# LARS-research/RED-GNN

Hardware: AMD Instinct MI355X
Metric: edges aggregated/sec + MRR-eval queries/sec, family KG n_layer=3 at 1/2/4/8 GPU (higher is better)
Workload: dtype f32; 1 GPU; C2 synthetic KG 10000 entities / 50 relations / 200000 triples (seed 1234), n_layer=3 hidden_dim=64 attn_dim=5, eval step = expansion + fused layers + GRU/readout + filtered ranking, 1024 queries per GPU; batch_per_gpu=1024, global_batch=1024

## Files before the change

include/redgnn.h:

```cpp
#ifndef REDGNN_H
#define REDGNN_H

#include <stddef.h>
#include <stdint.h>

#ifdef __cplusplus
extern "C" {
#endif

typedef struct rg_graph rg_graph;
typedef struct rg_frontier rg_frontier;

const char* rg_last_error(void);
int rg_version(void);
int rg_hipgraph_fill_nodes(void* hip_graph);

int rg_graph_create(int32_t n_ent, int32_t n_rel, const int32_t* triples_host, int64_t n,
                    int add_inverse, rg_graph** out);
int rg_graph_create_device(int32_t n_ent, int32_t n_rel, const int32_t* triples_dev, int64_t n,
                           int add_inverse, void* stream, rg_graph** out);
int rg_graph_export_packs(const rg_graph* g, int32_t* n_packs, int32_t* n_vrows, int32_t* ent_host, int32_t* pack_host, int32_t* rows_host,
                          int32_t* vrows_host);
int rg_tgraph_create(int32_t n_ent, int32_t n_rela_rows, int32_t n_time, const int32_t* quads_host, int64_t n,
                     rg_graph** out);
int rg_tgraph_create_excluding(int32_t n_ent, int32_t n_rela_rows, int32_t n_time, const int32_t* quads_host, int64_t n,
                               const int64_t* exclude_rows_host, int64_t n_exclude, rg_graph** out);
int rg_graph_destroy(rg_graph* g);
int64_t rg_graph_n_fact(const rg_graph* g);
int rg_graph_export(const rg_graph* g, int32_t* out_ptr_host, int32_t* out_rel_tail_host,
                    int32_t* in_ptr_host, int32_t* in_head_rel_host);
int rg_graph_export_out_by_tail(const rg_graph* g, int32_t* rel_tail_host, int32_t* pos_host, uint32_t* packed_host);
int rg_graph_export_time(const rg_graph* g, int32_t* out_time_host, int32_t* in_time_host);

size_t rg_frontier_workspace_bytes(int32_t n_ent, int32_t batch, int32_t n_levels);
int rg_frontier_create(int32_t n_ent, int32_t batch, int32_t n_levels, void* workspace_dev,
                       size_t workspace_bytes, rg_frontier** out);
int rg_frontier_destroy(rg_frontier* f);
int rg_frontier_reset(rg_frontier* f, const int32_t* q_sub_dev, void* stream);
int rg_frontier_reset_nodes(rg_frontier* f, const int32_t* nodes_dev, int64_t n, void* stream);
int rg_frontier_expand(rg_frontier* f, const rg_graph* g, int64_t* counts_host, void* stream);
int rg_frontier_expand_async(rg_frontier* f, const rg_graph* g, void* stream);
int rg_frontier_expand_nodes_async(rg_frontier* f, const rg_graph* g, int32_t* nodes_out, int32_t* prev_idx_out, void* stream);
int rg_frontier_set_edge_hint(rg_frontier* f, int64_t n_edges);
const int32_t* rg_frontier_count_ptr(const rg_frontier* f);
int rg_frontier_level_counts(const rg_frontier* f, int64_t* counts_host, void* stream);
int rg_frontier_nodes(const rg_frontier* f, int32_t* nodes_out, int32_t* prev_idx_out,
                      int32_t* old_nodes_new_idx_out, void* stream);
size_t rg_frontier_edges_scratch_bytes(int64_t n_new);
int rg_frontier_edges(const rg_frontier* f, const rg_graph* g, int32_t level,
                      const int32_t* nodes_new, int64_t n_new, int32_t* edges_out,
                      int32_t* row_ptr_out, void* scratch_dev, void* stream);

size_t rg_layer_fwd_scratch_bytes(const rg_frontier* f, const rg_graph* g, int32_t ld);
int rg_layer_fwd_plan(const rg_frontier* f, const rg_graph* g, int32_t level, int64_t n_old, int64_t n_new,
                      int64_t n_edges, int32_t ld);
int rg_layer_fwd_single_source(const rg_frontier* f, const rg_graph* g, int32_t level);
int rg_layer_fwd(const rg_frontier* f, const rg_graph* g, int32_t level, int64_t n_new,
                 const float* hidden, const float* rela, int32_t d, int32_t ld,
                 const float* a_s, const float* a_r, const float* a_q, int32_t ap,
                 const float* w_alpha, const float* b_alpha, int32_t attn_dim,
                 float* agg_out, void* scratch_dev, size_t scratch_bytes, int32_t walk, void* stream);

int rg_attn_tables(int32_t n_layer, int32_t n_rela_rows, int32_t batch, int32_t d, int32_t ld, int32_t attn_dim, int32_t ap,
                   const float* const* rela, const float* const* Wr, const float* const* Wqr, const float* const* bqr,
                   const int64_t* q_rel, float* a_r_out, float* a_q_out, float* rela_pad_out, void* stream);

int rg_tlayer_fwd(const rg_frontier* f, const rg_graph* g, int32_t level, int64_t n_new, const int32_t* q_time,
                  const float* hidden_dir, const float* rela_dir, const float* time_dir, int32_t d, int32_t ld,
                  const float* a_s, const float* a_r, const float* a_q, int32_t ap,
                  const float* w_alpha, const float* b_alpha, int32_t attn_dim,
                  float* agg_out, void* scratch_dev, size_t scratch_bytes, void* stream);

int rg_frontier_set_window(rg_frontier* f, const int32_t* win_lo_dev, const int32_t* win_hi_dev, int32_t n_data);
int rg_xlayer_fwd(const rg_frontier* f, const rg_graph* g, int32_t level, int64_t n_new, const int32_t* q_time,
                  const int32_t* loop_time, const int32_t* row_time, int32_t n_data,
                  const float* hidden_p, const float* rela_p, const float* time_p, int32_t n_tab, int32_t d, int32_t ld,
                  const float* a_s, const float* a_r, const float* a_q, int32_t ap,
                  const float* w_alpha, const float* b_alpha, int32_t attn_dim,
                  float* agg_out, void* scratch_dev, size_t scratch_bytes, void* stream);

size_t rg_layer_bwd_scratch_bytes(const rg_frontier* f, const rg_graph* g, int32_t ld, int32_t ap);
int rg_layer_bwd(const rg_frontier* f, const rg_graph* g, int32_t level, int64_t n_old,
                 const float* hidden, const float* rela, int32_t d, int32_t ld,
                 const float* a_s, const float* a_r, const float* a_q, int32_t ap,
                 const float* w_alpha, const float* b_alpha, int32_t attn_dim,
                 const float* grad_agg,
                 float* grad_hidden, float* grad_rela, float* grad_a_s, float* grad_a_r, float* grad_a_q,
                 float* grad_w_alpha, float* grad_b_alpha,
                 void* scratch_dev, size_t scratch_bytes, void* stream);

size_t rg_tlayer_bwd_scratch_bytes(const rg_frontier* f, const rg_graph* g, int32_t ld, int32_t ap);
int rg_tlayer_bwd(const rg_frontier* f, const rg_graph* g, int32_t level, int64_t n_old, const int32_t* q_time,
                  const float* hidden_dir, const float* rela_dir, const float* time_dir, int32_t d, int32_t ld,
                  const float* a_s, const float* a_r, const float* a_q, int32_t ap,
                  const float* w_alpha, const float* b_alpha, int32_t attn_dim,
                  const float* grad_agg,
                  float* grad_hidden_dir, float* grad_rela_dir, float* grad_time_dir, float* grad_a_s, float* grad_a_r,
                  float* grad_a_q, float* grad_w_alpha,
                  void* scratch_dev, size_t scratch_bytes, void* stream);

int rg_xlayer_bwd(const rg_frontier* f, const rg_graph* g, int32_t level, int64_t n_old, const int32_t* q_time,
                  const int32_t* loop_time, const int32_t* row_time, int32_t n_data,
                  const float* hidden_p, const float* rela_p, const float* time_p, int32_t n_tab, int32_t d, int32_t ld,
                  const float* a_s, const float* a_r, const float* a_q, int32_t ap,
                  const float* w_alpha, const float* b_alpha, int32_t attn_dim,
                  const float* grad_agg,
                  float* grad_hidden_p, float* grad_rela_p, float* grad_time_p, float* grad_a_s, float* grad_a_r,
                  float* grad_a_q, float* grad_w_alpha,
                  void* scratch_dev, size_t scratch_bytes, void* stream);

int rg_dense_fwd_supported(int32_t d, int32_t attn_dim);
int rg_dense_fwd(int64_t n, int32_t d, int32_t ld, const float* agg, const float* hidden_prev,
                 const int32_t* prev_idx, const float* W_h, int32_t act,
                 const float* w_ih, const float* w_hh, const float* b_ih, const float* b_hh,
                 const float* Ws_next, int32_t attn_dim, int32_t ap, float* a_s_out,
                 const float* W_final, const int32_t* nodes, int32_t n_ent, float* scores_all,
                 float* hidden_out, int32_t precision, void* scratch, int64_t scratch_bytes, void* stream);
int64_t rg_dense_scratch_bytes(int32_t d, int32_t precision);

int rg_split3_roundtrip(const float* x, int64_t n_rows, int32_t cols, float* back, float* parts, void* stream);
int rg_split3_product_check(int32_t which, int64_t n, int32_t d, const float* agg, const float* hidden_prev, const int32_t* prev_idx,
                            const float* W_h, int32_t act, const float* w_ih, const float* w_hh, const float* b_ih, const float* b_hh,
                            float* out, void* stream);

size_t rg_gram_tn_scratch_bytes(int32_t m, int32_t n);
int rg_gram_tn(const float* g, int64_t ldg, int32_t m, const float* x, int64_t ldx, int32_t n, int64_t n_rows, float* out, float* colsum,
               void* scratch_dev, size_t scratch_bytes, void* stream);

int rg_rank(const float* scores, int32_t batch, int32_t n_ent,
            const int32_t* ans_ptr, const int32_t* ans_idx,
            const int32_t* filt_ptr, const int32_t* filt_idx,
            float* ranks_out, void* stream);

int rg_topk(const float* scores, int32_t batch, int32_t n_ent, int32_t k, const int64_t* q_key,
            const int64_t* known_keys, const int64_t* known_ptr, const int32_t* known_idx, int64_t n_keys,
            int32_t* idx_out, float* score_out, void* stream);

int rg_segment_rank(const float* scores, const int32_t* ent, int64_t n_pairs, const void* seg_ptr, int32_t seg_ptr_is64,
                    const int32_t* target, int32_t batch,
                    const int64_t* key_sp, const int64_t* sp_keys, const int64_t* sp_ptr, const int32_t* sp_idx, int64_t n_sp,
                    const int64_t* key_spt, const int64_t* spt_keys, const int64_t* spt_ptr, const int32_t* spt_idx, int64_t n_spt,
                    float* rank_out, float* rank_fil_out, float* rank_fil_t_out, int32_t* found_out, void* stream);

int rg_segment_topk(const float* scores, const int32_t* ent, int64_t n_pairs, const void* seg_ptr, int32_t seg_ptr_is64,
                    int32_t batch, int32_t k, const int64_t* q_key, const int64_t* known_keys, const int64_t* known_ptr,
                    const int32_t* known_idx, int64_t n_keys, int32_t* idx_out, float* score_out, float* prob_out, void* stream);

int rg_segment_eval(const float* scores, const int32_t* ent, int64_t n_pairs, const void* seg_ptr, int32_t seg_ptr_is64,
                    const int32_t* target, int32_t batch, int32_t n_ent,
                    const int64_t* key_a, const int64_t* a_keys, const int64_t* a_ptr, const int32_t* a_idx, int64_t n_a,
                    const int64_t* key_b, const int64_t* b_keys, const int64_t* b_ptr, const int32_t* b_idx, int64_t n_b,
                    float* logp_out, int32_t* count_out, int32_t* visited_out, void* stream);

size_t rg_paths_scratch_bytes(int64_t n_edges, int32_t k);
int rg_paths_topk(const int32_t* edges, const float* alpha, const int64_t* offsets, int32_t row_lo, int32_t row_hi, int32_t n_hops,
                  int32_t k, void* scratch, int64_t* path_edge, double* path_prod, int32_t* path_count, void* stream);

size_t rg_rule_ground_scratch_bytes(int32_t n_ent, int32_t n_rules, int32_t n_sources);
int rg_rule_ground(const rg_graph* g, const int32_t* head, const int32_t* body, int32_t n_rules, int32_t n_hops,
                   const int32_t* sources, int32_t n_sources, void* scratch, int64_t* counts, void* stream);

int rg_dense_fwd_dev(int64_t n_cap, const int32_t* n_dev, int64_t n_hint, int32_t d, int32_t ld, const float* agg, const float* hidden_prev,
                     const int32_t* prev_idx, const float* W_h, int32_t act,
                     const float* w_ih, const float* w_hh, const float* b_ih, const float* b_hh,
                     const float* Ws_next, int32_t attn_dim, int32_t ap, float* a_s_out,
                     const float* W_final, const int32_t* nodes, int32_t n_ent, float* scores_all,
                     float* hidden_out, int32_t precision, void* scratch, int64_t scratch_bytes, void* stream);

int rg_dense_train_fwd(int64_t n, int32_t d, const float* agg, const float* hidden_prev, const int32_t* prev_idx,
                       const float* W_h, int32_t act, const float* w_ih, const float* w_hh, const float* b_ih, const float* b_hh,
                       const float* mask, float* hidden_out, float* x_out, float* gates_ws_out, void* stream);

int rg_dense_train_fwd_as(int64_t n, int32_t d, const float* agg, const float* hidden_prev, const int32_t* prev_idx,
                          const float* W_h, int32_t act, const float* w_ih, const float* w_hh, const float* b_ih, const float* b_hh,
                          const float* mask, const float* Ws_next, int32_t attn_dim, int32_t ap,
                          float* hidden_out, float* x_out, float* gates_ws_out, float* a_s_out, void* stream);

int rg_rows_addmm(const float* base, int64_t ldb, const float* g, int64_t ldg, int32_t k, const float* W, int32_t n, int64_t n_rows,
                  float* out, int64_t ldo, void* stream);

int rg_rows_linear(const float* x, int64_t n_rows, int64_t ldx, int32_t k, const float* w, const float* bias, int32_t n,
                   float* out, int64_t ldo, void* stream);

int rg_dense_train_bwd(int64_t n, int32_t d, const float* grad_hidden, const float* gates_ws, const float* x, const float* mask,
                       float keep, int32_t act, const float* W_h, const float* w_ih, const float* w_hh,
                       float* grad_gates_i, float* grad_gates_h, float* grad_pre, float* grad_agg, float* grad_h0, void* stream);

int rg_dense_train_bwd2(int64_t n, int32_t d, const float* grad_hidden, const float* gates_ws, const float* x, const float* mask,
                        float keep, int32_t act, const float* W_h, const float* w_ih, const float* w_hh, const int32_t* prev_idx,
                        float* grad_gates_i, float* grad_gates_hn, float* grad_pre, float* grad_agg, float* grad_prev, void* stream);

size_t rg_explain_scratch_bytes(const rg_frontier* f);
int rg_explain_seed(const rg_frontier* f, int32_t batch, int32_t n_ent, int32_t level, const int32_t* objs, uint32_t* marks_out,
                    uint8_t* reached_out, void* stream);
int rg_explain_count(const rg_frontier* f, const rg_graph* g, int32_t batch, int32_t n_ent, int32_t level, const uint32_t* marks,
                     const float* a_s, const float* a_r, const float* a_q, int32_t ap, const float* w_alpha, const float* b_alpha,
                     int32_t attn_dim, float min_alpha, uint32_t* marks_prev_out, int32_t* word_ptr_out, void* scratch,
                     size_t scratch_bytes, int64_t* n_edges_host, void* stream);
int rg_explain_emit(const rg_frontier* f, const rg_graph* g, int32_t batch, int32_t n_ent, int32_t level, const uint32_t* marks,
                    const float* a_s, const float* a_r, const float* a_q, int32_t ap, const float* w_alpha, const float* b_alpha,
                    int32_t attn_dim, float min_alpha, const int32_t* word_ptr, int32_t* edges_out, float* alpha_out, void* stream);
int rg_explain_gather(int64_t n, int32_t hop, int32_t batch, const int32_t* edges, const float* alpha, const int64_t* row_first,
                      const int64_t* row_base, int64_t n_out, int32_t* edges_out, float* alpha_out, void* stream);

int rg_texplain_count(const rg_frontier* f, const rg_graph* g, int32_t batch, int32_t n_ent, int32_t level, const uint32_t* marks,
                      const float* a_s, const float* a_r, const float* a_q, int32_t ap, const float* w_alpha, const float* b_alpha,
                      int32_t attn_dim, float min_alpha, uint32_t* marks_prev_out, int32_t* word_ptr_out, void* scratch,
                      size_t scratch_bytes, int64_t* n_edges_host, void* stream);
int rg_texplain_emit(const rg_frontier* f, const rg_graph* g, int32_t batch, int32_t n_ent, int32_t level, const uint32_t* marks,
                     const float* a_s, const float* a_r, const float* a_q, int32_t ap, const float* w_alpha, const float* b_alpha,
                     int32_t attn_dim, float min_alpha, const int32_t* word_ptr, int32_t* edges_out, float* alpha_out,
                     int32_t* time_out, void* stream);

int rg_xexplain_count(const rg_frontier* f, const rg_graph* g, int32_t batch, int32_t n_ent, int32_t level, const uint32_t* marks,
                      const float* a_s, const float* a_r, const float* a_q, int32_t ap, const float* w_alpha, const float* b_alpha,
                      int32_t attn_dim, float min_alpha, uint32_t* marks_prev_out, int32_t* word_ptr_out, void* scratch,
                      size_t scratch_bytes, int64_t* n_edges_host, void* stream);
int rg_xexplain_emit(const rg_frontier* f, const rg_graph* g, int32_t batch, int32_t n_ent, int32_t level, const uint32_t* marks,
                     const float* a_s, const float* a_r, const float* a_q, int32_t ap, const float* w_alpha, const float* b_alpha,
                     int32_t attn_dim, float min_alpha, const int32_t* word_ptr, int32_t* edges_out, float* alpha_out,
                     int32_t* row_out, void* stream);

int rg_attn_profile(const rg_frontier* f, const rg_graph* g, int32_t batch, int32_t n_ent, int32_t level, int64_t n_old,
                    const float* a_s, const float* a_r, const float* a_q, int32_t ap, const float* w_alpha, const float* b_alpha,
                    int32_t attn_dim, int64_t* sum_out, int64_t* count_out, void* stream);

int rg_tattn_profile(const rg_frontier* f, const rg_graph* g, int32_t batch, int32_t n_ent, int32_t level, int64_t n_old,
                     const int32_t* q_time, const float* a_s, const float* a_r, const float* a_q, int32_t ap, const float* w_alpha,
                     const float* b_alpha, int32_t attn_dim, int64_t* sum_out, int64_t* count_out, void* stream);

int rg_xattn_profile(const rg_frontier* f, const rg_graph* g, int32_t batch, int32_t n_ent, int32_t level, int64_t n_old,
                     const int32_t* q_time, const int32_t* loop_time, const int32_t* row_time,
                     const uint8_t* lag_bin, int32_t n_lag, int32_t n_bins,
                     const float* a_s, const float* a_r, const float* a_q, int32_t ap, const float* w_alpha,
                     const float* b_alpha, int32_t attn_dim, int64_t* sum_out, int64_t* count_out, void* stream);

#ifdef __cplusplus
}
#endif
#endif
```

red-gnn_amd/_lib.py:

```python
import ctypes as C
import os

_PKG = os.path.dirname(os.path.abspath(__file__))
LIB_PATH = os.environ.get("RG_LIB") or os.path.join(_PKG, "libredgnn.so")

SYMBOLS = [
    "rg_last_error", "rg_version", "rg_hipgraph_fill_nodes",
    "rg_graph_create", "rg_graph_create_device", "rg_graph_export_packs", "rg_tgraph_create", "rg_tgraph_create_excluding", "rg_graph_destroy", "rg_graph_n_fact", "rg_graph_export", "rg_graph_export_out_by_tail",
    "rg_frontier_workspace_bytes", "rg_frontier_create", "rg_frontier_destroy", "rg_frontier_reset",
    "rg_frontier_reset_nodes", "rg_frontier_expand", "rg_frontier_nodes", "rg_frontier_edges_scratch_bytes", "rg_frontier_edges",
    "rg_layer_fwd_scratch_bytes", "rg_layer_fwd", "rg_layer_fwd_plan", "rg_layer_fwd_single_source", "rg_tlayer_fwd", "rg_xlayer_fwd", "rg_frontier_set_window", "rg_layer_bwd_scratch_bytes", "rg_layer_bwd", "rg_tlayer_bwd_scratch_bytes", "rg_tlayer_bwd", "rg_xlayer_bwd", "rg_dense_fwd_supported", "rg_dense_scratch_bytes", "rg_dense_fwd", "rg_dense_fwd_dev", "rg_dense_train_fwd", "rg_dense_train_fwd_as", "rg_rows_addmm", "rg_dense_train_bwd", "rg_dense_train_bwd2", "rg_split3_roundtrip", "rg_split3_product_check", "rg_gram_tn_scratch_bytes", "rg_gram_tn", "rg_rank",
    "rg_frontier_expand_async", "rg_frontier_expand_nodes_async", "rg_frontier_set_edge_hint", "rg_frontier_count_ptr", "rg_frontier_level_counts", "rg_attn_tables",
    "rg_explain_scratch_bytes", "rg_explain_seed", "rg_explain_count", "rg_explain_emit", "rg_explain_gather",
    "rg_topk",
    "rg_attn_profile",
    "rg_graph_export_time", "rg_texplain_count", "rg_texplain_emit", "rg_tattn_profile",
    "rg_segment_rank", "rg_segment_topk",
    "rg_xexplain_count", "rg_xexplain_emit",
    "rg_xattn_profile", "rg_rows_linear",
    "rg_segment_eval",
    "rg_paths_scratch_bytes", "rg_paths_topk",
    "rg_rule_ground_scratch_bytes", "rg_rule_ground",
]

_lib = None


class NativeError(RuntimeError):
    pass


def lib():
    global _lib
    if _lib is not None:
        return _lib
    if not os.path.exists(LIB_PATH):
        raise NativeError(
            "libredgnn.so is missing at %s: the HIP extension is not built. Run "
            "`python -c 'import __graft_entry__ as g; g.build()'` (needs hipcc). There is no CPU fallback." % LIB_PATH)
    import torch
    L = C.CDLL(LIB_PATH)
    vp, i32, i64, sz = C.c_void_p, C.c_int32, C.c_int64, C.c_size_t
    L.rg_last_error.restype = C.c_char_p
    L.rg_version.restype = C.c_int
    L.rg_hipgraph_fill_nodes.argtypes = [vp]
    L.rg_graph_create.argtypes = [i32, i32, vp, i64, C.c_int, C.POINTER(vp)]
    L.rg_graph_create_device.argtypes = [i32, i32, vp, i64, C.c_int, vp, C.POINTER(vp)]
    L.rg_graph_export_packs.argtypes = [vp, C.POINTER(i32), C.POINTER(i32), vp, vp, vp, vp]
    L.rg_tgraph_create.argtypes = [i32, i32, i32, vp, i64, C.POINTER(vp)]
    L.rg_tgraph_create_excluding.argtypes = [i32, i32, i32, vp, i64, vp, i64, C.POINTER(vp)]
    L.rg_graph_destroy.argtypes = [vp]
    L.rg_graph_n_fact.argtypes = [vp]
    L.rg_graph_n_fact.restype = i64
    L.rg_graph_export.argtypes = [vp, vp, vp, vp, vp]
    L.rg_graph_export_out_by_tail.argtypes = [vp, vp, vp, vp]
    L.rg_frontier_workspace_bytes.argtypes = [i32, i32, i32]
    L.rg_frontier_workspace_bytes.restype = sz
    L.rg_frontier_create.argtypes = [i32, i32, i32, vp, sz, C.POINTER(vp)]
    L.rg_frontier_destroy.argtypes = [vp]
    L.rg_frontier_reset.argtypes = [vp, vp, vp]
    L.rg_frontier_reset_nodes.argtypes = [vp, vp, i64, vp]
    L.rg_frontier_expand.argtypes = [vp, vp, C.POINTER(i64), vp]
    L.rg_frontier_expand_async.argtypes = [vp, vp, vp]
    L.rg_frontier_expand_nodes_async.argtypes = [vp, vp, vp, vp, vp]
    L.rg_frontier_set_edge_hint.argtypes = [vp, i64]
    L.rg_attn_tables.argtypes = [i32, i32, i32, i32, i32, i32, i32, vp, vp, vp, vp, vp, vp, vp, vp, vp]
    L.rg_frontier_count_ptr.argtypes = [vp]
    L.rg_frontier_count_ptr.restype = vp
    L.rg_frontier_level_counts.argtypes = [vp, C.POINTER(i64), vp]
    L.rg_frontier_nodes.argtypes = [vp, vp, vp, vp, vp]
    L.rg_frontier_edges_scratch_bytes.argtypes = [i64]
    L.rg_frontier_edges_scratch_bytes.restype = sz
    L.rg_frontier_edges.argtypes = [vp, vp, i32, vp, i64, vp, vp, vp, vp]
    L.rg_layer_fwd_scratch_bytes.argtypes = [vp, vp, i32]
    L.rg_layer_fwd_scratch_bytes.restype = sz
    L.rg_layer_fwd.argtypes = [vp, vp, i32, i64, vp, vp, i32, i32, vp, vp, vp, i32, vp, vp, i32, vp, vp, sz, i32, vp]
    L.rg_layer_fwd_plan.argtypes = [vp, vp, i32, i64, i64, i64, i32]
    L.rg_layer_fwd_single_source.argtypes = [vp, vp, i32]
    L.rg_tlayer_fwd.argtypes = [vp, vp, i32, i64, vp, vp, vp, vp, i32, i32, vp, vp, vp, i32, vp, vp, i32, vp, vp, sz, vp]
    L.rg_xlayer_fwd.argtypes = [vp, vp, i32, i64, vp, vp, vp, i32, vp, vp, vp, i32, i32, i32, vp, vp, vp, i32, vp, vp, i32, vp, vp, sz, vp]
    L.rg_frontier_set_window.argtypes = [vp, vp, vp, i32]
    L.rg_layer_bwd_scratch_bytes.argtypes = [vp, vp, i32, i32]
    L.rg_layer_bwd_scratch_bytes.restype = sz
    L.rg_layer_bwd.argtypes = [vp, vp, i32, i64, vp, vp, i32, i32, vp, vp, vp, i32, vp, vp, i32,
                               vp, vp, vp, vp, vp, vp, vp, vp, vp, sz, vp]
    L.rg_tlayer_bwd_scratch_bytes.argtypes = [vp, vp, i32, i32]
    L.rg_tlayer_bwd_scratch_bytes.restype = sz
    L.rg_tlayer_bwd.argtypes = [vp, vp, i32, i64, vp, vp, vp, vp, i32, i32, vp, vp, vp, i32, vp, vp, i32,
                                vp, vp, vp, vp, vp, vp, vp, vp, vp, sz, vp]
    L.rg_xlayer_bwd.argtypes = [vp, vp, i32, i64, vp, vp, vp, i32, vp, vp, vp, i32, i32, i32, vp, vp, vp, i32, vp, vp, i32,
                                vp, vp, vp, vp, vp, vp, vp, vp, vp, sz, vp]
    L.rg_dense_fwd_supported.argtypes = [i32, i32]
    L.rg_dense_fwd.argtypes = [i64, i32, i32, vp, vp, vp, vp, i32, vp, vp, vp, vp, vp, i32, i32, vp, vp, vp, i32, vp, vp, i32, vp, i64, vp]
    L.rg_dense_scratch_bytes.argtypes = [i32, i32]
    L.rg_dense_scratch_bytes.restype = i64
    L.rg_dense_fwd_dev.argtypes = [i64, vp, i64, i32, i32, vp, vp, vp, vp, i32, vp, vp, vp, vp, vp, i32, i32, vp, vp, vp, i32, vp, vp, i32, vp, i64, vp]
    L.rg_dense_train_fwd.argtypes = [i64, i32, vp, vp, vp, vp, i32, vp, vp, vp, vp, vp, vp, vp, vp, vp]
    L.rg_dense_train_fwd_as.argtypes = [i64, i32, vp, vp, vp, vp, i32, vp, vp, vp, vp, vp, vp, i32, i32, vp, vp, vp, vp, vp]
    L.rg_rows_addmm.argtypes = [vp, i64, vp, i64, i32, vp, i32, i64, vp, i64, vp]
    L.rg_dense_train_bwd.argtypes = [i64, i32, vp, vp, vp, vp, C.c_float, i32, vp, vp, vp, vp, vp, vp, vp, vp, vp]
    L.rg_dense_train_bwd2.argtypes = [i64, i32, vp, vp, vp, vp, C.c_float, i32, vp, vp, vp, vp, vp, vp, vp, vp, vp, vp]
    L.rg_rank.argtypes = [vp, i32, i32, vp, vp, vp, vp, vp, vp]
    L.rg_topk.argtypes = [vp, i32, i32, i32, vp, vp, vp, vp, i64, vp, vp, vp]
    L.rg_split3_roundtrip.argtypes = [vp, i64, i32, vp, vp, vp]
    L.rg_gram_tn_scratch_bytes.argtypes = [i32, i32]
    L.rg_gram_tn_scratch_bytes.restype = sz
    L.rg_gram_tn.argtypes = [vp, i64, i32, vp, i64, i32, i64, vp, vp, vp, sz, vp]
    L.rg_split3_product_check.argtypes = [i32, i64, i32, vp, vp, vp, vp, i32, vp, vp, vp, vp, vp, vp]
    L.rg_explain_scratch_bytes.argtypes = [vp]
    L.rg_explain_scratch_bytes.restype = sz
    L.rg_explain_seed.argtypes = [vp, i32, i32, i32, vp, vp, vp, vp]
    L.rg_explain_count.argtypes = [vp, vp, i32, i32, i32, vp, vp, vp, vp, i32, vp, vp, i32, C.c_float, vp, vp, vp, sz,
                                   C.POINTER(i64), vp]
    L.rg_explain_emit.argtypes = [vp, vp, i32, i32, i32, vp, vp, vp, vp, i32, vp, vp, i32, C.c_float, vp, vp, vp, vp]
    L.rg_explain_gather.argtypes = [i64, i32, i32, vp, vp, vp, vp, i64, vp, vp, vp]
    L.rg_attn_profile.argtypes = [vp, vp, i32, i32, i32, i64, vp, vp, vp, i32, vp, vp, i32, vp, vp, vp]
    L.rg_graph_export_time.argtypes = [vp, vp, vp]
    L.rg_texplain_count.argtypes = L.rg_explain_count.argtypes
    L.rg_texplain_emit.argtypes = [vp, vp, i32, i32, i32, vp, vp, vp, vp, i32, vp, vp, i32, C.c_float, vp, vp, vp, vp, vp]
    L.rg_tattn_profile.argtypes = [vp, vp, i32, i32, i32, i64, vp, vp, vp, vp, i32, vp, vp, i32, vp, vp, vp]
    L.rg_segment_rank.argtypes = [vp, vp, i64, vp, i32, vp, i32, vp, vp, vp, vp, i64, vp, vp, vp, vp, i64, vp, vp, vp, vp, vp]
    L.rg_segment_topk.argtypes = [vp, vp, i64, vp, i32, i32, i32, vp, vp, vp, vp, i64, vp, vp, vp, vp]
    L.rg_segment_eval.argtypes = [vp, vp, i64, vp, i32, vp, i32, i32, vp, vp, vp, vp, i64, vp, vp, vp, vp, i64, vp, vp, vp, vp]
    L.rg_xexplain_count.argtypes = L.rg_explain_count.argtypes
    L.rg_xexplain_emit.argtypes = L.rg_texplain_emit.argtypes
    L.rg_rows_linear.argtypes = [vp, i64, i64, i32, vp, vp, i32, vp, i64, vp]
    L.rg_xattn_profile.argtypes = [vp, vp, i32, i32, i32, i64, vp, vp, vp, vp, i32, i32, vp, vp, vp, i32, vp, vp, i32, vp, vp, vp]
    L.rg_paths_scratch_bytes.argtypes = [i64, i32]
    L.rg_paths_scratch_bytes.restype = sz
    L.rg_paths_topk.argtypes = [vp, vp, vp, i32, i32, i32, i32, vp, vp, vp, vp, vp]
    L.rg_rule_ground_scratch_bytes.argtypes = [i32, i32, i32]
    L.rg_rule_ground_scratch_bytes.restype = sz
    L.rg_rule_ground.argtypes = [vp, vp, vp, i32, i32, vp, i32, vp, vp, vp]
    _lib = L
    return L


def check(rc):
    if rc != 0:
        raise NativeError(lib().rg_last_error().decode("utf-8", "replace"))


def ptr(t):
    if t is None:
        return None
    if hasattr(t, "data_ptr"):
        return C.c_void_p(t.data_ptr())
    return C.c_void_p(t.ctypes.data)


def stream_ptr():
    import torch
    return C.c_void_p(torch.cuda.current_stream().cuda_stream)
```

red-gnn_amd/csrc/attn.h:

```cpp
#pragma once
#include "common.h"

namespace rg {

__device__ __forceinline__ bool bm_has(const int2& wp, int e) { return ((uint32_t)wp.x >> (e & 31)) & 1u; }
__device__ __forceinline__ int bm_rank(const int2& wp, int e) { return wp.y + __popc((uint32_t)wp.x & ((1u << (e & 31)) - 1u)); }

__device__ __forceinline__ float4 f4add(const float4& a, const float4& b) { return make_float4(a.x + b.x, a.y + b.y, a.z + b.z, a.w + b.w); }

__device__ __forceinline__ float4 attn_w4(const float* __restrict__ w_alpha, int attn_dim, int k) {
  float w[4];
#pragma unroll
  for (int u = 0; u < 4; ++u) w[u] = 4 * k + u < attn_dim ? w_alpha[4 * k + u] : 0.f;
  return make_float4(w[0], w[1], w[2], w[3]);
}

template <int AP4, int BLOCK>
__device__ __forceinline__ void stage_attention(float4* ar_l, float4* w_l, const float4* __restrict__ a_r, int n_rows,
                                                const float* __restrict__ w_alpha, int attn_dim) {
  for (int i = threadIdx.x; i < n_rows * AP4; i += BLOCK) ar_l[i] = a_r[i];
  if (threadIdx.x < AP4) w_l[threadIdx.x] = attn_w4(w_alpha, attn_dim, threadIdx.x);
}

__device__ __forceinline__ float attn_term(float& z, float w, float pre) {
  const float zr = fmaxf(pre, 0.f);
  z = fmaf(w, zr, z);
  return zr;
}
__device__ __forceinline__ void attn_acc(float& z, const float4& w, const float4& u, const float4& v, float4& zr) {
  zr.x = attn_term(z, w.x, u.x + v.x);
  zr.y = attn_term(z, w.y, u.y + v.y);
  zr.z = attn_term(z, w.z, u.z + v.z);
  zr.w = attn_term(z, w.w, u.w + v.w);
}
__device__ __forceinline__ void attn_acc(float& z, const float4& w, const float4& u, const float4& v) {
  float4 zr;
  attn_acc(z, w, u, v, zr);
}
__device__ __forceinline__ void attn_acc_fwd(float& z, const float4& w, const float4& as, const float4& ar, const float4& aq) {
  attn_term(z, w.x, as.x + ar.x + aq.x);
  attn_term(z, w.y, as.y + ar.y + aq.y);
  attn_term(z, w.z, as.z + ar.z + aq.z);
  attn_term(z, w.w, as.w + ar.w + aq.w);
}

__device__ __forceinline__ float attn_alpha(float z) { return __builtin_amdgcn_rcpf(1.0f + __expf(-z)); }

template <bool WG_RELEASE>
__device__ __forceinline__ void strip_fence() {
  if constexpr (WG_RELEASE) __builtin_amdgcn_fence(__ATOMIC_RELEASE, "workgroup");
  else __builtin_amdgcn_fence(__ATOMIC_ACQ_REL, "wavefront");
  __builtin_amdgcn_wave_barrier();
}

template <int G, bool WG_RELEASE>
__device__ __forceinline__ int group_compact(float4* my_stage, int lane, bool valid, const float4& t) {
  const int lane_g = lane & (G - 1), gshift = lane & ~(G - 1);
  const unsigned long long gmask = G == 64 ? ~0ull : ((1ull << G) - 1ull);
  const unsigned long long m = (__ballot(valid) >> gshift) & gmask;
  const int cnt = __popcll(m);
  const int pos = __popcll(m & ((1ull << lane_g) - 1ull));
  strip_fence<WG_RELEASE>();
  if (lane_g >= cnt) my_stage[lane_g] = f4zero();
  if (valid) my_stage[pos] = t;
  strip_fence<WG_RELEASE>();
  return cnt;
}

}
```

red-gnn_amd/csrc/common.h:

```cpp
#pragma once
#include <hip/hip_runtime.h>
#include <stdint.h>
#include <stdio.h>
#include <string>
#include <type_traits>

#include "redgnn.h"

namespace rg {

void set_error(const char* fmt, ...);

#define RG_CHECK(cond, ...)                 \
  do {                                      \
    if (!(cond)) {                          \
      ::rg::set_error(__VA_ARGS__);         \
      return 1;                             \
    }                                       \
  } while (0)

#define RG_HIP(expr)                                                                  \
  do {                                                                                \
    hipError_t e_ = (expr);                                                           \
    if (e_ != hipSuccess) {                                                           \
      ::rg::set_error("%s failed: %s (%s:%d)", #expr, hipGetErrorString(e_), __FILE__, \
                      __LINE__);                                                      \
      return 1;                                                                       \
    }                                                                                 \
  } while (0)

#define RG_LAUNCH_CHECK() RG_HIP(hipGetLastError())

int zero_async(void* p, size_t bytes, hipStream_t s);
int zero2_async(void* p1, size_t bytes1, void* p2, size_t bytes2, hipStream_t s);
int copy_words_async(void* dst, const void* src, int n_words, hipStream_t s);

static inline int64_t ceil_div(int64_t a, int64_t b) { return (a + b - 1) / b; }
static inline size_t align_up(size_t x, size_t a) { return (x + a - 1) / a * a; }

size_t scan_scratch_elems(int64_t n);
int scan_exclusive(const uint32_t* in, int32_t* out, int64_t n, bool popc, int32_t* total_dev,
                   int32_t* scratch, hipStream_t s);

template <typename F>
inline int with_ap4(int ap4, const char* who, F&& f) {
  switch (ap4) {
    case 1: return f(std::integral_constant<int, 1>());
    case 2: return f(std::integral_constant<int, 2>());
    case 3: return f(std::integral_constant<int, 3>());
    case 4: return f(std::integral_constant<int, 4>());
    case 8: return f(std::integral_constant<int, 8>());
    default: set_error("%s: padded attention dim %d not in {4,8,12,16,32}", who, ap4 * 4); return 1;
  }
}

template <typename F>
inline int with_g(int ld4, F&& f) {
  if (ld4 <= 4) return f(std::integral_constant<int, 4>());
  if (ld4 <= 8) return f(std::integral_constant<int, 8>());
  if (ld4 <= 16) return f(std::integral_constant<int, 16>());
  if (ld4 <= 32) return f(std::integral_constant<int, 32>());
  return f(std::integral_constant<int, 64>());
}

__device__ __forceinline__ float4 f4zero() { return make_float4(0.f, 0.f, 0.f, 0.f); }

template <int CTRL>
__device__ __forceinline__ float dpp_add(float v) {
  const int t = __builtin_amdgcn_update_dpp(0, __float_as_int(v), CTRL, 0xf, 0xf, false);
  return v + __int_as_float(t);
}

template <int G>
__device__ __forceinline__ float group_sum(float v) {
  if constexpr (G >= 16) {
    v = dpp_add<0x128>(v);
    v = dpp_add<0x124>(v);
    v = dpp_add<0x122>(v);
    v = dpp_add<0x121>(v);
    if constexpr (G >= 32) v += __shfl_xor(v, 16, 64);
    if constexpr (G >= 64) v += __shfl_xor(v, 32, 64);
  } else {
    for (int o = G / 2; o > 0; o >>= 1) v += __shfl_xor(v, o, 64);
  }
  return v;
}

}

#include <vector>
namespace rg { int place_rows_best_fit(const int4* vrows, int32_t n_vrows, std::vector<int4>* place, std::vector<int32_t>* pack_nrows); }

constexpr int RG_VROW_MAX = 128;
struct rg_vrows {
  int32_t n = 0, n_split = 0, n_slots = 0;
  int4* rows = nullptr;
  int4* split = nullptr;
};

constexpr int RG_PACK = 128;
struct rg_packs {
  int32_t n = 0;
  int2* ent = nullptr;
  int4* pack = nullptr;
  int2* rows = nullptr;
};

struct rg_graph {
  void* arena = nullptr;
  int32_t n_ent = 0, n_rel = 0;
  int32_t n_rela_rows = 0;
  int32_t n_time = 0;
  int32_t* in_time = nullptr;
  int32_t* out_time = nullptr;
  int64_t n_fact = 0;
  int32_t max_in_deg = 0, max_out_deg = 0;
  int32_t* out_ptr = nullptr;
  int2* out_rt = nullptr;
  int32_t* in_ptr = nullptr;
  int2* in_hr = nullptr;
  uint32_t* in_pk = nullptr;
  uint32_t* out_pk = nullptr;
  int2* out_bt_rt = nullptr;
  uint32_t* out_bt_pk = nullptr;
  int32_t* out_bt_pos = nullptr;
  rg_vrows in_vr, out_vr;
  rg_packs in_pk_packs;
  int32_t* rel_ptr = nullptr;
  int2* rel_ht = nullptr;
  rg_vrows rel_vr;
  int32_t* rel_tm = nullptr;
  int32_t* time_ptr = nullptr;
  int2* time_ht = nullptr;
  int32_t* time_rel = nullptr;
  rg_vrows time_vr;
};

constexpr int RG_MAX_LEVELS = 16;
constexpr int RG_QSTRIDE = 32;
constexpr size_t RG_QUEUE_BYTES = 8 * RG_QSTRIDE * sizeof(int32_t);
struct rg_frontier {
  int32_t n_ent = 0, B = 0, BW = 0, W = 0, n_levels = 0;
  uint32_t* bitsT[2] = {nullptr, nullptr};
  int2* bm[RG_MAX_LEVELS] = {};
  uint32_t* words_tmp = nullptr;
  int32_t* prefix_tmp = nullptr;
  int32_t* scan_scratch = nullptr;
  int32_t* counters = nullptr;
  const int32_t* win_lo = nullptr;
  const int32_t* win_hi = nullptr;
  int32_t win_n_data = 0;
  mutable bool queues_clean = false;
  int32_t* queues = nullptr;
  int64_t* counts_pinned = nullptr;
  int level = -1;
  int tcur = 0;
  int64_t n_nodes[RG_MAX_LEVELS] = {};
  int64_t n_edges = 0;
  bool single_source = false;
  int32_t* sub = nullptr;
  int64_t edge_hint = -1;
  const int2* bm_of(int lvl) const { return bm[lvl % n_levels]; }
};
```

red-gnn_amd/csrc/graph.hip:

```cpp
#include <stdarg.h>
#include <string.h>

#include <algorithm>
#include <vector>

#include "common.h"

namespace rg {

static thread_local std::string g_err;

void set_error(const char* fmt, ...) {
  char buf[1024];
  va_list ap;
  va_start(ap, fmt);
  vsnprintf(buf, sizeof(buf), fmt, ap);
  va_end(ap);
  g_err = buf;
}

constexpr int SCAN_T = 256;
constexpr int SCAN_ITEMS = 8;
constexpr int SCAN_TILE = SCAN_T * SCAN_ITEMS;

template <bool POPC>
__device__ __forceinline__ int32_t scan_load(const uint32_t* in, int64_t i, int64_t n) {
  if (i >= n) return 0;
  uint32_t v = in[i];
  return POPC ? __popc(v) : (int32_t)v;
}

__device__ __forceinline__ int32_t wave_incl_scan(int32_t v) {
  const int lane = threadIdx.x & 63;
#pragma unroll
  for (int o = 1; o < 64; o <<= 1) {
    int32_t t = __shfl_up(v, o, 64);
    if (lane >= o) v += t;
  }
  return v;
}

__device__ __forceinline__ int32_t block_excl_scan(int32_t v, int32_t* block_total) {
  __shared__ int32_t wsum[SCAN_T / 64];
  const int lane = threadIdx.x & 63, w = threadIdx.x >> 6;
  int32_t inc = wave_incl_scan(v);
  if (lane == 63) wsum[w] = inc;
  __syncthreads();
  int32_t base = 0, tot = 0;
#pragma unroll
  for (int i = 0; i < SCAN_T / 64; ++i) {
    int32_t x = wsum[i];
    if (i < w) base += x;
    tot += x;
  }
  __syncthreads();
  *block_total = tot;
  return base + inc - v;
}

template <bool POPC>
__global__ __launch_bounds__(SCAN_T) void scan_reduce_kernel(const uint32_t* in, int64_t n, int32_t* sums) {
  const int64_t base = (int64_t)blockIdx.x * SCAN_TILE + (int64_t)threadIdx.x * SCAN_ITEMS;
  int32_t acc = 0;
#pragma unroll
  for (int i = 0; i < SCAN_ITEMS; ++i) acc += scan_load<POPC>(in, base + i, n);
  int32_t tot;
  block_excl_scan(acc, &tot);
  if (threadIdx.x == 0) sums[blockIdx.x] = tot;
}

template <bool POPC>
__global__ __launch_bounds__(SCAN_T) void scan_apply_kernel(const uint32_t* in, int32_t* out, int64_t n,
                                                            const int32_t* offsets, int32_t* total) {
  const int64_t base = (int64_t)blockIdx.x * SCAN_TILE + (int64_t)threadIdx.x * SCAN_ITEMS;
  int32_t v[SCAN_ITEMS];
  int32_t acc = 0;
#pragma unroll
  for (int i = 0; i < SCAN_ITEMS; ++i) {
    v[i] = scan_load<POPC>(in, base + i, n);
    acc += v[i];
  }
  int32_t tot;
  int32_t ex = block_excl_scan(acc, &tot);
  if (offsets) ex += offsets[blockIdx.x];
#pragma unroll
  for (int i = 0; i < SCAN_ITEMS; ++i) {
    if (base + i < n) out[base + i] = ex;
    ex += v[i];
  }
  if (!offsets && total && threadIdx.x == 0) *total = tot;
}

__global__ void zero_words_kernel(uint32_t* __restrict__ p, int64_t n_words) {
  const int64_t stride = (int64_t)gridDim.x * blockDim.x;
  for (int64_t i = (int64_t)blockIdx.x * blockDim.x + threadIdx.x; i < n_words; i += stride) p[i] = 0u;
}
__global__ void zero_quads_kernel(uint4* __restrict__ p, int64_t n_quads) {
  const int64_t stride = (int64_t)gridDim.x * blockDim.x;
  for (int64_t i = (int64_t)blockIdx.x * blockDim.x + threadIdx.x; i < n_quads; i += stride) p[i] = make_uint4(0u, 0u, 0u, 0u);
}
__global__ void copy_words_kernel(uint32_t* __restrict__ dst, const uint32_t* __restrict__ src, int n) {
  if ((int)threadIdx.x < n) dst[threadIdx.x] = src[threadIdx.x];
}

int zero_async(void* p, size_t bytes, hipStream_t s) {
  if (bytes == 0) return 0;
  RG_CHECK(((uintptr_t)p & 3) == 0 && (bytes & 3) == 0, "zero_async: unaligned fill (%p, %zu B)", p, bytes);
  if (((uintptr_t)p & 15) == 0 && (bytes & 15) == 0 && bytes >= 4096) {
    const int64_t n = (int64_t)(bytes / 16);
    hipLaunchKernelGGL(zero_quads_kernel, dim3((unsigned)std::min<int64_t>(ceil_div(n, 256), 4096)), dim3(256), 0, s, (uint4*)p, n);
  } else {
    const int64_t n = (int64_t)(bytes / 4);
    hipLaunchKernelGGL(zero_words_kernel, dim3((unsigned)std::min<int64_t>(ceil_div(n, 256), 4096)), dim3(256), 0, s, (uint32_t*)p, n);
  }
  RG_LAUNCH_CHECK();
  return 0;
}

__global__ void zero2_quads_kernel(uint4* __restrict__ p1, int64_t n1, uint4* __restrict__ p2, int64_t n2) {
  const int64_t stride = (int64_t)gridDim.x * blockDim.x;
  for (int64_t i = (int64_t)blockIdx.x * blockDim.x + threadIdx.x; i < n1 + n2; i += stride) {
    if (i < n1) p1[i] = make_uint4(0u, 0u, 0u, 0u);
    else p2[i - n1] = make_uint4(0u, 0u, 0u, 0u);
  }
}

int zero2_async(void* p1, size_t bytes1, void* p2, size_t bytes2, hipStream_t s) {
  if ((((uintptr_t)p1 | (uintptr_t)p2) & 15) != 0 || ((bytes1 | bytes2) & 15) != 0) return zero_async(p1, bytes1, s) || zero_async(p2, bytes2, s);
  const int64_t n = (int64_t)((bytes1 + bytes2) / 16);
  if (n == 0) return 0;
  hipLaunchKernelGGL(zero2_quads_kernel, dim3((unsigned)std::min<int64_t>(ceil_div(n, 256), 4096)), dim3(256), 0, s, (uint4*)p1,
                     (int64_t)(bytes1 / 16), (uint4*)p2, (int64_t)(bytes2 / 16));
  RG_LAUNCH_CHECK();
  return 0;
}

int copy_words_async(void* dst, const void* src, int n_words, hipStream_t s) {
  RG_CHECK(n_words > 0 && n_words <= 256, "copy_words_async: %d words", n_words);
  hipLaunchKernelGGL(copy_words_kernel, dim3(1), dim3(256), 0, s, (uint32_t*)dst, (const uint32_t*)src, n_words);
  RG_LAUNCH_CHECK();
  return 0;
}

size_t scan_scratch_elems(int64_t n) {
  size_t tot = 0;
  while (n > SCAN_TILE) {
    n = ceil_div(n, SCAN_TILE);
    tot += align_up((size_t)n, 64) * 2;
  }
  return tot + 64;
}

int scan_exclusive(const uint32_t* in, int32_t* out, int64_t n, bool popc, int32_t* total_dev,
                   int32_t* scratch, hipStream_t s) {
  if (n <= 0) {
    if (total_dev && zero_async(total_dev, sizeof(int32_t), s)) return 1;
    return 0;
  }
  const int64_t nb = ceil_div(n, SCAN_TILE);
  if (nb == 1) {
    if (popc)
      hipLaunchKernelGGL(scan_apply_kernel<true>, dim3(1), dim3(SCAN_T), 0, s, in, out, n, nullptr, total_dev);
    else
      hipLaunchKernelGGL(scan_apply_kernel<false>, dim3(1), dim3(SCAN_T), 0, s, in, out, n, nullptr, total_dev);
    RG_LAUNCH_CHECK();
    return 0;
  }
  int32_t* sums = scratch;
  int32_t* sums_scanned = scratch + align_up((size_t)nb, 64);
  int32_t* next = sums_scanned + align_up((size_t)nb, 64);
  if (popc)
    hipLaunchKernelGGL(scan_reduce_kernel<true>, dim3(nb), dim3(SCAN_T), 0, s, in, n, sums);
  else
    hipLaunchKernelGGL(scan_reduce_kernel<false>, dim3(nb), dim3(SCAN_T), 0, s, in, n, sums);
  RG_LAUNCH_CHECK();
  if (scan_exclusive((const uint32_t*)sums, sums_scanned, nb, false, total_dev, next, s)) return 1;
  if (popc)
    hipLaunchKernelGGL(scan_apply_kernel<true>, dim3(nb), dim3(SCAN_T), 0, s, in, out, n, sums_scanned, nullptr);
  else
    hipLaunchKernelGGL(scan_apply_kernel<false>, dim3(nb), dim3(SCAN_T), 0, s, in, out, n, sums_scanned, nullptr);
  RG_LAUNCH_CHECK();
  return 0;
}

}

struct HostVrows { std::vector<int4> rows, split; };
static void host_vrows(const std::vector<int32_t>& ptr, int32_t n_ent, HostVrows* h, rg_vrows* out) {
  std::vector<int4>& rows = h->rows;
  std::vector<int4>& split = h->split;
  int32_t slots = 0;
  for (int32_t e = 0; e < n_ent; ++e) {
    const int32_t beg = ptr[e], len = ptr[e + 1] - ptr[e];
    if (len <= RG_VROW_MAX) {
      rows.push_back(make_int4(e, beg, len, -1));
    } else {
      const int32_t n_seg = (len + RG_VROW_MAX - 1) / RG_VROW_MAX;
      split.push_back(make_int4(e, slots, n_seg, 0));
      for (int32_t k = 0; k < n_seg; ++k) {
        const int32_t b = beg + k * RG_VROW_MAX;
        rows.push_back(make_int4(e, b, std::min(RG_VROW_MAX, beg + len - b), slots + k));
      }
      slots += n_seg;
    }
  }
  std::stable_sort(rows.begin(), rows.end(), [](const int4& a, const int4& b) { return a.z > b.z; });
  out->n = (int32_t)rows.size(); out->n_split = (int32_t)split.size(); out->n_slots = slots;
}

struct HostPacks { std::vector<int2> ent; std::vector<int4> pack; std::vector<int2> rows; };

namespace rg {
int place_rows_best_fit(const int4* vrows, int32_t n_vrows, std::vector<int4>* place, std::vector<int32_t>* pack_nrows) {
  std::vector<int32_t> open_by_room[RG_PACK + 1];
  std::vector<int32_t> fill;
  place->assign(n_vrows, make_int4(-1, 0, 0, 0));
  pack_nrows->clear();
  for (int32_t i = 0; i < n_vrows; ++i) {
    const int4& r = vrows[i];
    if (r.z <= 0) continue;
    int32_t p;
    if (r.w >= 0) { p = (int32_t)fill.size(); fill.push_back(0); pack_nrows->push_back(0); }
    else {
      int room = r.z;
      while (room <= RG_PACK && open_by_room[room].empty()) ++room;
      if (room > RG_PACK) { p = (int32_t)fill.size(); fill.push_back(0); pack_nrows->push_back(0); room = RG_PACK; }
      else { p = open_by_room[room].back(); open_by_room[room].pop_back(); }
      if (room - r.z > 0) open_by_room[room - r.z].push_back(p);
    }
    (*place)[i] = make_int4(p, fill[p], (*pack_nrows)[p], 0);
    fill[p] += r.z;
    (*pack_nrows)[p] += 1;
  }
  return (int)fill.size();
}
}

static void host_packs(const std::vector<int4>& vrows, const std::vector<uint32_t>& in_pk, HostPacks* hp, rg_packs* out) {
  std::vector<int4> place;
  std::vector<int32_t> pack_nrows;
  const size_t n = (size_t)rg::place_rows_best_fit(vrows.data(), (int32_t)vrows.size(), &place, &pack_nrows);
  std::vector<int32_t> row0(n + 1, 0);
  for (size_t p = 0; p < n; ++p) row0[p + 1] = row0[p] + pack_nrows[p];
  hp->ent.assign(n * RG_PACK, make_int2(-1, 0));
  hp->pack.resize(n);
  hp->rows.resize(row0[n]);
  for (size_t i = 0; i < vrows.size(); ++i) {
    const int4& r = vrows[i];
    const int4& pl = place[i];
    if (pl.x < 0) continue;
    for (int32_t j = 0; j < r.z; ++j) hp->ent[(size_t)pl.x * RG_PACK + pl.y + j] = make_int2((int32_t)in_pk[r.y + j], pl.z);
    hp->rows[row0[pl.x] + pl.z] = make_int2(r.x, r.w);
    if (pl.z == 0) hp->pack[pl.x] = make_int4(row0[pl.x], pack_nrows[pl.x], r.w, r.x);
  }
  out->n = (int32_t)n;
}

struct Arena {
  struct Item { void** field; const void* src; size_t bytes, off; };
  std::vector<Item> items;
  size_t total = 0;
  template <typename P, typename V>
  void add(P** field, const V& v) {
    const size_t bytes = v.size() * sizeof(typename V::value_type);
    items.push_back({(void**)field, (const void*)v.data(), bytes, total});
    total += rg::align_up(std::max<size_t>(bytes, 16), 256);
  }
};

extern "C" {

const char* rg_last_error(void) { return rg::g_err.c_str(); }
int rg_version(void) { return 12; }

static int build_graph(int32_t n_ent, int32_t n_rel, int32_t n_rela_rows, const std::vector<int32_t>& H,
                       const std::vector<int32_t>& R, const std::vector<int32_t>& T, const std::vector<int32_t>* TIME,
                       int32_t n_time, rg_graph** out) {
  const int64_t n_fact = (int64_t)H.size();
  std::vector<int32_t> out_ptr(n_ent + 1, 0), in_ptr(n_ent + 1, 0);
  for (int64_t i = 0; i < n_fact; ++i) { out_ptr[H[i] + 1]++; in_ptr[T[i] + 1]++; }
  int32_t max_in = 0, max_out = 0;
  for (int32_t e = 0; e < n_ent; ++e) {
    max_out = out_ptr[e + 1] > max_out ? out_ptr[e + 1] : max_out;
    max_in = in_ptr[e + 1] > max_in ? in_ptr[e + 1] : max_in;
    out_ptr[e + 1] += out_ptr[e];
    in_ptr[e + 1] += in_ptr[e];
  }
  std::vector<int2> out_rt(n_fact), in_hr(n_fact);
  std::vector<int32_t> in_time(TIME ? n_fact : 0), out_time(TIME ? n_fact : 0);
  {
    std::vector<int32_t> po(out_ptr.begin(), out_ptr.end() - 1), pi(in_ptr.begin(), in_ptr.end() - 1);
    for (int64_t i = 0; i < n_fact; ++i) {
      const int32_t q = pi[T[i]]++;
      in_hr[q] = make_int2(H[i], R[i]);
      if (TIME) in_time[q] = (*TIME)[i];
    }
    std::vector<int32_t> by_rel(n_fact), out_fact(n_fact);
    {
      std::vector<int32_t> pr(n_rela_rows + 1, 0);
      for (int64_t i = 0; i < n_fact; ++i) pr[R[i] + 1]++;
      for (int32_t r = 0; r < n_rela_rows; ++r) pr[r + 1] += pr[r];
      for (int64_t i = 0; i < n_fact; ++i) by_rel[pr[R[i]]++] = (int32_t)i;
    }
    for (int64_t k = 0; k < n_fact; ++k) out_fact[po[H[by_rel[k]]]++] = by_rel[k];
    for (int64_t j = 0; j < n_fact; ++j) {
      const int32_t i = out_fact[j];
      out_rt[j] = make_int2(R[i], T[i]);
      if (TIME) out_time[j] = (*TIME)[i];
    }
  }
  rg_graph* g = new rg_graph();
  g->n_ent = n_ent; g->n_rel = n_rel; g->n_rela_rows = n_rela_rows; g->n_time = n_time;
  g->n_fact = n_fact; g->max_in_deg = max_in; g->max_out_deg = max_out;
  Arena A;
  A.add(&g->out_ptr, out_ptr); A.add(&g->in_ptr, in_ptr); A.add(&g->out_rt, out_rt); A.add(&g->in_hr, in_hr);
  if (TIME) { A.add(&g->in_time, in_time); A.add(&g->out_time, out_time); }
  std::vector<uint32_t> in_pk, out_pk;
  if (n_ent <= (1 << 20) && n_rela_rows <= (1 << 12)) {
    in_pk.resize(n_fact); out_pk.resize(n_fact);
    for (int64_t i = 0; i < n_fact; ++i) {
      in_pk[i] = ((uint32_t)in_hr[i].y << 20) | (uint32_t)in_hr[i].x;
      out_pk[i] = ((uint32_t)out_rt[i].x << 20) | (uint32_t)out_rt[i].y;
    }
    A.add(&g->in_pk, in_pk); A.add(&g->out_pk, out_pk);
  }
  std::vector<int2> out_bt_rt;
  std::vector<uint32_t> out_bt_pk;
  std::vector<int32_t> out_bt_pos;
  if (!TIME) {
    out_bt_rt.resize(n_fact); out_bt_pos.resize(n_fact);
    std::vector<int32_t> po(out_ptr.begin(), out_ptr.end() - 1);
    for (int32_t t = 0; t < n_ent; ++t)
      for (int32_t q = in_ptr[t]; q < in_ptr[t + 1]; ++q) {
        const int32_t j = po[in_hr[q].x]++;
        out_bt_rt[j] = make_int2(in_hr[q].y, t);
        out_bt_pos[j] = q;
      }
    A.add(&g->out_bt_rt, out_bt_rt); A.add(&g->out_bt_pos, out_bt_pos);
    if (!in_pk.empty()) {
      out_bt_pk.resize(n_fact);
      for (int64_t j = 0; j < n_fact; ++j) out_bt_pk[j] = ((uint32_t)out_bt_rt[j].x << 20) | (uint32_t)out_bt_rt[j].y;
      A.add(&g->out_bt_pk, out_bt_pk);
    }
  }
  std::vector<int32_t> rel_ptr(n_rela_rows + 1, 0), rel_tm(TIME ? n_fact : 0);
  std::vector<int2> rel_ht(n_fact);
  for (int64_t i = 0; i < n_fact; ++i) rel_ptr[R[i] + 1]++;
  for (int32_t r = 0; r < n_rela_rows; ++r) rel_ptr[r + 1] += rel_ptr[r];
  {
    std::vector<int32_t> pr(rel_ptr.begin(), rel_ptr.end() - 1);
    for (int64_t i = 0; i < n_fact; ++i) {
      const int32_t q = pr[R[i]]++;
      rel_ht[q] = make_int2(H[i], T[i]);
      if (TIME) rel_tm[q] = (*TIME)[i];
    }
  }
  A.add(&g->rel_ptr, rel_ptr); A.add(&g->rel_ht, rel_ht);
  std::vector<int32_t> time_ptr, time_rel;
  std::vector<int2> time_ht;
  HostVrows hv_in, hv_out, hv_rel, hv_time;
  if (TIME) {
    A.add(&g->rel_tm, rel_tm);
    time_ptr.assign(n_time + 1, 0); time_rel.resize(n_fact); time_ht.resize(n_fact);
    for (int64_t i = 0; i < n_fact; ++i) time_ptr[(*TIME)[i] + 1]++;
    for (int32_t t = 0; t < n_time; ++t) time_ptr[t + 1] += time_ptr[t];
    std::vector<int32_t> pt(time_ptr.begin(), time_ptr.end() - 1);
    for (int64_t i = 0; i < n_fact; ++i) {
      const int32_t q = pt[(*TIME)[i]]++;
      time_ht[q] = make_int2(H[i], T[i]);
      time_rel[q] = R[i];
    }
    A.add(&g->time_ptr, time_ptr); A.add(&g->time_ht, time_ht); A.add(&g->time_rel, time_rel);
    host_vrows(time_ptr, n_time, &hv_time, &g->time_vr);
    A.add(&g->time_vr.rows, hv_time.rows); A.add(&g->time_vr.split, hv_time.split);
  }
  host_vrows(in_ptr, n_ent, &hv_in, &g->in_vr);
  host_vrows(out_ptr, n_ent, &hv_out, &g->out_vr);
  host_vrows(rel_ptr, n_rela_rows, &hv_rel, &g->rel_vr);
  A.add(&g->in_vr.rows, hv_in.rows); A.add(&g->in_vr.split, hv_in.split);
  A.add(&g->out_vr.rows, hv_out.rows); A.add(&g->out_vr.split, hv_out.split);
  A.add(&g->rel_vr.rows, hv_rel.rows); A.add(&g->rel_vr.split, hv_rel.split);
  HostPacks hp;
  if (!TIME && !in_pk.empty() && n_rela_rows < (1 << 12)) {
    host_packs(hv_in.rows, in_pk, &hp, &g->in_pk_packs);
    A.add(&g->in_pk_packs.ent, hp.ent); A.add(&g->in_pk_packs.pack, hp.pack); A.add(&g->in_pk_packs.rows, hp.rows);
  }

  std::vector<char> staging(A.total);
  for (const Arena::Item& it : A.items)
    if (it.bytes) memcpy(staging.data() + it.off, it.src, it.bytes);
  hipError_t e = hipMalloc(&g->arena, A.total);
  if (e == hipSuccess) e = hipMemcpy(g->arena, staging.data(), A.total, hipMemcpyHostToDevice);
  if (e != hipSuccess) {
    rg::set_error("rg_graph_create: uploading %zu B failed: %s", A.total, hipGetErrorString(e));
    rg_graph_destroy(g);
    return 1;
  }
  for (const Arena::Item& it : A.items) *it.field = (char*)g->arena + it.off;
  *out = g;
  return 0;
}

int rg_graph_create(int32_t n_ent, int32_t n_rel, const int32_t* triples, int64_t n, int add_inverse,
                    rg_graph** out) {
  RG_CHECK(out != nullptr, "rg_graph_create: out is NULL");
  *out = nullptr;
  RG_CHECK(n_ent > 0 && n_rel > 0, "rg_graph_create: n_ent=%d n_rel=%d must be positive", n_ent, n_rel);
  RG_CHECK(n >= 0 && (n == 0 || triples != nullptr), "rg_graph_create: bad triples (n=%lld)", (long long)n);
  const int64_t n_fact = (add_inverse ? 2 * n : n) + n_ent;
  RG_CHECK(n_fact < (int64_t)1 << 31, "rg_graph_create: %lld fact rows do not fit int32", (long long)n_fact);
  std::vector<int32_t> H(n_fact), R(n_fact), T(n_fact);
  const int32_t max_rel = add_inverse ? n_rel : 2 * n_rel;
  for (int64_t i = 0; i < n; ++i) {
    const int32_t h = triples[3 * i], r = triples[3 * i + 1], t = triples[3 * i + 2];
    RG_CHECK(h >= 0 && h < n_ent && t >= 0 && t < n_ent && r >= 0 && r < max_rel,
             "rg_graph_create: triple %lld = (%d,%d,%d) out of range", (long long)i, h, r, t);
    H[i] = h; R[i] = r; T[i] = t;
    if (add_inverse) { H[n + i] = t; R[n + i] = r + n_rel; T[n + i] = h; }
  }
  const int64_t id0 = n_fact - n_ent;
  for (int32_t e = 0; e < n_ent; ++e) { H[id0 + e] = e; R[id0 + e] = 2 * n_rel; T[id0 + e] = e; }
  return build_graph(n_ent, n_rel, 2 * n_rel + 1, H, R, T, nullptr, 0, out);
}

static int tgraph_create(const char* who, int32_t n_ent, int32_t n_rela_rows, int32_t n_time, const int32_t* quads, int64_t n,
                         const int64_t* exclude, int64_t n_exclude, rg_graph** out) {
  RG_CHECK(out != nullptr, "%s: out is NULL", who);
  *out = nullptr;
  RG_CHECK(n_ent > 0 && n_rela_rows > 0 && n_time > 0, "%s: n_ent=%d n_rela_rows=%d n_time=%d must be positive", who, n_ent, n_rela_rows, n_time);
  RG_CHECK(n >= 0 && n < ((int64_t)1 << 31) && (n == 0 || quads != nullptr), "%s: bad quadruples (n=%lld)", who, (long long)n);
  RG_CHECK(n_exclude >= 0 && (n_exclude == 0 || exclude != nullptr), "%s: bad exclusion list", who);
  std::vector<char> drop(n_exclude ? n : 0, 0);
  for (int64_t k = 0; k < n_exclude; ++k) {
    RG_CHECK(exclude[k] >= 0 && exclude[k] < n, "%s: excluded row %lld out of range (n=%lld)", who, (long long)exclude[k], (long long)n);
    drop[exclude[k]] = 1;
  }
  std::vector<int32_t> H, R, T, TM;
  H.reserve(n); R.reserve(n); T.reserve(n); TM.reserve(n);
  for (int64_t i = 0; i < n; ++i) {
    if (n_exclude && drop[i]) continue;
    const int32_t h = quads[4 * i], r = quads[4 * i + 1], t = quads[4 * i + 2], tm = quads[4 * i + 3];
    RG_CHECK(h >= 0 && h < n_ent && t >= 0 && t < n_ent && r >= 0 && r < n_rela_rows && tm >= 0 && tm < n_time,
             "%s: quadruple %lld = (%d,%d,%d,%d) out of range", who, (long long)i, h, r, t, tm);
    H.push_back(h); R.push_back(r); T.push_back(t); TM.push_back(tm);
  }
  return build_graph(n_ent, 0, n_rela_rows, H, R, T, &TM, n_time, out);
}

int rg_tgraph_create(int32_t n_ent, int32_t n_rela_rows, int32_t n_time, const int32_t* quads, int64_t n, rg_graph** out) {
  return tgraph_create("rg_tgraph_create", n_ent, n_rela_rows, n_time, quads, n, nullptr, 0, out);
}

int rg_tgraph_create_excluding(int32_t n_ent, int32_t n_rela_rows, int32_t n_time, const int32_t* quads, int64_t n,
                               const int64_t* exclude_rows, int64_t n_exclude, rg_graph** out) {
  return tgraph_create("rg_tgraph_create_excluding", n_ent, n_rela_rows, n_time, quads, n, exclude_rows, n_exclude, out);
}

int rg_graph_destroy(rg_graph* g) {
  if (!g) return 0;
  if (g->arena) (void)hipFree(g->arena);
  delete g;
  return 0;
}

int64_t rg_graph_n_fact(const rg_graph* g) { return g ? g->n_fact : -1; }

int rg_graph_export(const rg_graph* g, int32_t* out_ptr, int32_t* out_rt, int32_t* in_ptr, int32_t* in_hr) {
  RG_CHECK(g != nullptr, "rg_graph_export: graph is NULL");
  if (out_ptr) RG_HIP(hipMemcpy(out_ptr, g->out_ptr, (g->n_ent + 1) * sizeof(int32_t), hipMemcpyDeviceToHost));
  if (in_ptr) RG_HIP(hipMemcpy(in_ptr, g->in_ptr, (g->n_ent + 1) * sizeof(int32_t), hipMemcpyDeviceToHost));
  if (out_rt) RG_HIP(hipMemcpy(out_rt, g->out_rt, g->n_fact * sizeof(int2), hipMemcpyDeviceToHost));
  if (in_hr) RG_HIP(hipMemcpy(in_hr, g->in_hr, g->n_fact * sizeof(int2), hipMemcpyDeviceToHost));
  return 0;
}

int rg_graph_export_out_by_tail(const rg_graph* g, int32_t* rel_tail, int32_t* pos, uint32_t* packed) {
  RG_CHECK(g != nullptr, "rg_graph_export_out_by_tail: graph is NULL");
  RG_CHECK(g->out_bt_rt && g->out_bt_pos, "rg_graph_export_out_by_tail: the graph has no out-list by tail (static graphs only)");
  RG_CHECK(!packed || g->out_bt_pk, "rg_graph_export_out_by_tail: the graph's entries are not packed");
  if (rel_tail) RG_HIP(hipMemcpy(rel_tail, g->out_bt_rt, g->n_fact * sizeof(int2), hipMemcpyDeviceToHost));
  if (pos) RG_HIP(hipMemcpy(pos, g->out_bt_pos, g->n_fact * sizeof(int32_t), hipMemcpyDeviceToHost));
  if (packed) RG_HIP(hipMemcpy(packed, g->out_bt_pk, g->n_fact * sizeof(uint32_t), hipMemcpyDeviceToHost));
  return 0;
}

int rg_graph_export_time(const rg_graph* g, int32_t* out_time, int32_t* in_time) {
  RG_CHECK(g != nullptr, "rg_graph_export_time: graph is NULL");
  RG_CHECK(g->n_time > 0 && g->in_time && g->out_time, "rg_graph_export_time: the graph has no timestamps (build it with rg_tgraph_create)");
  if (out_time) RG_HIP(hipMemcpy(out_time, g->out_time, g->n_fact * sizeof(int32_t), hipMemcpyDeviceToHost));
  if (in_time) RG_HIP(hipMemcpy(in_time, g->in_time, g->n_fact * sizeof(int32_t), hipMemcpyDeviceToHost));
  return 0;
}

int rg_hipgraph_fill_nodes(void* graph) {
  size_t n = 0;
  if (hipGraphGetNodes((hipGraph_t)graph, nullptr, &n) != hipSuccess) { rg::set_error("rg_hipgraph_fill_nodes: hipGraphGetNodes failed"); return -1; }
  std::vector<hipGraphNode_t> nodes(n);
  if (n && hipGraphGetNodes((hipGraph_t)graph, nodes.data(), &n) != hipSuccess) { rg::set_error("rg_hipgraph_fill_nodes: hipGraphGetNodes failed"); return -1; }
  int count = 0;
  for (size_t i = 0; i < n; ++i) {
    hipGraphNodeType t;
    if (hipGraphNodeGetType(nodes[i], &t) != hipSuccess) { rg::set_error("rg_hipgraph_fill_nodes: hipGraphNodeGetType failed"); return -1; }
    if (t == hipGraphNodeTypeMemset) ++count;
  }
  return count;
}

int rg_graph_export_packs(const rg_graph* g, int32_t* n_packs, int32_t* n_vrows, int32_t* ent, int32_t* pack, int32_t* rows, int32_t* vrows) {
  RG_CHECK(g != nullptr, "rg_graph_export_packs: graph is NULL");
  if (n_packs) *n_packs = g->in_pk_packs.n;
  if (n_vrows) *n_vrows = g->in_vr.n;
  if (ent && g->in_pk_packs.n) RG_HIP(hipMemcpy(ent, g->in_pk_packs.ent, (size_t)g->in_pk_packs.n * RG_PACK * sizeof(int2), hipMemcpyDeviceToHost));
  if (pack && g->in_pk_packs.n) RG_HIP(hipMemcpy(pack, g->in_pk_packs.pack, (size_t)g->in_pk_packs.n * sizeof(int4), hipMemcpyDeviceToHost));
  if (rows && g->in_pk_packs.n) RG_HIP(hipMemcpy(rows, g->in_pk_packs.rows, (size_t)g->in_vr.n * sizeof(int2), hipMemcpyDeviceToHost));
  if (vrows) RG_HIP(hipMemcpy(vrows, g->in_vr.rows, (size_t)g->in_vr.n * sizeof(int4), hipMemcpyDeviceToHost));
  return 0;
}

}
```

red-gnn_amd/csrc/graph_device.hip:

```cpp
#include <hipcub/hipcub.hpp>

#include <algorithm>
#include <vector>

#include "common.h"

namespace {

struct Tmp {
  std::vector<void*> ptrs;
  char* block = nullptr;
  size_t block_bytes = 0, used = 0;
  explicit Tmp(size_t bytes) {
    if (hipMalloc((void**)&block, bytes) == hipSuccess) block_bytes = bytes; else block = nullptr;
  }
  template <typename T>
  T* get(size_t n) {
    const size_t bytes = rg::align_up(std::max<size_t>(n, 1) * sizeof(T), 256);
    if (used + bytes <= block_bytes) { T* p = (T*)(block + used); used += bytes; return p; }
    void* p = nullptr;
    if (hipMalloc(&p, bytes) != hipSuccess) return nullptr;
    ptrs.push_back(p);
    return (T*)p;
  }
  ~Tmp() {
    for (void* p : ptrs) (void)hipFree(p);
    if (block) (void)hipFree(block);
  }
};

__global__ void rows_kernel(const int32_t* __restrict__ trip, int64_t n, int add_inverse, int n_ent, int n_rel, int max_rel,
                            int32_t* __restrict__ H, int32_t* __restrict__ R, int32_t* __restrict__ T, int64_t n_fact, int32_t* __restrict__ err) {
  const int64_t i = (int64_t)blockIdx.x * blockDim.x + threadIdx.x;
  if (i >= n_fact) return;
  const int64_t n_dir = add_inverse ? 2 * n : n;
  if (i < n_dir) {
    const int64_t j = i < n ? i : i - n;
    const int32_t h = trip[3 * j], r = trip[3 * j + 1], t = trip[3 * j + 2];
    if (h < 0 || h >= n_ent || t < 0 || t >= n_ent || r < 0 || r >= max_rel) { atomicMax(err, 1 + (int32_t)std::min<int64_t>(j, 0x7ffffffe)); H[i] = R[i] = T[i] = 0; return; }
    if (i < n) { H[i] = h; R[i] = r; T[i] = t; }
    else { H[i] = t; R[i] = r + n_rel; T[i] = h; }
  } else {
    const int32_t e = (int32_t)(i - n_dir);
    H[i] = e; R[i] = 2 * n_rel; T[i] = e;
  }
}

__global__ void iota_kernel(uint32_t* __restrict__ v, int64_t n) {
  const int64_t i = (int64_t)blockIdx.x * blockDim.x + threadIdx.x;
  if (i < n) v[i] = (uint32_t)i;
}

template <int MODE>
__global__ void keys_kernel(const int32_t* __restrict__ H, const int32_t* __restrict__ R, const int32_t* __restrict__ T, int rel_bits,
                            uint64_t* __restrict__ keys, int64_t n) {
  const int64_t i = (int64_t)blockIdx.x * blockDim.x + threadIdx.x;
  if (i >= n) return;
  keys[i] = MODE == 0 ? (uint64_t)T[i] : (MODE == 1 ? (((uint64_t)H[i] << rel_bits) | (uint64_t)R[i])
                                       : (MODE == 2 ? (uint64_t)R[i] : (((uint64_t)H[i] << rel_bits) | (uint64_t)T[i])));
}

__global__ void invert_perm_kernel(const uint32_t* __restrict__ perm, int32_t* __restrict__ inv, int64_t n) {
  const int64_t q = (int64_t)blockIdx.x * blockDim.x + threadIdx.x;
  if (q < n) inv[perm[q]] = (int32_t)q;
}
__global__ void gather_words_kernel(const uint32_t* __restrict__ perm, const int32_t* __restrict__ in, int32_t* __restrict__ out, int64_t n) {
  const int64_t j = (int64_t)blockIdx.x * blockDim.x + threadIdx.x;
  if (j < n) out[j] = in[perm[j]];
}

__global__ void hist_kernel(const int32_t* __restrict__ key, int64_t n, uint32_t* __restrict__ cnt) {
  const int64_t i = (int64_t)blockIdx.x * blockDim.x + threadIdx.x;
  if (i < n) atomicAdd(&cnt[key[i]], 1u);
}

__global__ void gather_pairs_kernel(const uint32_t* __restrict__ perm, const int32_t* __restrict__ A, const int32_t* __restrict__ B,
                                    int2* __restrict__ out, uint32_t* __restrict__ pk, int pk_mode, int64_t n) {
  const int64_t q = (int64_t)blockIdx.x * blockDim.x + threadIdx.x;
  if (q >= n) return;
  const uint32_t i = perm[q];
  const int2 v = make_int2(A[i], B[i]);
  out[q] = v;
  if (pk) pk[q] = pk_mode == 0 ? (((uint32_t)v.y << 20) | (uint32_t)v.x)
                               : (((uint32_t)v.x << 20) | (uint32_t)v.y);
}

__global__ void vrow_count_kernel(const int32_t* __restrict__ ptr, int n_rows, uint32_t* __restrict__ n_seg, uint32_t* __restrict__ is_split,
                                  uint32_t* __restrict__ split_seg) {
  const int e = blockIdx.x * blockDim.x + threadIdx.x;
  if (e >= n_rows) return;
  const int len = ptr[e + 1] - ptr[e];
  const int cut = len > RG_VROW_MAX;
  const int k = cut ? (len + RG_VROW_MAX - 1) / RG_VROW_MAX : 1;
  n_seg[e] = k; is_split[e] = cut; split_seg[e] = cut ? k : 0;
}

__global__ void vrow_emit_kernel(const int32_t* __restrict__ ptr, int n_rows, const int32_t* __restrict__ row_off, const int32_t* __restrict__ split_off,
                                 const int32_t* __restrict__ slot_off, int4* __restrict__ rows, uint32_t* __restrict__ keys, int4* __restrict__ split) {
  const int e = blockIdx.x * blockDim.x + threadIdx.x;
  if (e >= n_rows) return;
  const int beg = ptr[e], len = ptr[e + 1] - ptr[e];
  if (len <= RG_VROW_MAX) {
    rows[row_off[e]] = make_int4(e, beg, len, -1);
    keys[row_off[e]] = (uint32_t)(RG_VROW_MAX - len);
  } else {
    const int k = (len + RG_VROW_MAX - 1) / RG_VROW_MAX;
    split[split_off[e]] = make_int4(e, slot_off[e], k, 0);
    for (int j = 0; j < k; ++j) {
      const int b = beg + j * RG_VROW_MAX, l = min(RG_VROW_MAX, beg + len - b);
      rows[row_off[e] + j] = make_int4(e, b, l, slot_off[e] + j);
      keys[row_off[e] + j] = (uint32_t)(RG_VROW_MAX - l);
    }
  }
}

__global__ void gather_rows_kernel(const uint32_t* __restrict__ perm, const int4* __restrict__ in, int4* __restrict__ out, int n) {
  const int i = blockIdx.x * blockDim.x + threadIdx.x;
  if (i < n) out[i] = in[perm[i]];
}

__global__ void pack_emit_kernel(const int4* __restrict__ vrows, const int4* __restrict__ place, int n_vrows, const int32_t* __restrict__ pack_row0,
                                 const uint32_t* __restrict__ in_pk, int2* __restrict__ ent, int4* __restrict__ pack, int2* __restrict__ rows) {
  const int i = blockIdx.x;
  if (i >= n_vrows) return;
  const int4 r = vrows[i];
  const int4 pl = place[i];
  if (pl.x < 0) return;
  for (int j = threadIdx.x; j < r.z; j += blockDim.x) ent[(int64_t)pl.x * RG_PACK + pl.y + j] = make_int2((int)in_pk[r.y + j], pl.z);
  if (threadIdx.x == 0) {
    rows[pack_row0[pl.x] + pl.z] = make_int2(r.x, r.w);
    if (pl.z == 0) pack[pl.x] = make_int4(pack_row0[pl.x], 0, r.w, r.x);
  }
}

__global__ void pack_count_kernel(const int32_t* __restrict__ pack_nrows, int4* __restrict__ pack, int n_packs) {
  const int p = blockIdx.x * blockDim.x + threadIdx.x;
  if (p < n_packs) pack[p].y = pack_nrows[p];
}

__global__ void fill_int2_kernel(int2* __restrict__ p, int64_t n, int2 v) {
  const int64_t i = (int64_t)blockIdx.x * blockDim.x + threadIdx.x;
  if (i < n) p[i] = v;
}

__global__ void max_kernel(const int32_t* __restrict__ ptr, int n_rows, int32_t* __restrict__ out) {
  const int e = blockIdx.x * blockDim.x + threadIdx.x;
  if (e < n_rows) atomicMax(out, ptr[e + 1] - ptr[e]);
}

#define DEV_HIP(expr)                                                                          \
  do {                                                                                         \
    hipError_t e_ = (expr);                                                                    \
    if (e_ != hipSuccess) {                                                                    \
      ::rg::set_error("rg_graph_create_device: %s failed: %s", #expr, hipGetErrorString(e_)); \
      return 1;                                                                                \
    }                                                                                          \
  } while (0)

inline unsigned blocks(int64_t n, int t = 256) { return (unsigned)std::max<int64_t>(rg::ceil_div(n, t), 1); }

static int sort_perm(Tmp& tmp, const uint64_t* keys, int bits, int64_t n, uint32_t* perm_out, hipStream_t s) {
  uint64_t* keys_out = tmp.get<uint64_t>(n);
  uint32_t* iota = tmp.get<uint32_t>(n);
  if (!keys_out || !iota) { rg::set_error("rg_graph_create_device: out of device memory"); return 1; }
  hipLaunchKernelGGL(iota_kernel, dim3(blocks(n)), dim3(256), 0, s, iota, n);
  size_t bytes = 0;
  DEV_HIP(hipcub::DeviceRadixSort::SortPairs(nullptr, bytes, keys, keys_out, iota, perm_out, (int)n, 0, bits, s));
  char* scratch = tmp.get<char>(bytes);
  if (!scratch) { rg::set_error("rg_graph_create_device: out of device memory"); return 1; }
  DEV_HIP(hipcub::DeviceRadixSort::SortPairs(scratch, bytes, keys, keys_out, iota, perm_out, (int)n, 0, bits, s));
  return 0;
}

static int build_ptr(Tmp& tmp, const int32_t* key, int64_t n, int n_rows, int32_t* ptr, hipStream_t s) {
  uint32_t* cnt = tmp.get<uint32_t>(n_rows + 1);
  int32_t* scr = tmp.get<int32_t>(rg::scan_scratch_elems(n_rows + 1));
  if (!cnt || !scr) { rg::set_error("rg_graph_create_device: out of device memory"); return 1; }
  DEV_HIP(hipMemsetAsync(cnt, 0, (size_t)(n_rows + 1) * 4, s));
  hipLaunchKernelGGL(hist_kernel, dim3(blocks(n)), dim3(256), 0, s, key, n, cnt);
  return rg::scan_exclusive(cnt, ptr, n_rows + 1, false, nullptr, scr, s);
}

struct VrowsDev { int4* rows = nullptr; int4* split = nullptr; int32_t* counts = nullptr; int cap_rows = 0, cap_split = 0; };

static int build_vrows(Tmp& tmp, const int32_t* ptr, int n_rows, int64_t n_fact, VrowsDev* out, hipStream_t s) {
  uint32_t* n_seg = tmp.get<uint32_t>(n_rows + 1);
  uint32_t* is_split = tmp.get<uint32_t>(n_rows + 1);
  uint32_t* split_seg = tmp.get<uint32_t>(n_rows + 1);
  int32_t* row_off = tmp.get<int32_t>(n_rows + 1);
  int32_t* split_off = tmp.get<int32_t>(n_rows + 1);
  int32_t* slot_off = tmp.get<int32_t>(n_rows + 1);
  int32_t* scr = tmp.get<int32_t>(rg::scan_scratch_elems(n_rows + 1));
  out->cap_rows = (int)(n_rows + n_fact / RG_VROW_MAX + 2);
  out->cap_split = (int)(n_fact / (RG_VROW_MAX + 1) + 2);
  int4* rows_u = tmp.get<int4>(out->cap_rows);
  uint32_t* keys = tmp.get<uint32_t>(out->cap_rows);
  uint32_t* keys_o = tmp.get<uint32_t>(out->cap_rows);
  uint32_t* iota = tmp.get<uint32_t>(out->cap_rows);
  uint32_t* perm = tmp.get<uint32_t>(out->cap_rows);
  out->rows = tmp.get<int4>(out->cap_rows);
  out->split = tmp.get<int4>(out->cap_split);
  out->counts = tmp.get<int32_t>(4);
  if (!n_seg || !is_split || !split_seg || !row_off || !split_off || !slot_off || !scr || !rows_u || !keys || !keys_o || !iota || !perm ||
      !out->rows || !out->split || !out->counts) { rg::set_error("rg_graph_create_device: out of device memory"); return 1; }
  hipLaunchKernelGGL(vrow_count_kernel, dim3(blocks(n_rows)), dim3(256), 0, s, ptr, n_rows, n_seg, is_split, split_seg);
  if (rg::scan_exclusive(n_seg, row_off, n_rows, false, &out->counts[0], scr, s)) return 1;
  if (rg::scan_exclusive(is_split, split_off, n_rows, false, &out->counts[1], scr, s)) return 1;
  if (rg::scan_exclusive(split_seg, slot_off, n_rows, false, &out->counts[2], scr, s)) return 1;
  hipLaunchKernelGGL(vrow_emit_kernel, dim3(blocks(n_rows)), dim3(256), 0, s, ptr, n_rows, row_off, split_off, slot_off, rows_u, keys, out->split);
  int32_t n_v = 0;
  DEV_HIP(hipMemcpyAsync(&n_v, &out->counts[0], 4, hipMemcpyDeviceToHost, s));
  DEV_HIP(hipStreamSynchronize(s));
  hipLaunchKernelGGL(iota_kernel, dim3(blocks(n_v)), dim3(256), 0, s, iota, (int64_t)n_v);
  size_t bytes = 0;
  DEV_HIP(hipcub::DeviceRadixSort::SortPairs(nullptr, bytes, keys, keys_o, iota, perm, n_v, 0, 8, s));
  char* scratch = tmp.get<char>(bytes);
  if (!scratch) { rg::set_error("rg_graph_create_device: out of device memory"); return 1; }
  DEV_HIP(hipcub::DeviceRadixSort::SortPairs(scratch, bytes, keys, keys_o, iota, perm, n_v, 0, 8, s));
  hipLaunchKernelGGL(gather_rows_kernel, dim3(blocks(n_v)), dim3(256), 0, s, perm, rows_u, out->rows, n_v);
  RG_LAUNCH_CHECK();
  return 0;
}

}

extern "C" int rg_graph_create_device(int32_t n_ent, int32_t n_rel, const int32_t* triples_dev, int64_t n, int add_inverse, void* stream,
                                      rg_graph** out) {
  RG_CHECK(out != nullptr, "rg_graph_create_device: out is NULL");
  *out = nullptr;
  RG_CHECK(n_ent > 0 && n_rel > 0, "rg_graph_create_device: n_ent=%d n_rel=%d must be positive", n_ent, n_rel);
  RG_CHECK(n >= 0 && (n == 0 || triples_dev != nullptr), "rg_graph_create_device: bad triples (n=%lld)", (long long)n);
  const int64_t n_fact = (add_inverse ? 2 * n : n) + n_ent;
  RG_CHECK(n_fact < (int64_t)1 << 31, "rg_graph_create_device: %lld fact rows do not fit int32", (long long)n_fact);
  hipStream_t s = (hipStream_t)stream;
  const int n_rela_rows = 2 * n_rel + 1;
  const int max_rel = add_inverse ? n_rel : 2 * n_rel;
  int rel_bits = 1, ent_bits = 1;
  while ((1 << rel_bits) < n_rela_rows) ++rel_bits;
  while (((int64_t)1 << ent_bits) < n_ent) ++ent_bits;
  Tmp tmp((size_t)n_fact * 208 + (size_t)n_ent * 96 + ((size_t)8 << 20));
  int32_t* H = tmp.get<int32_t>(n_fact); int32_t* R = tmp.get<int32_t>(n_fact); int32_t* T = tmp.get<int32_t>(n_fact);
  uint64_t* keys = tmp.get<uint64_t>(n_fact);
  uint32_t* perm_in = tmp.get<uint32_t>(n_fact); uint32_t* perm_out = tmp.get<uint32_t>(n_fact); uint32_t* perm_rel = tmp.get<uint32_t>(n_fact);
  int32_t* flags = tmp.get<int32_t>(16);
  int32_t* out_ptr = tmp.get<int32_t>(n_ent + 2); int32_t* in_ptr = tmp.get<int32_t>(n_ent + 2); int32_t* rel_ptr = tmp.get<int32_t>(n_rela_rows + 2);
  int2* out_rt = tmp.get<int2>(n_fact); int2* in_hr = tmp.get<int2>(n_fact); int2* rel_ht = tmp.get<int2>(n_fact);
  const bool packed = n_ent <= (1 << 20) && n_rela_rows <= (1 << 12);
  uint32_t* in_pk = packed ? tmp.get<uint32_t>(n_fact) : nullptr; uint32_t* out_pk = packed ? tmp.get<uint32_t>(n_fact) : nullptr;
  RG_CHECK(H && R && T && keys && perm_in && perm_out && perm_rel && flags && out_ptr && in_ptr && rel_ptr && out_rt && in_hr && rel_ht &&
           (!packed || (in_pk && out_pk)), "rg_graph_create_device: out of device memory");
  DEV_HIP(hipMemsetAsync(flags, 0, 64, s));
  hipLaunchKernelGGL(rows_kernel, dim3(blocks(n_fact)), dim3(256), 0, s, triples_dev, n, add_inverse, n_ent, n_rel, max_rel, H, R, T, n_fact, flags);
  hipLaunchKernelGGL(keys_kernel<0>, dim3(blocks(n_fact)), dim3(256), 0, s, H, R, T, rel_bits, keys, n_fact);
  if (sort_perm(tmp, keys, ent_bits, n_fact, perm_in, s)) return 1;
  hipLaunchKernelGGL(keys_kernel<1>, dim3(blocks(n_fact)), dim3(256), 0, s, H, R, T, rel_bits, keys, n_fact);
  if (sort_perm(tmp, keys, ent_bits + rel_bits, n_fact, perm_out, s)) return 1;
  hipLaunchKernelGGL(keys_kernel<2>, dim3(blocks(n_fact)), dim3(256), 0, s, H, R, T, rel_bits, keys, n_fact);
  if (sort_perm(tmp, keys, rel_bits, n_fact, perm_rel, s)) return 1;
  hipLaunchKernelGGL(gather_pairs_kernel, dim3(blocks(n_fact)), dim3(256), 0, s, perm_in, H, R, in_hr, in_pk, 0, n_fact);
  hipLaunchKernelGGL(gather_pairs_kernel, dim3(blocks(n_fact)), dim3(256), 0, s, perm_out, R, T, out_rt, out_pk, 1, n_fact);
  hipLaunchKernelGGL(gather_pairs_kernel, dim3(blocks(n_fact)), dim3(256), 0, s, perm_rel, H, T, rel_ht, (uint32_t*)nullptr, 0, n_fact);
  uint32_t* perm_bt = tmp.get<uint32_t>(n_fact); int32_t* inv_in = tmp.get<int32_t>(n_fact);
  int2* out_bt_rt = tmp.get<int2>(n_fact); int32_t* out_bt_pos = tmp.get<int32_t>(n_fact);
  uint32_t* out_bt_pk = packed ? tmp.get<uint32_t>(n_fact) : nullptr;
  RG_CHECK(perm_bt && inv_in && out_bt_rt && out_bt_pos && (!packed || out_bt_pk), "rg_graph_create_device: out of device memory");
  hipLaunchKernelGGL(keys_kernel<3>, dim3(blocks(n_fact)), dim3(256), 0, s, H, R, T, ent_bits, keys, n_fact);
  if (sort_perm(tmp, keys, 2 * ent_bits, n_fact, perm_bt, s)) return 1;
  hipLaunchKernelGGL(invert_perm_kernel, dim3(blocks(n_fact)), dim3(256), 0, s, perm_in, inv_in, n_fact);
  hipLaunchKernelGGL(gather_pairs_kernel, dim3(blocks(n_fact)), dim3(256), 0, s, perm_bt, R, T, out_bt_rt, out_bt_pk, 1, n_fact);
  hipLaunchKernelGGL(gather_words_kernel, dim3(blocks(n_fact)), dim3(256), 0, s, perm_bt, inv_in, out_bt_pos, n_fact);
  if (build_ptr(tmp, T, n_fact, n_ent, in_ptr, s) || build_ptr(tmp, H, n_fact, n_ent, out_ptr, s) || build_ptr(tmp, R, n_fact, n_rela_rows, rel_ptr, s)) return 1;
  hipLaunchKernelGGL(max_kernel, dim3(blocks(n_ent)), dim3(256), 0, s, in_ptr, n_ent, &flags[1]);
  hipLaunchKernelGGL(max_kernel, dim3(blocks(n_ent)), dim3(256), 0, s, out_ptr, n_ent, &flags[2]);
  VrowsDev vin, vout, vrel;
  if (build_vrows(tmp, in_ptr, n_ent, n_fact, &vin, s) || build_vrows(tmp, out_ptr, n_ent, n_fact, &vout, s) ||
      build_vrows(tmp, rel_ptr, n_rela_rows, n_fact, &vrel, s)) return 1;
  int32_t host[16];
  DEV_HIP(hipMemcpyAsync(host, vin.counts, 12, hipMemcpyDeviceToHost, s));
  DEV_HIP(hipMemcpyAsync(host + 4, vout.counts, 12, hipMemcpyDeviceToHost, s));
  DEV_HIP(hipMemcpyAsync(host + 8, vrel.counts, 12, hipMemcpyDeviceToHost, s));
  DEV_HIP(hipMemcpyAsync(host + 12, flags, 16, hipMemcpyDeviceToHost, s));
  DEV_HIP(hipStreamSynchronize(s));
  RG_CHECK(host[12] == 0, "rg_graph_create_device: triple %d out of range", host[12] - 1);
  const bool want_packs = packed && n_rela_rows < (1 << 12);
  int4* place = nullptr; int32_t* pack_nrows = nullptr; int32_t* pack_row0 = nullptr;
  int n_packs = 0;
  if (want_packs) {
    const int nv = host[0];
    place = tmp.get<int4>(nv);
    pack_nrows = tmp.get<int32_t>(nv + 1);
    pack_row0 = tmp.get<int32_t>(nv + 1);
    int32_t* scr = tmp.get<int32_t>(rg::scan_scratch_elems(nv + 1));
    RG_CHECK(place && pack_nrows && pack_row0 && scr, "rg_graph_create_device: out of device memory");
    std::vector<int4> vrows_h(nv), place_h;
    std::vector<int32_t> nrows_h;
    DEV_HIP(hipMemcpyAsync(vrows_h.data(), vin.rows, (size_t)nv * sizeof(int4), hipMemcpyDeviceToHost, s));
    DEV_HIP(hipStreamSynchronize(s));
    n_packs = rg::place_rows_best_fit(vrows_h.data(), nv, &place_h, &nrows_h);
    DEV_HIP(hipMemcpyAsync(place, place_h.data(), (size_t)nv * sizeof(int4), hipMemcpyHostToDevice, s));
    if (n_packs) DEV_HIP(hipMemcpyAsync(pack_nrows, nrows_h.data(), (size_t)n_packs * sizeof(int32_t), hipMemcpyHostToDevice, s));
    DEV_HIP(hipStreamSynchronize(s));
    if (rg::scan_exclusive((const uint32_t*)pack_nrows, pack_row0, n_packs, false, nullptr, scr, s)) return 1;
  }
  rg_graph* g = new rg_graph();
  g->n_ent = n_ent; g->n_rel = n_rel; g->n_rela_rows = n_rela_rows; g->n_time = 0; g->n_fact = n_fact;
  g->max_in_deg = host[13]; g->max_out_deg = host[14];
  g->in_vr.n = host[0]; g->in_vr.n_split = host[1]; g->in_vr.n_slots = host[2];
  g->out_vr.n = host[4]; g->out_vr.n_split = host[5]; g->out_vr.n_slots = host[6];
  g->rel_vr.n = host[8]; g->rel_vr.n_split = host[9]; g->rel_vr.n_slots = host[10];
  g->in_pk_packs.n = n_packs;
  struct Item { void** field; const void* src; size_t bytes, off; };
  std::vector<Item> items;
  size_t total = 0;
  auto add = [&](void** field, const void* src, size_t bytes) {
    items.push_back({field, src, bytes, total});
    total += rg::align_up(std::max<size_t>(bytes, 16), 256);
  };
  add((void**)&g->out_ptr, out_ptr, (size_t)(n_ent + 1) * 4); add((void**)&g->in_ptr, in_ptr, (size_t)(n_ent + 1) * 4);
  add((void**)&g->out_rt, out_rt, (size_t)n_fact * 8); add((void**)&g->in_hr, in_hr, (size_t)n_fact * 8);
  if (packed) { add((void**)&g->in_pk, in_pk, (size_t)n_fact * 4); add((void**)&g->out_pk, out_pk, (size_t)n_fact * 4); }
  add((void**)&g->out_bt_rt, out_bt_rt, (size_t)n_fact * 8); add((void**)&g->out_bt_pos, out_bt_pos, (size_t)n_fact * 4);
  if (packed) add((void**)&g->out_bt_pk, out_bt_pk, (size_t)n_fact * 4);
  add((void**)&g->rel_ptr, rel_ptr, (size_t)(n_rela_rows + 1) * 4); add((void**)&g->rel_ht, rel_ht, (size_t)n_fact * 8);
  add((void**)&g->in_vr.rows, vin.rows, (size_t)g->in_vr.n * 16); add((void**)&g->in_vr.split, vin.split, (size_t)g->in_vr.n_split * 16);
  add((void**)&g->out_vr.rows, vout.rows, (size_t)g->out_vr.n * 16); add((void**)&g->out_vr.split, vout.split, (size_t)g->out_vr.n_split * 16);
  add((void**)&g->rel_vr.rows, vrel.rows, (size_t)g->rel_vr.n * 16); add((void**)&g->rel_vr.split, vrel.split, (size_t)g->rel_vr.n_split * 16);
  const size_t ent_off = total;
  if (n_packs > 0) {
    add((void**)&g->in_pk_packs.ent, nullptr, (size_t)n_packs * RG_PACK * 8);
    add((void**)&g->in_pk_packs.pack, nullptr, (size_t)n_packs * 16);
    add((void**)&g->in_pk_packs.rows, nullptr, (size_t)g->in_vr.n * 8);
  }
  hipError_t e = hipMalloc(&g->arena, total);
  if (e != hipSuccess) {
    rg::set_error("rg_graph_create_device: allocating %zu B failed: %s", total, hipGetErrorString(e));
    delete g;
    return 1;
  }
  for (const Item& it : items) {
    *it.field = (char*)g->arena + it.off;
    if (it.src && it.bytes) (void)hipMemcpyAsync(*it.field, it.src, it.bytes, hipMemcpyDeviceToDevice, s);
  }
  (void)ent_off;
  if (n_packs > 0) {
    hipLaunchKernelGGL(fill_int2_kernel, dim3(blocks((int64_t)n_packs * RG_PACK)), dim3(256), 0, s, g->in_pk_packs.ent, (int64_t)n_packs * RG_PACK,
                       make_int2(-1, 0));
    hipLaunchKernelGGL(pack_emit_kernel, dim3(g->in_vr.n), dim3(64), 0, s, g->in_vr.rows, place, g->in_vr.n, pack_row0, g->in_pk, g->in_pk_packs.ent,
                       g->in_pk_packs.pack, g->in_pk_packs.rows);
    hipLaunchKernelGGL(pack_count_kernel, dim3(blocks(n_packs)), dim3(256), 0, s, pack_nrows, g->in_pk_packs.pack, n_packs);
  }
  e = hipStreamSynchronize(s);
  if (e == hipSuccess) e = hipGetLastError();
  if (e != hipSuccess) {
    rg::set_error("rg_graph_create_device: build failed: %s", hipGetErrorString(e));
    rg_graph_destroy(g);
    return 1;
  }
  *out = g;
  return 0;
}
```

red-gnn_amd/csrc/layer_fwd.hip:

```cpp
#include "layer_fwd_kernel.h"
#include "layer_fwd_src1.h"
#include "layer_fwd_wp.h"

extern "C" size_t rg_layer_fwd_scratch_bytes(const rg_frontier* f, const rg_graph* g, int32_t ld) {
  if (!f || !g) return 0;
  return rg::align_up((size_t)f->B * g->in_vr.n_slots * ld * sizeof(float), 256) + rg::align_up((size_t)f->B * g->in_vr.n_slots, 256) + 256;
}

static bool src1_applies(const rg_frontier* f, const rg_graph* g, int32_t level) {
  return level == 1 && f->level >= 1 && f->single_source && f->sub && !f->win_lo && g->n_time == 0 && g->out_bt_pos && g->out_bt_rt;
}

static int plan_general(const rg_frontier* f, const rg_graph* g, int32_t level, int64_t n_old, int64_t n_new, int64_t n_edges, int32_t ld) {
  if (g->in_pk_packs.n == 0 || level != f->level || n_old < 0 || n_new <= 0 || n_edges < 0 || !rgwp::offsets_fit(n_old, ld)) return 1;
  const double candidates = (double)n_new * (double)g->n_fact / (double)g->n_ent;
  const bool tiny = n_new * 16 < (int64_t)f->B * f->n_ent;
  const bool short_rows = (double)g->n_fact < 12.0 * (double)g->n_ent;
  if (!tiny && !short_rows && (double)n_edges >= 0.4 * candidates) return 1;
  const double group_bytes = (double)n_old * ld * sizeof(float) / f->BW;
  int code = group_bytes <= 3.0 * (1 << 20) ? 2 : (group_bytes <= 6.0 * (1 << 20) ? 3 : 4);
  auto items = [&](int c) { return (int64_t)f->BW * (1 << (c - 2)) * g->in_pk_packs.n; };
  while (code < 5 && items(code) < 16384 && n_edges > 256 * items(code)) ++code;
  return code;
}

static int plan_walk(const rg_frontier* f, const rg_graph* g, int32_t level, int64_t n_old, int64_t n_new, int64_t n_edges, int32_t ld) {
  return src1_applies(f, g, level) ? 8 : plan_general(f, g, level, n_old, n_new, n_edges, ld);
}

extern "C" int rg_layer_fwd_single_source(const rg_frontier* f, const rg_graph* g, int32_t level) {
  return f && g && src1_applies(f, g, level) ? 1 : 0;
}

extern "C" int rg_layer_fwd_plan(const rg_frontier* f, const rg_graph* g, int32_t level, int64_t n_old, int64_t n_new,
                                 int64_t n_edges, int32_t ld) {
  if (!f || !g) return 1;
  return plan_general(f, g, level, n_old, n_new, n_edges, ld);
}

extern "C" int rg_layer_fwd(const rg_frontier* f, const rg_graph* g, int32_t level, int64_t n_new, const float* hidden,
                            const float* rela, int32_t d, int32_t ld, const float* a_s, const float* a_r,
                            const float* a_q, int32_t ap, const float* w_alpha, const float* b_alpha, int32_t attn_dim,
                            float* agg_out, void* scratch, size_t scratch_bytes, int32_t walk, void* stream) {
  RG_CHECK(f && g && hidden && rela && a_s && a_r && a_q && w_alpha && b_alpha && agg_out, "rg_layer_fwd: NULL argument");
  RG_CHECK((((uintptr_t)hidden | (uintptr_t)rela | (uintptr_t)a_s | (uintptr_t)a_r | (uintptr_t)a_q | (uintptr_t)agg_out |
             (uintptr_t)scratch) & 15) == 0, "rg_layer_fwd: float buffers must be 16-B aligned");
  RG_CHECK(walk >= 0 && walk <= 8, "rg_layer_fwd: walk=%d not in 0..8", walk);
  RG_CHECK(walk != 8 || src1_applies(f, g, level), "rg_layer_fwd: the single-source walk (8) needs level 1 of a frontier started by "
           "rg_frontier_reset, on a static graph (level %d, newest %d)", level, f->level);
  rgfwd::FwdArgs A;
  if (rgfwd::fill_common("rg_layer_fwd", f, g, level, n_new, d, ld, ap, attn_dim, scratch, scratch_bytes,
                         rg_layer_fwd_scratch_bytes(f, g, ld), &A)) return 1;
  if (n_new == 0) return 0;
  A.hidden = (const float4*)hidden; A.rela = (const float4*)rela;
  A.a_s = (const float4*)a_s; A.a_r = (const float4*)a_r; A.a_q = (const float4*)a_q;
  A.w_alpha = w_alpha; A.b_alpha = b_alpha;
  A.agg = (float4*)agg_out; A.partial = (float4*)scratch;
  hipStream_t s = (hipStream_t)stream;
  if (walk == 0)
    walk = plan_walk(f, g, level, f->n_nodes[(level - 1) % f->n_levels], f->n_nodes[level % f->n_levels],
                     level == f->level ? f->n_edges : -1, ld);
  if (walk == 8) {
    rgsrc1::Src1Args S;
    S.B = f->B; S.W = f->W; S.sub = f->sub; S.out_ptr = g->out_ptr; S.in_ptr = g->in_ptr;
    S.list_pk = g->out_bt_pk; S.list_rt = g->out_bt_rt; S.list_pos = g->out_bt_pos; S.bm_new = A.bm_new;
    S.hidden = A.hidden; S.rela = A.rela; S.ld4 = A.ld4; S.a_s = A.a_s; S.a_r = A.a_r; S.a_q = A.a_q;
    S.w_alpha = w_alpha; S.b_alpha = b_alpha; S.attn_dim = attn_dim; S.agg = A.agg;
    f->queues_clean = A.walk.queues_clean;
    return rgsrc1::launch(S, ld / 4, ap / 4, g->max_out_deg, s);
  }
  if (walk >= 2 && f->n_nodes[(level - 1) % f->n_levels] < 0 && !rgwp::offsets_fit((int64_t)f->B * f->n_ent, ld))
    walk = 1;
  if (walk >= 2) {
    RG_CHECK(g->in_pk_packs.n > 0, "rg_layer_fwd: the word-parallel walk needs a static graph with packed entries");
    RG_CHECK(level == f->level, "rg_layer_fwd: the word-parallel walk reads the entity-major bitmaps of the newest hop only "
             "(level %d, newest %d)", level, f->level);
    const int64_t n_old = f->n_nodes[(level - 1) % f->n_levels] >= 0 ? f->n_nodes[(level - 1) % f->n_levels] : (int64_t)f->B * f->n_ent;
    RG_CHECK(rgwp::offsets_fit(n_old, ld), "rg_layer_fwd: the word-parallel walk addresses the previous level by 32-bit byte offsets "
             "(%lld rows x %d floats is 4 GiB or more)", (long long)n_old, ld);
    rgwp::WpArgs W;
    W.n_sub = 1 << (walk - 2);
    W.n_packs = g->in_pk_packs.n; W.BW = f->BW; W.W = f->W; W.n_slots = g->in_vr.n_slots;
    W.n_items = (int64_t)f->BW * W.n_sub * W.n_packs;
    W.ent = g->in_pk_packs.ent; W.pack = g->in_pk_packs.pack; W.rows = g->in_pk_packs.rows;
    W.bits_old = f->bitsT[f->tcur ^ 1]; W.bits_new = f->bitsT[f->tcur];
    W.bm_old = A.bm_old; W.bm_new = A.bm_new;
    W.hidden = A.hidden; W.rela = A.rela; W.ld4 = A.ld4; W.a_s = A.a_s; W.a_r = A.a_r; W.a_q = A.a_q;
    W.w_alpha = w_alpha; W.b_alpha = b_alpha; W.attn_dim = attn_dim; W.n_rela_rows = g->n_rela_rows;
    W.agg = A.agg; W.partial = A.partial; W.queues = f->queues; W.queues_clean = A.walk.queues_clean;
    const int64_t n_e = level == f->level ? (f->n_edges >= 0 ? f->n_edges : f->edge_hint) : -1;
    const int64_t by_work = n_e < 0 ? 2 : 200 * W.n_items / std::max<int64_t>(n_e, 1);
    W.ipt = (int32_t)std::max<int64_t>(std::min<int64_t>(std::min<int64_t>(by_work, W.n_items / 8192), 32), 1);
    const size_t n_part = (size_t)f->B * g->in_vr.n_slots;
    W.written = n_part ? (uint8_t*)scratch + rg::align_up(n_part * ld * sizeof(float), 256) : nullptr;
    if (n_part && rg::zero_async(W.written, rg::align_up(n_part, 256), s)) return 1;
    if (rgwp::launch(W, ap / 4, s)) return 1;
    return rgfwd::launch_combine(A, f->B, g->in_vr, s, W.written);
  }
  const bool dense = n_new * 4 >= (int64_t)f->B * f->n_ent;
  return rgfwd::dispatch<false>(A, ld / 4, ap / 4, f->B, g->in_vr, dense, rg::walk_kpg(g->n_fact, g->in_vr.n), s);
}
```

red-gnn_amd/csrc/layer_fwd_kernel.h:

```cpp
#pragma once
#include "walk.h"

namespace rgfwd {
namespace {

struct FwdArgs {
  rg::WalkArgs walk;
  const int2* in_hr;
  const uint32_t* in_pk;
  const int2* bm_old;
  const int2* bm_new;
  int W;
  const float4* hidden;
  const float4* rela;
  int ld4;
  const float4* a_s;
  const float4* a_r;
  const float4* a_q;
  const float* w_alpha;
  const float* b_alpha;
  int attn_dim;
  int n_rela_rows;
  int rela_in_lds;
  float4* agg;
  float4* partial;
  const int32_t* in_time;
  const int32_t* q_time;
  int n_time;
  const float4* time_tab;
  const int32_t* win_lo;
  const int32_t* win_hi;
  const int32_t* row_time;
  const int32_t* loop_time;
  int n_data;
};

constexpr int FWD_BLOCK = 512;

template <int G, int AP4, bool PACKED, bool DENSE, int KPG, bool RELA_LDS, bool TEMPORAL>
__global__ __launch_bounds__(FWD_BLOCK, TEMPORAL ? 4 : (G >= 32 ? 4 : 6)) void layer_fwd_kernel(FwdArgs A) {
  extern __shared__ float4 lds[];
  constexpr int BLOCK = FWD_BLOCK;
  float4* stage = lds;
  float4* ar_l = lds + BLOCK;
  float4* w_l = ar_l + A.n_rela_rows * AP4;
  float4* rela_l = w_l + AP4;
  int4* recs = reinterpret_cast<int4*>(rela_l + (RELA_LDS ? A.n_rela_rows * G : 0));

  rg::stage_attention<AP4, BLOCK>(ar_l, w_l, A.a_r, A.n_rela_rows, A.w_alpha, A.attn_dim);
  if constexpr (RELA_LDS) {
    for (int i = threadIdx.x; i < A.n_rela_rows * G; i += BLOCK) {
      const int r = i / G, c = i - r * G;
      rela_l[i] = c < A.ld4 ? A.rela[(int64_t)r * A.ld4 + c] : rg::f4zero();
    }
  }
  __syncthreads();
  const float b_alpha = A.b_alpha[0];

  const int lane = threadIdx.x & 63, wv = threadIdx.x >> 6;
  const int lane_g = lane & (G - 1), gi_w = lane / G;
  float4* my_stage = stage + wv * 64 + gi_w * G;
  const bool row_lane = lane_g < A.ld4;
  const int lane_c = row_lane ? lane_g : A.ld4 - 1;

  auto run_item = [&](int beg, int end, int b) -> float4 {
    const float4* aq_p = A.a_q + (int64_t)b * AP4;
    float4 aq[AP4 <= 2 ? AP4 : 1];
    if constexpr (AP4 <= 2) {
#pragma unroll
      for (int k = 0; k < AP4; ++k) aq[k] = aq_p[k];
    }
    const int2* bm_row = A.bm_old + (int64_t)b * A.W;
    int qt = 0, wlo = 0, whi = 0;
    if constexpr (TEMPORAL) {
      qt = A.q_time[b];
      if (A.win_lo) { wlo = A.win_lo[b]; whi = A.win_hi[b]; }
    }
    float4 acc = rg::f4zero();
    for (int c0 = beg; c0 < end; c0 += G) {
      const int c = c0 + lane_g;
      bool valid = c < end;
      int s = 0, r = 0, trow = 0;
      float alpha = 0.f;
      if (valid) {
        int hd;
        if constexpr (PACKED) { const uint32_t pk = A.in_pk[c]; hd = pk & 0xFFFFF; r = pk >> 20; }
        else { const int2 hr = A.in_hr[c]; hd = hr.x; r = hr.y; }
        const int2 wp = bm_row[hd >> 5];
        valid = rg::bm_has(wp, hd);
        if constexpr (TEMPORAL) {
          if (A.win_lo && valid) {
            const int row = A.in_time[c];
            valid = row >= A.n_data || (row >= wlo && row < whi);
          }
        }
        if (valid) {
          s = rg::bm_rank(wp, hd);
          float z = b_alpha;
#pragma clang loop unroll_count(AP4 >= 8 ? 2 : AP4)
          for (int k = 0; k < AP4; ++k) {
            const float4 as = A.a_s[(int64_t)s * AP4 + k];
            const float4 ar = ar_l[r * AP4 + k];
            const float4 w = w_l[k];
            float4 q;
            if constexpr (AP4 <= 2) q = aq[k]; else q = aq_p[k];
            rg::attn_acc_fwd(z, w, as, ar, q);
          }
          alpha = rg::attn_alpha(z);
          if constexpr (TEMPORAL) {
            if (A.win_lo) {
              const int row = A.in_time[c];
              const int delta = qt - (row >= A.n_data ? A.loop_time[b] : A.row_time[row]);
              trow = min(max(delta, 0), A.n_time - 1);
            } else {
              const int dt = A.in_time[c] - qt;
              const int dir = dt > 0 ? 2 : (dt == 0 ? 1 : 0);
              s = s * 3 + dir;
              r = dir * A.n_rela_rows + r;
              trow = dir * A.n_time + (dt < 0 ? -dt : dt);
            }
          }
        }
      }
      const int cnt = rg::group_compact<G, false>(my_stage, lane, valid,
                                                  make_float4(__int_as_float(s), __int_as_float(r), alpha, __int_as_float(trow)));

      for (int k = 0; k < cnt; k += 4) {
        float4 tp[4], hv[4];
#pragma unroll
        for (int u = 0; u < 4; ++u) tp[u] = my_stage[k + u];
#pragma unroll
        for (int u = 0; u < 4; ++u)
          hv[u] = A.hidden[(int64_t)__float_as_int(tp[u].x) * A.ld4 + lane_c];
#pragma unroll
        for (int u = 0; u < 4; ++u) {
          const int ru = __float_as_int(tp[u].y);
          float4 rv;
          if constexpr (RELA_LDS) rv = rela_l[ru * G + lane_g];
          else rv = A.rela[(int64_t)ru * A.ld4 + lane_c];
          if constexpr (TEMPORAL) {
            const float4 tv = A.time_tab[(int64_t)__float_as_int(tp[u].w) * A.ld4 + lane_c];
            rv.x += tv.x; rv.y += tv.y; rv.z += tv.z; rv.w += tv.w;
          }
          const float al = tp[u].z;
          acc.x = fmaf(al, hv[u].x + rv.x, acc.x);
          acc.y = fmaf(al, hv[u].y + rv.y, acc.y);
          acc.z = fmaf(al, hv[u].z + rv.z, acc.z);
          acc.w = fmaf(al, hv[u].w + rv.w, acc.w);
        }
      }
    }
    return acc;
  };
  auto store_row = [&](int out, float4 acc) {
    if (!row_lane) return;
    if (out >= 0) A.agg[(int64_t)out * A.ld4 + lane_g] = acc;
    else A.partial[(int64_t)(-out - 1) * A.ld4 + lane_g] = acc;
  };
  rg::walk_items<G, DENSE, KPG, BLOCK>(A.walk, recs, [&](const int4& R, bool live) {
    const float4 acc = run_item(R.x, R.x + rg::walk_len(R), R.z);
    if (live) store_row(rg::walk_out(R, A.walk.n_slots), acc);
  });
}

__global__ void combine_kernel(const int4* __restrict__ split, int n_split, int n_slots, int B, const int2* __restrict__ bm_new,
                               int W, const float4* __restrict__ partial, float4* __restrict__ agg, int ld4,
                               const uint8_t* __restrict__ written) {
  const int64_t tid = (int64_t)blockIdx.x * blockDim.x + threadIdx.x;
  const int64_t item = tid / ld4;
  const int c = (int)(tid - item * ld4);
  if (item >= (int64_t)B * n_split) return;
  const int b = (int)(item / n_split);
  const int4 se = split[item - (int64_t)b * n_split];
  const int2 wp = bm_new[(int64_t)b * W + (se.x >> 5)];
  if (!rg::bm_has(wp, se.x)) return;
  const int o = rg::bm_rank(wp, se.x);
  const float4* p = partial + ((int64_t)b * n_slots + se.y) * ld4 + c;
  const uint8_t* wr = written ? written + (int64_t)b * n_slots + se.y : nullptr;
  float4 acc = make_float4(0.f, 0.f, 0.f, 0.f);
  bool started = false;
  for (int k0 = 0; k0 < se.z; k0 += 8) {
    float4 v[8];
    bool on[8];
#pragma unroll
    for (int u = 0; u < 8; ++u) {
      on[u] = k0 + u < se.z && (!wr || wr[k0 + u]);
      v[u] = p[(int64_t)min(k0 + u, se.z - 1) * ld4];
    }
#pragma unroll
    for (int u = 0; u < 8; ++u) {
      if (!on[u]) continue;
      if (!started) { acc = v[u]; started = true; }
      else { acc.x += v[u].x; acc.y += v[u].y; acc.z += v[u].z; acc.w += v[u].w; }
    }
  }
  agg[(int64_t)o * ld4 + c] = acc;
}

inline int launch_combine(const FwdArgs& A, int B, const rg_vrows& vr, hipStream_t s, const uint8_t* written = nullptr) {
  if (vr.n_split > 0) {
    const int64_t threads = (int64_t)B * vr.n_split * A.ld4;
    hipLaunchKernelGGL(combine_kernel, dim3(rg::ceil_div(threads, 256)), dim3(256), 0, s, vr.split, vr.n_split, vr.n_slots, B,
                       A.bm_new, A.W, A.partial, A.agg, A.ld4, written);
    RG_LAUNCH_CHECK();
  }
  return 0;
}

template <int G, int AP4, bool PACKED, bool DENSE, int KPG, bool RELA_LDS, bool TEMPORAL>
int launch3(const FwdArgs& A, size_t lds, int B, const rg_vrows& vr, hipStream_t s) {
  constexpr int BLOCK = FWD_BLOCK;
  auto kern = layer_fwd_kernel<G, AP4, PACKED, DENSE, KPG, RELA_LDS, TEMPORAL>;
  if (lds > 64 * 1024) RG_HIP(hipFuncSetAttribute((const void*)kern, hipFuncAttributeMaxDynamicSharedMemorySize, (int)lds));
  const int per_cu = lds <= 53 * 1024 ? 3 : (lds <= 80 * 1024 ? 2 : 1);
  const int grid = rg::walk_grid(A.walk.n_items, BLOCK, G, DENSE, per_cu, KPG);
  if (!A.walk.queues_clean && rg::zero_async(A.walk.queues, RG_QUEUE_BYTES, s)) return 1;
  hipLaunchKernelGGL(kern, dim3(grid), dim3(BLOCK), lds, s, A);
  RG_LAUNCH_CHECK();
  return launch_combine(A, B, vr, s);
}

template <int G, int AP4, bool PACKED, bool DENSE, int KPG, bool TEMPORAL>
int launch2k(const FwdArgs& A, int B, const rg_vrows& vr, hipStream_t s) {
  size_t lds = (size_t)(FWD_BLOCK + A.n_rela_rows * AP4 + AP4) * sizeof(float4);
  if (!DENSE) lds += (size_t)FWD_BLOCK * sizeof(int4);
  const size_t rela_bytes = (size_t)A.n_rela_rows * G * sizeof(float4);
  RG_CHECK(lds <= 160 * 1024, "rg_layer_fwd: attention tables need %zu B of LDS (> 160 KiB)", lds);
  if constexpr (!TEMPORAL) {
    if (lds + rela_bytes <= 53 * 1024) return launch3<G, AP4, PACKED, DENSE, KPG, true, false>(A, lds + rela_bytes, B, vr, s);
  }
  return launch3<G, AP4, PACKED, DENSE, KPG, false, TEMPORAL>(A, lds, B, vr, s);
}

template <int G, int AP4, bool PACKED, bool DENSE, bool TEMPORAL>
int launch2(const FwdArgs& A, int B, const rg_vrows& vr, int kpg, hipStream_t s) {
  if constexpr (DENSE) {
    if (kpg > 1) return launch2k<G, AP4, PACKED, true, rg::RG_KPG_SHORT, TEMPORAL>(A, B, vr, s);
  }
  return launch2k<G, AP4, PACKED, DENSE, 1, TEMPORAL>(A, B, vr, s);
}

template <int G, int AP4, bool TEMPORAL>
int launch(const FwdArgs& A, int B, const rg_vrows& vr, bool dense, int kpg, hipStream_t s) {
  if (A.in_pk) return dense ? launch2<G, AP4, true, true, TEMPORAL>(A, B, vr, kpg, s) : launch2<G, AP4, true, false, TEMPORAL>(A, B, vr, kpg, s);
  return dense ? launch2<G, AP4, false, true, TEMPORAL>(A, B, vr, kpg, s) : launch2<G, AP4, false, false, TEMPORAL>(A, B, vr, kpg, s);
}

inline int fill_common(const char* who, const rg_frontier* f, const rg_graph* g, int32_t level, int64_t n_new, int32_t d,
                       int32_t ld, int32_t ap, int32_t attn_dim, const void* scratch, size_t scratch_bytes, size_t need, FwdArgs* A) {
  RG_CHECK(g->n_ent == f->n_ent, "%s: graph has %d entities, frontier %d", who, g->n_ent, f->n_ent);
  RG_CHECK(level >= 1 && level <= f->level && level > f->level - f->n_levels + 1, "%s: level %d not resident (current %d, %d kept)",
           who, level, f->level, f->n_levels);
  RG_CHECK(f->n_nodes[level % f->n_levels] < 0 || n_new == f->n_nodes[level % f->n_levels], "%s: n_new=%lld but level %d has %lld nodes",
           who, (long long)n_new, level, (long long)f->n_nodes[level % f->n_levels]);
  RG_CHECK(d > 0 && ld >= d && ld % 4 == 0 && ld >= 16 && ld <= 256, "%s: d=%d ld=%d (need ld%%4==0, 16<=ld<=256)", who, d, ld);
  RG_CHECK(attn_dim > 0 && ap >= attn_dim && ap % 4 == 0, "%s: attn_dim=%d ap=%d", who, attn_dim, ap);
  RG_CHECK(g->in_vr.n_slots == 0 || (scratch && scratch_bytes >= need), "%s: scratch %zu B < required %zu B", who, scratch_bytes, need);
  RG_CHECK((int64_t)f->B * std::max(g->in_vr.n_slots, 1) < ((int64_t)1 << 31) && g->in_vr.n_slots < (1 << 22),
           "%s: batch * hub segments overflows int32", who);
  const int64_t n_items = (int64_t)f->B * g->in_vr.n;
  RG_CHECK(n_items / 8 + ((int64_t)1 << 26) < ((int64_t)1 << 31), "%s: work space too large for 32-bit queue tickets", who);
  A->walk.n_items = n_items; A->walk.n_vrows = g->in_vr.n; A->walk.n_slots = g->in_vr.n_slots; A->walk.vrows = g->in_vr.rows;
  A->walk.bm_test = f->bm_of(level); A->walk.W = f->W; A->walk.queues = f->queues;
  A->walk.queues_clean = f->queues_clean;
  f->queues_clean = false;
  A->in_hr = g->in_hr; A->in_pk = g->in_pk;
  A->bm_old = f->bm_of(level - 1); A->bm_new = f->bm_of(level); A->W = f->W;
  A->ld4 = ld / 4; A->attn_dim = attn_dim; A->n_rela_rows = g->n_rela_rows; A->rela_in_lds = 0;
  A->in_time = nullptr; A->q_time = nullptr; A->n_time = 0; A->time_tab = nullptr;
  A->win_lo = nullptr; A->win_hi = nullptr; A->row_time = nullptr; A->loop_time = nullptr; A->n_data = 0;
  return 0;
}

template <bool TEMPORAL>
int dispatch(const FwdArgs& A, int ld4, int ap4, int B, const rg_vrows& vr, bool dense, int kpg, hipStream_t s) {
  return rg::with_g(ld4, [&](auto g) {
    return rg::with_ap4(ap4, "rg_layer_fwd", [&](auto ap) {
      return launch<decltype(g)::value, decltype(ap)::value, TEMPORAL>(A, B, vr, dense, kpg, s);
    });
  });
}

}
}
```

red-gnn_amd/csrc/walk.h:

```cpp
#pragma once
#include "attn.h"

namespace rg {

struct WalkArgs {
  int64_t n_items;
  int32_t n_vrows;
  int32_t n_slots;
  const int4* vrows;
  const int2* bm_test;
  int W;
  int32_t* queues;
  bool queues_clean = false;
};

constexpr int RG_KPG_SHORT = 8;

__device__ __forceinline__ int walk_len(const int4& R) { return R.y & 255; }
__device__ __forceinline__ int walk_out(const int4& R, int n_slots) {
  const int sp1 = R.y >> 8;
  return sp1 == 0 ? R.w : -(R.z * n_slots + sp1 - 1) - 1;
}

template <int G, bool DENSE, int KPG, int BLOCK, bool ALWAYS = false, typename F = void>
__device__ __forceinline__ void walk_items(const WalkArgs& A, int4* recs, F&& run_item) {
  constexpr int GW = 64 / G, WPB = BLOCK / 64;
  constexpr int STEP = DENSE ? WPB * GW * KPG : WPB * 64;
  const int lane = threadIdx.x & 63, wv = threadIdx.x >> 6, gi_w = lane / G;

  auto test_item = [&](int b, int vr, int4& rec) -> bool {
    const int4 row = A.vrows[vr];
    if constexpr (ALWAYS) { rec = make_int4(row.y, row.z, b, row.x); return true; }
    const int2 wp = A.bm_test[(int64_t)b * A.W + (row.x >> 5)];
    if (!bm_has(wp, row.x)) return false;
    rec = make_int4(row.y, row.z | ((row.w + 1) << 8), b, bm_rank(wp, row.x));
    return true;
  };

  __shared__ int slot[2][4];
  int q = __builtin_amdgcn_s_getreg((3 << 11) | 20) & 7;
  auto resolve = [&](int off, int* out) {
    for (;;) {
      const int64_t qs = A.n_items * q / 8, ql = A.n_items * (q + 1) / 8 - qs;
      if (off < ql) {
        const int64_t item = qs + off;
        const int b0 = (int)(item / A.n_vrows);
        out[0] = b0; out[1] = (int)(item - (int64_t)b0 * A.n_vrows); out[2] = (int)min((int64_t)STEP, ql - off);
        return;
      }
      int head[8];
#pragma unroll
      for (int k = 0; k < 8; ++k) head[k] = __hip_atomic_load(&A.queues[k * RG_QSTRIDE], __ATOMIC_RELAXED, __HIP_MEMORY_SCOPE_AGENT);
      int best = -1;
#pragma unroll
      for (int j = 7; j >= 1; --j) {
        const int k = (q + j) & 7;
        if (head[k] < A.n_items * (k + 1) / 8 - A.n_items * k / 8) best = k;
      }
      if (best < 0) { out[2] = 0; return; }
      q = best;
      off = atomicAdd(&A.queues[q * RG_QSTRIDE], STEP);
    }
  };
  if (threadIdx.x == 0) resolve(atomicAdd(&A.queues[q * RG_QSTRIDE], STEP), slot[0]);
  int4* my_recs = recs + wv * 64;
  for (int p = 0;; p ^= 1) {
    __syncthreads();
    const int b0 = slot[p][0], vr0 = slot[p][1], cnt_items = slot[p][2];
    if (cnt_items == 0) break;
    int next_off = 0;
    if (threadIdx.x == 0) next_off = atomicAdd(&A.queues[q * RG_QSTRIDE], STEP);

    if constexpr (DENSE) {
#pragma unroll 1
      for (int k = 0; k < KPG; ++k) {
        const int idx = k * (WPB * GW) + wv * GW + gi_w;
        int b = b0, vr = vr0 + idx;
        while (vr >= A.n_vrows) { vr -= A.n_vrows; ++b; }
        int4 R = make_int4(0, 0, 0, 0);
        const bool live = idx < cnt_items && test_item(b, vr, R);
        if (!live) { R.x = 0; R.y = 0; }
        run_item(R, live);
      }
    } else {
      const int idx = wv * 64 + lane;
      int b = b0, vr = vr0 + idx;
      while (vr >= A.n_vrows) { vr -= A.n_vrows; ++b; }
      int4 rec = make_int4(0, 0, 0, 0);
      const bool ok = idx < cnt_items && test_item(b, vr, rec);
      const unsigned long long surv = __ballot(ok);
      const int n_surv = __popcll(surv);
      if (n_surv > 0) {
        __builtin_amdgcn_fence(__ATOMIC_ACQ_REL, "wavefront");
        __builtin_amdgcn_wave_barrier();
        if (ok) my_recs[__popcll(surv & ((1ull << lane) - 1ull))] = rec;
        __builtin_amdgcn_fence(__ATOMIC_ACQ_REL, "wavefront");
        __builtin_amdgcn_wave_barrier();
        for (int j = 0; j < n_surv; j += GW) {
          const bool live = j + gi_w < n_surv;
          const int4 R = live ? my_recs[j + gi_w] : make_int4(0, 0, 0, 0);
          run_item(R, live);
        }
      }
    }
    if (threadIdx.x == 0) resolve(next_off, slot[p ^ 1]);
  }
}

static inline int walk_kpg(int64_t n_fact, int32_t n_vrows) {
  return (double)n_fact / std::max(n_vrows, 1) < 12.0 ? RG_KPG_SHORT : 1;
}

static inline int walk_grid(int64_t n_items, int block, int g, bool dense, int per_cu, int kpg) {
  const int64_t steps = ceil_div(n_items, (int64_t)(block / 64) * (dense ? (64 / g) * kpg : 64));
  return (int)std::max<int64_t>(std::min<int64_t>(steps, 256 * per_cu), 1);
}

}
```

red-gnn_amd/engine.py:

```python
import ctypes as C

import numpy as np
import torch

from . import _lib


FORCE_WALK = 0

KERNEL_EVENTS = None
DENSE_EVENTS = None
BWD_EVENTS = None
EXPLAIN_EVENTS = None
PROFILE_EVENTS = None


def _require_gpu(device):
    device = torch.device(device)
    if device.type != "cuda":
        raise _lib.NativeError("red_gnn_amd runs on an MI355X (device 'cuda'); got device %r. "
                               "There is no CPU path in the product — the CPU restatement lives in oracle/ for tests only."
                               % (device,))
    if not torch.cuda.is_available():
        raise _lib.NativeError("red_gnn_amd needs an MI355X: no ROCm device is visible to this process. The HIP path has "
                               "no CPU fallback (the CPU restatement in oracle/ is test infrastructure only).")
    return device


_GRAPH_SERIAL = [0]


def _next_serial():
    _GRAPH_SERIAL[0] += 1
    return _GRAPH_SERIAL[0]


class Graph:

    def __init__(self, n_ent, n_rel, triples, add_inverse=True, device="cuda"):
        self.serial = _next_serial()
        self.device = _require_gpu(device)
        trip = np.ascontiguousarray(np.asarray(triples, dtype=np.int32).reshape(-1, 3))
        self.n_ent, self.n_rel = int(n_ent), int(n_rel)
        h = C.c_void_p()
        with torch.cuda.device(self.device):
            _lib.check(_lib.lib().rg_graph_create(self.n_ent, self.n_rel, _lib.ptr(trip), len(trip),
                                                  1 if add_inverse else 0, C.byref(h)))
        self.handle = h
        self.n_fact = int(_lib.lib().rg_graph_n_fact(h))

    @classmethod
    def from_device(cls, n_ent, n_rel, triples_dev, add_inverse=True):
        self = cls.__new__(cls)
        self.serial = _next_serial()
        self.device = _require_gpu(triples_dev.device)
        assert triples_dev.dtype == torch.int32 and triples_dev.dim() == 2 and triples_dev.shape[1] == 3
        trip = triples_dev.contiguous()
        self.n_ent, self.n_rel = int(n_ent), int(n_rel)
        h = C.c_void_p()
        with torch.cuda.device(self.device):
            _lib.check(_lib.lib().rg_graph_create_device(self.n_ent, self.n_rel, _lib.ptr(trip), trip.shape[0], 1 if add_inverse else 0,
                                                         _lib.stream_ptr(), C.byref(h)))
        self.handle = h
        self.n_fact = int(_lib.lib().rg_graph_n_fact(h))
        return self

    def export_packs(self):
        L = _lib.lib()
        n_packs, n_vrows = C.c_int32(), C.c_int32()
        _lib.check(L.rg_graph_export_packs(self.handle, C.byref(n_packs), C.byref(n_vrows), None, None, None, None))
        vr = np.empty((n_vrows.value, 4), np.int32)
        ent = np.empty((n_packs.value * 128, 2), np.int32)
        pack = np.empty((n_packs.value, 4), np.int32)
        rows = np.empty((n_vrows.value if n_packs.value else 0, 2), np.int32)
        _lib.check(L.rg_graph_export_packs(self.handle, None, None, _lib.ptr(ent), _lib.ptr(pack), _lib.ptr(rows), _lib.ptr(vr)))
        return vr, ent, pack, rows

    def export(self):
        op = np.empty(self.n_ent + 1, np.int32)
        ip = np.empty(self.n_ent + 1, np.int32)
        ort = np.empty((self.n_fact, 2), np.int32)
        ihr = np.empty((self.n_fact, 2), np.int32)
        _lib.check(_lib.lib().rg_graph_export(self.handle, _lib.ptr(op), _lib.ptr(ort), _lib.ptr(ip), _lib.ptr(ihr)))
        return op, ort, ip, ihr

    def export_out_by_tail(self):
        rt = np.empty((self.n_fact, 2), np.int32)
        pos = np.empty(self.n_fact, np.int32)
        _lib.check(_lib.lib().rg_graph_export_out_by_tail(self.handle, _lib.ptr(rt), _lib.ptr(pos), None))
        return rt, pos

    def close(self):
        if getattr(self, "handle", None) is not None and _lib._lib is not None:
            _lib.lib().rg_graph_destroy(self.handle)
        self.handle = None

    def __del__(self):
        try:
            self.close()
        except Exception:
            pass


class TemporalGraph(Graph):

    def __init__(self, n_ent, n_rela_rows, n_time, quads, device="cuda", exclude=None):
        self.serial = _next_serial()
        self.device = _require_gpu(device)
        q = quads if (isinstance(quads, np.ndarray) and quads.dtype == np.int32 and quads.flags.c_contiguous and quads.ndim == 2) \
            else np.ascontiguousarray(np.asarray(quads, dtype=np.int32).reshape(-1, 4))
        self.n_ent, self.n_rel, self.n_rela_rows, self.n_time = int(n_ent), 0, int(n_rela_rows), int(n_time)
        h = C.c_void_p()
        with torch.cuda.device(self.device):
            if exclude is None:
                _lib.check(_lib.lib().rg_tgraph_create(self.n_ent, self.n_rela_rows, self.n_time, _lib.ptr(q), len(q), C.byref(h)))
            else:
                ex = np.ascontiguousarray(np.asarray(exclude, dtype=np.int64).reshape(-1))
                _lib.check(_lib.lib().rg_tgraph_create_excluding(self.n_ent, self.n_rela_rows, self.n_time, _lib.ptr(q), len(q),
                                                                 _lib.ptr(ex), len(ex), C.byref(h)))
        self.handle = h
        self.n_fact = int(_lib.lib().rg_graph_n_fact(h))


    def export_time(self):
        ot = np.empty(self.n_fact, np.int32)
        it = np.empty(self.n_fact, np.int32)
        _lib.check(_lib.lib().rg_graph_export_time(self.handle, _lib.ptr(ot), _lib.ptr(it)))
        return ot, it


class Frontier:

    def __init__(self, n_ent, batch, n_levels=2, device="cuda"):
        self.device = _require_gpu(device)
        L = _lib.lib()
        self.n_ent, self.batch, self.n_levels = int(n_ent), int(batch), int(n_levels)
        nbytes = L.rg_frontier_workspace_bytes(self.n_ent, self.batch, self.n_levels)
        if nbytes == 0:
            raise _lib.NativeError("bad frontier shape n_ent=%d batch=%d n_levels=%d" % (n_ent, batch, n_levels))
        self.workspace = torch.empty(nbytes + 256, dtype=torch.uint8, device=self.device)
        base = self.workspace.data_ptr()
        aligned = (base + 255) // 256 * 256
        h = C.c_void_p()
        _lib.check(L.rg_frontier_create(self.n_ent, self.batch, self.n_levels, C.c_void_p(aligned), nbytes, C.byref(h)))
        self.handle = h
        self._counts = (C.c_int64 * 4)()
        self.level = -1
        self.n_new = self.n_old = self.n_edges = 0
        self.generation = 0
        self.leases = 0

    def reset(self, q_sub):
        assert q_sub.dtype == torch.int32 and q_sub.is_cuda and q_sub.numel() == self.batch
        _lib.check(_lib.lib().rg_frontier_reset(self.handle, _lib.ptr(q_sub), _lib.stream_ptr()))
        self.level, self.n_new, self.n_old, self.n_edges = 0, self.batch, 0, 0
        self.generation += 1

    def reset_nodes(self, nodes):
        assert nodes.dtype == torch.int32 and nodes.is_cuda and nodes.dim() == 2 and nodes.shape[1] == 2
        nodes = nodes.contiguous()
        _lib.check(_lib.lib().rg_frontier_reset_nodes(self.handle, _lib.ptr(nodes), nodes.shape[0], _lib.stream_ptr()))
        self.level, self.n_new, self.n_old, self.n_edges = 0, nodes.shape[0], 0, 0
        self.generation += 1

    def set_window(self, win_lo, win_hi, n_data):
        if win_lo is None:
            self._window = None
            _lib.check(_lib.lib().rg_frontier_set_window(self.handle, None, None, 0))
            return
        assert win_lo.dtype == torch.int32 and win_hi.dtype == torch.int32 and win_lo.is_cuda and win_lo.numel() == self.batch == win_hi.numel()
        self._window = (win_lo.contiguous(), win_hi.contiguous())
        _lib.check(_lib.lib().rg_frontier_set_window(self.handle, _lib.ptr(self._window[0]), _lib.ptr(self._window[1]), int(n_data)))

    def expand(self, graph):
        _lib.check(_lib.lib().rg_frontier_expand(self.handle, graph.handle, self._counts, _lib.stream_ptr()))
        self.n_new, self.n_edges, self.n_old, self.level = (int(self._counts[i]) for i in range(4))
        return self.n_new, self.n_edges, self.n_old

    def expand_async(self, graph):
        _lib.check(_lib.lib().rg_frontier_expand_async(self.handle, graph.handle, _lib.stream_ptr()))
        self.level += 1
        self.n_new = self.n_old = self.n_edges = -1

    def expand_nodes_async(self, graph, nodes, prev, edge_hint=None):
        _lib.check(_lib.lib().rg_frontier_expand_nodes_async(self.handle, graph.handle, _lib.ptr(nodes), _lib.ptr(prev), _lib.stream_ptr()))
        if edge_hint is not None and edge_hint >= 0:
            _lib.check(_lib.lib().rg_frontier_set_edge_hint(self.handle, int(edge_hint)))
        self.level += 1
        self.n_new = self.n_old = self.n_edges = -1

    def count_ptr(self):
        return C.c_void_p(_lib.lib().rg_frontier_count_ptr(self.handle))

    def level_counts(self):
        buf = (C.c_int64 * 32)()
        _lib.check(_lib.lib().rg_frontier_level_counts(self.handle, buf, _lib.stream_ptr()))
        return [(int(buf[2 * l]), int(buf[2 * l + 1])) for l in range(self.level + 1)]

    def nodes_into(self, nodes, prev):
        _lib.check(_lib.lib().rg_frontier_nodes(self.handle, _lib.ptr(nodes), _lib.ptr(prev), None, _lib.stream_ptr()))

    def nodes(self, want_prev=True, want_old_new=True):
        nodes = torch.empty((self.n_new, 2), dtype=torch.int32, device=self.device)
        prev = torch.empty(self.n_new, dtype=torch.int32, device=self.device) if want_prev else None
        old_new = (torch.empty(self.n_old, dtype=torch.int32, device=self.device)
                   if (want_old_new and self.level > 0) else None)
        _lib.check(_lib.lib().rg_frontier_nodes(self.handle, _lib.ptr(nodes), _lib.ptr(prev), _lib.ptr(old_new),
                                                _lib.stream_ptr()))
        return nodes, prev, old_new

    def edges(self, graph, nodes_new, level=None):
        level = self.level if level is None else level
        n_new = nodes_new.shape[0]
        L = _lib.lib()
        scratch = torch.empty(L.rg_frontier_edges_scratch_bytes(n_new), dtype=torch.uint8, device=self.device)
        row_ptr = torch.empty(n_new + 1, dtype=torch.int32, device=self.device)
        _lib.check(L.rg_frontier_edges(self.handle, graph.handle, level, _lib.ptr(nodes_new), n_new, None,
                                       _lib.ptr(row_ptr), _lib.ptr(scratch), _lib.stream_ptr()))
        n_e = int(row_ptr[-1].item())
        edges = torch.empty((n_e, 6), dtype=torch.int32, device=self.device)
        _lib.check(L.rg_frontier_edges(self.handle, graph.handle, level, _lib.ptr(nodes_new), n_new, _lib.ptr(edges),
                                       _lib.ptr(row_ptr), _lib.ptr(scratch), _lib.stream_ptr()))
        return edges, row_ptr

    def scratch(self, nbytes):
        buf = getattr(self, "_scratch", None)
        if buf is None or buf.numel() < nbytes:
            buf = self._scratch = torch.empty(max(nbytes, 256), dtype=torch.uint8, device=self.device)
        return buf

    def close(self):
        if getattr(self, "handle", None) is not None and _lib._lib is not None:
            _lib.lib().rg_frontier_destroy(self.handle)
        self.handle = None

    def __del__(self):
        try:
            self.close()
        except Exception:
            pass


class FrontierLease:
    __slots__ = ("frontier", "generation", "released")

    def __init__(self, frontier):
        self.frontier, self.generation, self.released = frontier, frontier.generation, False
        frontier.leases += 1

    def release(self):
        if not self.released:
            self.released = True
            self.frontier.leases -= 1

    def check(self):
        if self.frontier.generation != self.generation:
            raise RuntimeError("red_gnn_amd: the frontier of this autograd graph was reset by a later forward (generation %d, now %d); "
                               "its level bitmaps are gone, the backward cannot run" % (self.generation, self.frontier.generation))

    def __del__(self):
        self.release()


class FrontierPool:

    def __init__(self, max_keys=64):
        self.max_keys, self.pool = max_keys, {}

    def get(self, n_ent, batch, n_levels, device):
        key = (n_ent, batch, n_levels, str(device), torch.cuda.current_stream(device).cuda_stream)
        frs = self.pool.get(key)
        if frs is None:
            if len(self.pool) >= self.max_keys:
                self.pool = {k: [f for f in v if f.leases > 0] for k, v in self.pool.items()}
                self.pool = {k: v for k, v in self.pool.items() if v}
            frs = self.pool[key] = []
        for fr in frs:
            if fr.leases == 0:
                return fr
        fr = Frontier(n_ent, batch, n_levels, device)
        frs.append(fr)
        return fr

    def clear(self):
        self.pool = {}


def layer_fwd(frontier, graph, level, nodes_new, hidden, rela, d, a_s, a_r, a_q, w_alpha, b_alpha, attn_dim):
    ld, ap = hidden.shape[1], a_s.shape[1]
    for t in (hidden, rela, a_s, a_r, a_q, w_alpha, b_alpha):
        assert t.is_cuda and t.dtype == torch.float32 and t.is_contiguous()
    assert rela.shape[1] == ld and a_r.shape[1] == ap and a_q.shape[1] == ap
    n_new = nodes_new.shape[0]
    agg = torch.empty((n_new, ld), dtype=torch.float32, device=hidden.device)
    nbytes = _lib.lib().rg_layer_fwd_scratch_bytes(frontier.handle, graph.handle, ld)
    scratch = frontier.scratch(nbytes)
    ev = None
    if KERNEL_EVENTS is not None:
        ev = (torch.cuda.Event(enable_timing=True), torch.cuda.Event(enable_timing=True))
        ev[0].record()
    _lib.check(_lib.lib().rg_layer_fwd(frontier.handle, graph.handle, level, n_new,
                                       _lib.ptr(hidden), _lib.ptr(rela), d, ld, _lib.ptr(a_s), _lib.ptr(a_r),
                                       _lib.ptr(a_q), ap, _lib.ptr(w_alpha), _lib.ptr(b_alpha), attn_dim,
                                       _lib.ptr(agg), _lib.ptr(scratch), nbytes, FORCE_WALK, _lib.stream_ptr()))
    if ev is not None:
        ev[1].record()
        KERNEL_EVENTS.append((ev[0], ev[1], frontier.n_edges, n_new))
    return agg


def explain_seed(frontier, level, objs):
    assert objs.dtype == torch.int32 and objs.is_cuda and objs.numel() == frontier.batch
    W = (frontier.n_ent + 31) // 32
    marks = torch.empty((frontier.batch, W), dtype=torch.int32, device=frontier.device)
    reached = torch.empty(frontier.batch, dtype=torch.bool, device=frontier.device)
    _lib.check(_lib.lib().rg_explain_seed(frontier.handle, frontier.batch, frontier.n_ent, level, _lib.ptr(objs.contiguous()),
                                          _lib.ptr(marks), _lib.ptr(reached), _lib.stream_ptr()))
    return marks, reached


def explain_hop(frontier, graph, level, marks, a_s, a_r, a_q, w_alpha, b_alpha, attn_dim, min_alpha):
    for t in (a_s, a_r, a_q, w_alpha, b_alpha):
        assert t.is_cuda and t.dtype == torch.float32 and t.is_contiguous()
    ap = a_s.shape[1]
    assert a_r.shape[1] == ap and a_q.shape[1] == ap
    L, dev = _lib.lib(), frontier.device
    marks_prev = torch.empty_like(marks)
    word_ptr = torch.empty(marks.numel() + 1, dtype=torch.int32, device=dev)
    scratch = frontier.scratch(L.rg_explain_scratch_bytes(frontier.handle) + 256)
    base = scratch.data_ptr()
    aligned = (base + 255) // 256 * 256
    n_e = C.c_int64()
    args = (frontier.handle, graph.handle, frontier.batch, frontier.n_ent, level, _lib.ptr(marks), _lib.ptr(a_s), _lib.ptr(a_r),
            _lib.ptr(a_q), ap, _lib.ptr(w_alpha), _lib.ptr(b_alpha), attn_dim, float(min_alpha))
    ev = None
    if EXPLAIN_EVENTS is not None:
        ev = (torch.cuda.Event(enable_timing=True), torch.cuda.Event(enable_timing=True))
        ev[0].record()
    _lib.check(L.rg_explain_count(*args, _lib.ptr(marks_prev), _lib.ptr(word_ptr), C.c_void_p(aligned),
                                  scratch.numel() - (aligned - base), C.byref(n_e), _lib.stream_ptr()))
    edges = torch.empty((n_e.value, 4), dtype=torch.int32, device=dev)
    alpha = torch.empty(n_e.value, dtype=torch.float32, device=dev)
    if n_e.value:
        _lib.check(L.rg_explain_emit(*args, _lib.ptr(word_ptr), _lib.ptr(edges), _lib.ptr(alpha), _lib.stream_ptr()))
    if ev is not None:
        ev[1].record()
        EXPLAIN_EVENTS.append((ev[0], ev[1], level, n_e.value))
    return marks_prev, edges, alpha


def texplain_hop(frontier, graph, level, marks, a_s, a_r, a_q, w_alpha, b_alpha, attn_dim, min_alpha, entry="rg_texplain"):
    count, emit = getattr(_lib.lib(), entry + "_count"), getattr(_lib.lib(), entry + "_emit")
    for t in (a_s, a_r, a_q, w_alpha, b_alpha):
        assert t.is_cuda and t.dtype == torch.float32 and t.is_contiguous()
    ap = a_s.shape[1]
    assert a_r.shape == (graph.n_rela_rows, ap) and a_q.shape == (frontier.batch, ap)
    L, dev = _lib.lib(), frontier.device
    marks_prev = torch.empty_like(marks)
    word_ptr = torch.empty(marks.numel() + 1, dtype=torch.int32, device=dev)
    scratch = frontier.scratch(L.rg_explain_scratch_bytes(frontier.handle) + 256)
    base = scratch.data_ptr()
    aligned = (base + 255) // 256 * 256
    n_e = C.c_int64()
    args = (frontier.handle, graph.handle, frontier.batch, frontier.n_ent, level, _lib.ptr(marks), _lib.ptr(a_s), _lib.ptr(a_r),
            _lib.ptr(a_q), ap, _lib.ptr(w_alpha), _lib.ptr(b_alpha), attn_dim, float(min_alpha))
    ev = None
    if EXPLAIN_EVENTS is not None:
        ev = (torch.cuda.Event(enable_timing=True), torch.cuda.Event(enable_timing=True))
        ev[0].record()
    _lib.check(count(*args, _lib.ptr(marks_prev), _lib.ptr(word_ptr), C.c_void_p(aligned),
                                   scratch.numel() - (aligned - base), C.byref(n_e), _lib.stream_ptr()))
    edges = torch.empty((n_e.value, 4), dtype=torch.int32, device=dev)
    alpha = torch.empty(n_e.value, dtype=torch.float32, device=dev)
    time = torch.empty(n_e.value, dtype=torch.int32, device=dev)
    if n_e.value:
        _lib.check(emit(*args, _lib.ptr(word_ptr), _lib.ptr(edges), _lib.ptr(alpha), _lib.ptr(time), _lib.stream_ptr()))
    if ev is not None:
        ev[1].record()
        EXPLAIN_EVENTS.append((ev[0], ev[1], level, n_e.value))
    return marks_prev, edges, alpha, time


def xexplain_hop(frontier, graph, level, marks, a_s, a_r, a_q, w_alpha, b_alpha, attn_dim, min_alpha):
    return texplain_hop(frontier, graph, level, marks, a_s, a_r, a_q, w_alpha, b_alpha, attn_dim, min_alpha, entry="rg_xexplain")


def explain_gather(hop, batch, edges, alpha, row_first, row_base, edges_out, alpha_out):
    assert edges.dtype == torch.int32 and edges.is_contiguous() and edges_out.is_contiguous() and alpha_out.is_contiguous()
    assert row_first.dtype == torch.int64 and row_base.dtype == torch.int64
    _lib.check(_lib.lib().rg_explain_gather(edges.shape[0], hop, batch, _lib.ptr(edges), _lib.ptr(alpha.contiguous()),
                                            _lib.ptr(row_first.contiguous()), _lib.ptr(row_base.contiguous()), edges_out.shape[0],
                                            _lib.ptr(edges_out), _lib.ptr(alpha_out), _lib.stream_ptr()))


def attn_profile(frontier, graph, level, a_s, a_r, a_q, w_alpha, b_alpha, attn_dim, sum_out, count_out):
    for t in (a_s, a_r, a_q, w_alpha, b_alpha):
        assert t.is_cuda and t.dtype == torch.float32 and t.is_contiguous()
    ap = a_s.shape[1]
    assert a_r.shape == (2 * graph.n_rel + 1, ap) and a_q.shape == (frontier.batch, ap)
    for t in (sum_out, count_out):
        assert t.is_cuda and t.dtype == torch.int64 and t.is_contiguous() and t.shape == (frontier.batch, a_r.shape[0])
    ev = None
    if PROFILE_EVENTS is not None:
        ev = (torch.cuda.Event(enable_timing=True), torch.cuda.Event(enable_timing=True))
        ev[0].record()
    _lib.check(_lib.lib().rg_attn_profile(frontier.handle, graph.handle, frontier.batch, frontier.n_ent, level, a_s.shape[0],
                                          _lib.ptr(a_s), _lib.ptr(a_r), _lib.ptr(a_q), ap, _lib.ptr(w_alpha), _lib.ptr(b_alpha),
                                          attn_dim, _lib.ptr(sum_out), _lib.ptr(count_out), _lib.stream_ptr()))
    if ev is not None:
        ev[1].record()
        PROFILE_EVENTS.append((ev[0], ev[1], level))


def tattn_profile(frontier, graph, level, q_time, a_s, a_r, a_q, w_alpha, b_alpha, attn_dim, sum_out, count_out):
    for t in (a_s, a_r, a_q, w_alpha, b_alpha):
        assert t.is_cuda and t.dtype == torch.float32 and t.is_contiguous()
    ap = a_s.shape[1]
    assert a_r.shape == (graph.n_rela_rows, ap) and a_q.shape == (frontier.batch, ap)
    assert q_time.is_cuda and q_time.dtype == torch.int32 and q_time.is_contiguous() and q_time.numel() == frontier.batch
    for t in (sum_out, count_out):
        assert t.is_cuda and t.dtype == torch.int64 and t.is_contiguous() and t.shape == (frontier.batch, 3, a_r.shape[0])
    ev = None
    if PROFILE_EVENTS is not None:
        ev = (torch.cuda.Event(enable_timing=True), torch.cuda.Event(enable_timing=True))
        ev[0].record()
    _lib.check(_lib.lib().rg_tattn_profile(frontier.handle, graph.handle, frontier.batch, frontier.n_ent, level, a_s.shape[0],
                                           _lib.ptr(q_time), _lib.ptr(a_s), _lib.ptr(a_r), _lib.ptr(a_q), ap, _lib.ptr(w_alpha),
                                           _lib.ptr(b_alpha), attn_dim, _lib.ptr(sum_out), _lib.ptr(count_out), _lib.stream_ptr()))
    if ev is not None:
        ev[1].record()
        PROFILE_EVENTS.append((ev[0], ev[1], level))


def xattn_profile(frontier, graph, level, q_time, loop_time, row_time, lag_bin, n_bins, a_s, a_r, a_q, w_alpha, b_alpha, attn_dim, sum_out,
                  count_out):
    for t in (a_s, a_r, a_q, w_alpha, b_alpha):
        assert t.is_cuda and t.dtype == torch.float32 and t.is_contiguous()
    ap = a_s.shape[1]
    assert a_r.shape == (graph.n_rela_rows, ap) and a_q.shape == (frontier.batch, ap)
    for t in (q_time, loop_time, row_time):
        assert t.is_cuda and t.dtype == torch.int32 and t.is_contiguous()
    assert q_time.numel() == frontier.batch and loop_time.numel() == frontier.batch
    assert lag_bin.is_cuda and lag_bin.dtype == torch.uint8 and lag_bin.is_contiguous() and lag_bin.dim() == 1 and lag_bin.numel() >= 1
    for t in (sum_out, count_out):
        assert t.is_cuda and t.dtype == torch.int64 and t.is_contiguous() and t.shape == (frontier.batch, n_bins, a_r.shape[0])
    ev = None
    if PROFILE_EVENTS is not None:
        ev = (torch.cuda.Event(enable_timing=True), torch.cuda.Event(enable_timing=True))
        ev[0].record()
    _lib.check(_lib.lib().rg_xattn_profile(frontier.handle, graph.handle, frontier.batch, frontier.n_ent, level, a_s.shape[0],
                                           _lib.ptr(q_time), _lib.ptr(loop_time), _lib.ptr(row_time), _lib.ptr(lag_bin), lag_bin.numel(),
                                           int(n_bins), _lib.ptr(a_s), _lib.ptr(a_r), _lib.ptr(a_q), ap, _lib.ptr(w_alpha),
                                           _lib.ptr(b_alpha), attn_dim, _lib.ptr(sum_out), _lib.ptr(count_out), _lib.stream_ptr()))
    if ev is not None:
        ev[1].record()
        PROFILE_EVENTS.append((ev[0], ev[1], level))


def layer_fwd_plan(frontier, graph, level, n_old, n_new, n_edges, ld):
    return int(_lib.lib().rg_layer_fwd_plan(frontier.handle, graph.handle, level, n_old, n_new, n_edges, ld))


def layer_fwd_walk(frontier, graph, level, n_old, n_new, n_edges, ld):
    if _lib.lib().rg_layer_fwd_single_source(frontier.handle, graph.handle, level):
        return 8
    return layer_fwd_plan(frontier, graph, level, n_old, n_new, n_edges, ld)


def layer_fwd_scratch_bytes(frontier, graph, ld):
    return _lib.lib().rg_layer_fwd_scratch_bytes(frontier.handle, graph.handle, ld)


def layer_fwd_into(frontier, graph, level, n_hint, hidden, rela, d, a_s, a_r, a_q, w_alpha, b_alpha, attn_dim, agg, scratch, walk=1):
    ld, ap = hidden.shape[1], a_s.shape[1]
    _lib.check(_lib.lib().rg_layer_fwd(frontier.handle, graph.handle, level, max(int(n_hint), 1),
                                       _lib.ptr(hidden), _lib.ptr(rela), d, ld, _lib.ptr(a_s), _lib.ptr(a_r),
                                       _lib.ptr(a_q), ap, _lib.ptr(w_alpha), _lib.ptr(b_alpha), attn_dim,
                                       _lib.ptr(agg), _lib.ptr(scratch), scratch.numel(), FORCE_WALK or max(int(walk), 1), _lib.stream_ptr()))


def tlayer_fwd(frontier, graph, level, n_new, q_time, hidden_dir, rela_dir, time_dir, d, a_s, a_r, a_q, w_alpha, b_alpha, attn_dim):
    ld, ap = hidden_dir.shape[1], a_s.shape[1]
    for t in (hidden_dir, rela_dir, time_dir, a_s, a_r, a_q, w_alpha, b_alpha):
        assert t.is_cuda and t.dtype == torch.float32 and t.is_contiguous()
    assert q_time.dtype == torch.int32 and q_time.is_cuda
    agg = torch.empty((n_new, ld), dtype=torch.float32, device=hidden_dir.device)
    nbytes = _lib.lib().rg_layer_fwd_scratch_bytes(frontier.handle, graph.handle, ld)
    scratch = frontier.scratch(nbytes)
    ev = None
    if KERNEL_EVENTS is not None:
        ev = (torch.cuda.Event(enable_timing=True), torch.cuda.Event(enable_timing=True))
        ev[0].record()
    _lib.check(_lib.lib().rg_tlayer_fwd(frontier.handle, graph.handle, level, n_new, _lib.ptr(q_time), _lib.ptr(hidden_dir),
                                        _lib.ptr(rela_dir), _lib.ptr(time_dir), d, ld, _lib.ptr(a_s), _lib.ptr(a_r), _lib.ptr(a_q),
                                        ap, _lib.ptr(w_alpha), _lib.ptr(b_alpha), attn_dim, _lib.ptr(agg), _lib.ptr(scratch),
                                        nbytes, _lib.stream_ptr()))
    if ev is not None:
        ev[1].record()
        KERNEL_EVENTS.append((ev[0], ev[1], frontier.n_edges, n_new))
    return agg


def xlayer_fwd(frontier, graph, level, n_new, q_time, loop_time, row_time, n_data, hidden_p, rela_p, time_p, d, a_s, a_r, a_q, w_alpha, b_alpha, attn_dim):
    ld, ap = hidden_p.shape[1], a_s.shape[1]
    for t in (hidden_p, rela_p, time_p, a_s, a_r, a_q, w_alpha, b_alpha):
        assert t.is_cuda and t.dtype == torch.float32 and t.is_contiguous()
    for t in (q_time, loop_time, row_time):
        assert t.dtype == torch.int32 and t.is_cuda and t.is_contiguous()
    agg = torch.empty((n_new, ld), dtype=torch.float32, device=hidden_p.device)
    nbytes = _lib.lib().rg_layer_fwd_scratch_bytes(frontier.handle, graph.handle, ld)
    scratch = frontier.scratch(nbytes)
    ev = None
    if KERNEL_EVENTS is not None:
        ev = (torch.cuda.Event(enable_timing=True), torch.cuda.Event(enable_timing=True))
        ev[0].record()
    _lib.check(_lib.lib().rg_xlayer_fwd(frontier.handle, graph.handle, level, n_new, _lib.ptr(q_time), _lib.ptr(loop_time), _lib.ptr(row_time),
                                        int(n_data), _lib.ptr(hidden_p), _lib.ptr(rela_p), _lib.ptr(time_p), time_p.shape[0], d, ld,
                                        _lib.ptr(a_s), _lib.ptr(a_r), _lib.ptr(a_q), ap, _lib.ptr(w_alpha), _lib.ptr(b_alpha), attn_dim,
                                        _lib.ptr(agg), _lib.ptr(scratch), nbytes, _lib.stream_ptr()))
    if ev is not None:
        ev[1].record()
        KERNEL_EVENTS.append((ev[0], ev[1], frontier.n_edges, n_new))
    return agg


def layer_bwd(frontier, graph, level, nodes_old, hidden, rela, d, a_s, a_r, a_q, w_alpha, b_alpha, attn_dim, grad_agg):
    ld, ap = hidden.shape[1], a_s.shape[1]
    grad_agg = grad_agg.contiguous()
    n_old = nodes_old.shape[0]
    dev = hidden.device
    g_h = torch.empty_like(hidden)
    g_as = torch.empty_like(a_s)
    g_rela = torch.zeros_like(rela)
    g_ar = torch.zeros_like(a_r)
    g_aq = torch.empty_like(a_q)
    g_w = torch.zeros(attn_dim, dtype=torch.float32, device=dev)
    g_b = torch.zeros(1, dtype=torch.float32, device=dev)
    nbytes = _lib.lib().rg_layer_bwd_scratch_bytes(frontier.handle, graph.handle, ld, ap)
    scratch = frontier.scratch(nbytes)
    ev = None
    if BWD_EVENTS is not None:
        ev = (torch.cuda.Event(enable_timing=True), torch.cuda.Event(enable_timing=True))
        ev[0].record()
    _lib.check(_lib.lib().rg_layer_bwd(frontier.handle, graph.handle, level, n_old,
                                       _lib.ptr(hidden), _lib.ptr(rela), d, ld, _lib.ptr(a_s), _lib.ptr(a_r),
                                       _lib.ptr(a_q), ap, _lib.ptr(w_alpha), _lib.ptr(b_alpha), attn_dim,
                                       _lib.ptr(grad_agg), _lib.ptr(g_h), _lib.ptr(g_rela), _lib.ptr(g_as),
                                       _lib.ptr(g_ar), _lib.ptr(g_aq), _lib.ptr(g_w), _lib.ptr(g_b), _lib.ptr(scratch), nbytes,
                                       _lib.stream_ptr()))
    if ev is not None:
        ev[1].record()
        BWD_EVENTS.append((ev[0], ev[1], level, n_old))
    return g_h, g_rela, g_as, g_ar, g_aq, g_w, g_b


def tlayer_bwd(frontier, graph, level, n_old, q_time, hidden_dir, rela_dir, time_dir, d, a_s, a_r, a_q, w_alpha, b_alpha, attn_dim,
               grad_agg):
    ld, ap = hidden_dir.shape[1], a_s.shape[1]
    grad_agg = grad_agg.contiguous()
    dev = hidden_dir.device
    g_hd = torch.empty_like(hidden_dir)
    g_as = torch.empty_like(a_s)
    g_rd = torch.zeros_like(rela_dir)
    g_td = torch.zeros_like(time_dir)
    g_ar = torch.zeros_like(a_r)
    g_aq = torch.empty_like(a_q)
    g_w = torch.zeros(attn_dim, dtype=torch.float32, device=dev)
    nbytes = _lib.lib().rg_tlayer_bwd_scratch_bytes(frontier.handle, graph.handle, ld, ap)
    scratch = frontier.scratch(nbytes)
    _lib.check(_lib.lib().rg_tlayer_bwd(frontier.handle, graph.handle, level, n_old, _lib.ptr(q_time), _lib.ptr(hidden_dir),
                                        _lib.ptr(rela_dir), _lib.ptr(time_dir), d, ld, _lib.ptr(a_s), _lib.ptr(a_r), _lib.ptr(a_q),
                                        ap, _lib.ptr(w_alpha), _lib.ptr(b_alpha), attn_dim, _lib.ptr(grad_agg), _lib.ptr(g_hd),
                                        _lib.ptr(g_rd), _lib.ptr(g_td), _lib.ptr(g_as), _lib.ptr(g_ar), _lib.ptr(g_aq), _lib.ptr(g_w),
                                        _lib.ptr(scratch), nbytes, _lib.stream_ptr()))
    return g_hd, g_rd, g_td, g_as, g_ar, g_aq, g_w


def xlayer_bwd(frontier, graph, level, n_old, q_time, loop_time, row_time, n_data, hidden_p, rela_p, time_p, d, a_s, a_r, a_q, w_alpha,
               b_alpha, attn_dim, grad_agg):
    ld, ap = hidden_p.shape[1], a_s.shape[1]
    grad_agg = grad_agg.contiguous()
    dev = hidden_p.device
    g_hp = torch.empty_like(hidden_p)
    g_as = torch.empty_like(a_s)
    g_rp = torch.zeros_like(rela_p)
    g_tp = torch.zeros_like(time_p)
    g_ar = torch.zeros_like(a_r)
    g_aq = torch.empty_like(a_q)
    g_w = torch.zeros(attn_dim, dtype=torch.float32, device=dev)
    nbytes = _lib.lib().rg_tlayer_bwd_scratch_bytes(frontier.handle, graph.handle, ld, ap)
    scratch = frontier.scratch(nbytes)
    _lib.check(_lib.lib().rg_xlayer_bwd(frontier.handle, graph.handle, level, n_old, _lib.ptr(q_time), _lib.ptr(loop_time), _lib.ptr(row_time),
                                        int(n_data), _lib.ptr(hidden_p), _lib.ptr(rela_p), _lib.ptr(time_p), time_p.shape[0], d, ld,
                                        _lib.ptr(a_s), _lib.ptr(a_r), _lib.ptr(a_q), ap, _lib.ptr(w_alpha), _lib.ptr(b_alpha), attn_dim,
                                        _lib.ptr(grad_agg), _lib.ptr(g_hp), _lib.ptr(g_rp), _lib.ptr(g_tp), _lib.ptr(g_as), _lib.ptr(g_ar),
                                        _lib.ptr(g_aq), _lib.ptr(g_w), _lib.ptr(scratch), nbytes, _lib.stream_ptr()))
    return g_hp, g_rp, g_tp, g_as, g_ar, g_aq, g_w


_GRAM_SCRATCH = {}


def gram_tn(g, x, colsum=False):
    assert g.is_cuda and x.is_cuda and g.dtype == torch.float32 and x.dtype == torch.float32 and g.shape[0] == x.shape[0]
    assert g.stride(1) == 1 and x.stride(1) == 1
    n_rows, m, n = g.shape[0], g.shape[1], x.shape[1]
    L = _lib.lib()
    out = torch.empty((m, n), dtype=torch.float32, device=g.device)
    cs = torch.empty(m, dtype=torch.float32, device=g.device) if colsum else None
    for m0 in range(0, m, 192):
        mc = min(192, m - m0)
        for n0 in range(0, n, 64):
            nc = min(64, n - n0)
            nbytes = L.rg_gram_tn_scratch_bytes(mc, nc)
            key = (str(g.device), torch.cuda.current_stream(g.device).cuda_stream)
            scratch = _GRAM_SCRATCH.get(key)
            if scratch is None or scratch.numel() < nbytes:
                scratch = _GRAM_SCRATCH[key] = torch.empty(nbytes, dtype=torch.uint8, device=g.device)
            tile = out if (mc == m and nc == n) else torch.empty((mc, nc), dtype=torch.float32, device=g.device)
            cs_t = None
            if colsum and n0 == 0:
                cs_t = cs if mc == m else torch.empty(mc, dtype=torch.float32, device=g.device)
            gv, xv = g[:, m0:m0 + mc], x[:, n0:n0 + nc]
            _lib.check(L.rg_gram_tn(C.c_void_p(gv.data_ptr()), g.stride(0), mc, C.c_void_p(xv.data_ptr()), x.stride(0), nc, n_rows,
                                    _lib.ptr(tile), _lib.ptr(cs_t), _lib.ptr(scratch), scratch.numel(), _lib.stream_ptr()))
            if tile is not out:
                out[m0:m0 + mc, n0:n0 + nc] = tile
            if cs_t is not None and cs_t is not cs:
                cs[m0:m0 + mc] = cs_t
    return (out, cs) if colsum else out


_BLAS_CHOICE = [None]


def prefer_blas(n_rows):
    choice = "cublas" if n_rows < (1 << 17) else "cublaslt"
    if _BLAS_CHOICE[0] != choice:
        import warnings
        with warnings.catch_warnings():
            warnings.simplefilter("ignore")
            torch.backends.cuda.preferred_blas_library(choice)
        _BLAS_CHOICE[0] = choice


def dense_supported(d, attn_dim):
    return bool(_lib.lib().rg_dense_fwd_supported(d, attn_dim))


DENSE_PRECISIONS = {"f32": 0, "f16x2": 1, "f16x3": 2}


def dense_scratch(d, precision, device):
    nbytes = int(_lib.lib().rg_dense_scratch_bytes(d, DENSE_PRECISIONS[precision]))
    return torch.empty(nbytes, dtype=torch.uint8, device=device) if nbytes else None


def dense_fwd(agg, hidden_prev, prev_idx, d, W_h, act, gate, Ws_next=None, attn_dim=0, ap=0, W_final=None, nodes=None,
              n_ent=0, scores_all=None, precision="f32", want_hidden=True):
    n, ld = agg.shape
    hidden = torch.empty_like(agg) if want_hidden else None
    a_s = torch.empty((n, ap), dtype=torch.float32, device=agg.device) if Ws_next is not None else None
    c = lambda t: None if t is None else t.detach().contiguous()
    W_h, w_ih, w_hh, b_ih, b_hh = c(W_h), c(gate.weight_ih_l0), c(gate.weight_hh_l0), c(gate.bias_ih_l0), c(gate.bias_hh_l0)
    Ws_next, W_final = c(Ws_next), c(W_final)
    scratch = dense_scratch(d, precision, agg.device)
    ev = None
    if DENSE_EVENTS is not None:
        ev = (torch.cuda.Event(enable_timing=True), torch.cuda.Event(enable_timing=True))
        ev[0].record()
    _lib.check(_lib.lib().rg_dense_fwd(n, d, ld, _lib.ptr(agg), _lib.ptr(hidden_prev), _lib.ptr(prev_idx), _lib.ptr(W_h),
                                       {"idd": 0, "relu": 1, "tanh": 2}[act], _lib.ptr(w_ih), _lib.ptr(w_hh), _lib.ptr(b_ih),
                                       _lib.ptr(b_hh), _lib.ptr(Ws_next), attn_dim, ap, _lib.ptr(a_s), _lib.ptr(W_final),
                                       _lib.ptr(nodes), n_ent, _lib.ptr(scores_all), _lib.ptr(hidden), DENSE_PRECISIONS[precision],
                                       _lib.ptr(scratch), 0 if scratch is None else scratch.numel(), _lib.stream_ptr()))
    if ev is not None:
        ev[1].record()
        DENSE_EVENTS.append((ev[0], ev[1], n))
    return hidden, a_s


def dense_fwd_dev(n_cap, count_ptr, agg, hidden_prev, prev_idx, d, W_h, act, gate, hidden_out, Ws_next=None, attn_dim=0, ap=0,
                  a_s_out=None, W_final=None, nodes=None, n_ent=0, scores_all=None, n_hint=0, precision="f32", scratch=None):
    ld = agg.shape[1]
    c = lambda t: None if t is None else t.detach().contiguous()
    W_h, w_ih, w_hh, b_ih, b_hh = c(W_h), c(gate.weight_ih_l0), c(gate.weight_hh_l0), c(gate.bias_ih_l0), c(gate.bias_hh_l0)
    Ws_next, W_final = c(Ws_next), c(W_final)
    if scratch is None:
        scratch = dense_scratch(d, precision, agg.device)
    _lib.check(_lib.lib().rg_dense_fwd_dev(n_cap, count_ptr, int(n_hint), d, ld, _lib.ptr(agg), _lib.ptr(hidden_prev), _lib.ptr(prev_idx),
                                           _lib.ptr(W_h), {"idd": 0, "relu": 1, "tanh": 2}[act], _lib.ptr(w_ih), _lib.ptr(w_hh),
                                           _lib.ptr(b_ih), _lib.ptr(b_hh), _lib.ptr(Ws_next), attn_dim, ap, _lib.ptr(a_s_out),
                                           _lib.ptr(W_final), _lib.ptr(nodes), n_ent, _lib.ptr(scores_all), _lib.ptr(hidden_out),
                                           DENSE_PRECISIONS[precision], _lib.ptr(scratch), 0 if scratch is None else scratch.numel(),
                                           _lib.stream_ptr()))


def dense_train_supported(d, act):
    return ((16 <= d <= 64 and d % 4 == 0) or d == 128) and act in ("idd", "relu", "tanh")


def dense_train_fwd(agg, hidden_prev, prev_idx, W_h, act, gate, mask=None, Ws_next=None):
    n, d = agg.shape
    dev = agg.device
    hidden = torch.empty((n, d), dtype=torch.float32, device=dev)
    x = torch.empty((n, d), dtype=torch.float32, device=dev)
    ws = torch.empty((n, 5 * d), dtype=torch.float32, device=dev)
    c = lambda t: None if t is None else t.detach().contiguous()
    common = (n, d, _lib.ptr(c(agg)), _lib.ptr(c(hidden_prev)), _lib.ptr(prev_idx), _lib.ptr(c(W_h)),
              {"idd": 0, "relu": 1, "tanh": 2}[act], _lib.ptr(c(gate.weight_ih_l0)), _lib.ptr(c(gate.weight_hh_l0)),
              _lib.ptr(c(gate.bias_ih_l0)), _lib.ptr(c(gate.bias_hh_l0)), _lib.ptr(c(mask)))
    if Ws_next is None:
        _lib.check(_lib.lib().rg_dense_train_fwd(*common, _lib.ptr(hidden), _lib.ptr(x), _lib.ptr(ws), _lib.stream_ptr()))
        return hidden, x, ws, None
    attn = Ws_next.shape[0]
    ap = (attn + 3) // 4 * 4
    a_s = torch.empty((n, ap), dtype=torch.float32, device=dev)
    _lib.check(_lib.lib().rg_dense_train_fwd_as(*common, _lib.ptr(c(Ws_next)), attn, ap, _lib.ptr(hidden), _lib.ptr(x), _lib.ptr(ws),
                                                _lib.ptr(a_s), _lib.stream_ptr()))
    return hidden, x, ws, a_s


def rows_addmm(base, g, W):
    assert base.is_cuda and base.dtype == g.dtype == W.dtype == torch.float32 and base.stride(1) == 1 and g.stride(1) == 1
    n_rows, n = base.shape
    k = W.shape[0]
    assert g.shape[0] == n_rows and g.shape[1] >= k and W.shape[1] == n
    out = torch.empty((n_rows, n), dtype=torch.float32, device=base.device)
    Wc = W.detach().contiguous()
    _lib.check(_lib.lib().rg_rows_addmm(C.c_void_p(base.data_ptr()), base.stride(0), C.c_void_p(g.data_ptr()), g.stride(0), k, _lib.ptr(Wc), n,
                                        n_rows, _lib.ptr(out), n, _lib.stream_ptr()))
    return out


def rows_linear(x, weight, bias=None):
    assert x.is_cuda and x.dtype == torch.float32 and x.dim() == 2
    if x.stride(1) != 1 or x.stride(0) < x.shape[1]:
        x = x.contiguous()
    w = weight.detach().to(torch.float32).contiguous()
    b = None if bias is None else bias.detach().to(torch.float32).contiguous()
    n_rows, k = x.shape
    n = w.shape[0]
    assert w.shape == (n, k) and (b is None or b.numel() == n)
    out = torch.empty((n_rows, n), dtype=torch.float32, device=x.device)
    _lib.check(_lib.lib().rg_rows_linear(_lib.ptr(x), n_rows, x.stride(0), k, _lib.ptr(w), _lib.ptr(b), n, _lib.ptr(out), n,
                                         _lib.stream_ptr()))
    return out


def dense_train_bwd2(g_h, ws, x, mask, keep, act, W_h, w_ih, w_hh, prev_idx, n_old):
    n, d = x.shape
    dev = x.device
    f = lambda rows, cols: torch.empty((rows, cols), dtype=torch.float32, device=dev)
    dgi, dgh_n, dpre, dagg, g_prev = f(n, 3 * d), f(n, d), f(n, d), f(n, d), f(n_old, d)
    c = lambda t: None if t is None else t.detach().contiguous()
    _lib.check(_lib.lib().rg_dense_train_bwd2(n, d, _lib.ptr(c(g_h)), _lib.ptr(ws), _lib.ptr(x), _lib.ptr(c(mask)), float(keep),
                                              {"idd": 0, "relu": 1, "tanh": 2}[act], _lib.ptr(c(W_h)), _lib.ptr(c(w_ih)), _lib.ptr(c(w_hh)),
                                              _lib.ptr(prev_idx), _lib.ptr(dgi), _lib.ptr(dgh_n), _lib.ptr(dpre), _lib.ptr(dagg), _lib.ptr(g_prev),
                                              _lib.stream_ptr()))
    return dgi, dgh_n, dpre, dagg, g_prev


def dense_train_bwd_supported(d):
    return 16 <= d <= 64 and d % 4 == 0


def dense_train_bwd(g_h, ws, x, mask, keep, act, W_h, w_ih, w_hh):
    n, d = x.shape
    dev = x.device
    f = lambda cols: torch.empty((n, cols), dtype=torch.float32, device=dev)
    dgi, dgh, dpre, dagg, dh0 = f(3 * d), f(3 * d), f(d), f(d), f(d)
    c = lambda t: None if t is None else t.detach().contiguous()
    _lib.check(_lib.lib().rg_dense_train_bwd(n, d, _lib.ptr(c(g_h)), _lib.ptr(ws), _lib.ptr(x), _lib.ptr(c(mask)), float(keep),
                                             {"idd": 0, "relu": 1, "tanh": 2}[act], _lib.ptr(c(W_h)), _lib.ptr(c(w_ih)), _lib.ptr(c(w_hh)),
                                             _lib.ptr(dgi), _lib.ptr(dgh), _lib.ptr(dpre), _lib.ptr(dagg), _lib.ptr(dh0), _lib.stream_ptr()))
    return dgi, dgh, dpre, dagg, dh0


def attn_tables(layers, q_rel, d, ld, attn_dim, ap):
    L, dev = len(layers), q_rel.device
    n_rows, B = layers[0].rela_embed.weight.shape[0], q_rel.numel()
    a_r = torch.empty((L, n_rows, ap), dtype=torch.float32, device=dev)
    a_q = torch.empty((L, B, ap), dtype=torch.float32, device=dev)
    rela_p = torch.empty((L, n_rows, ld), dtype=torch.float32, device=dev) if ld != d else None
    arr = lambda ts: (C.c_void_p * L)(*[t.data_ptr() for t in ts])
    for l in layers:
        for t in (l.rela_embed.weight, l.Wr_attn.weight, l.Wqr_attn.weight, l.Wqr_attn.bias):
            assert t.is_contiguous() and t.dtype == torch.float32 and t.is_cuda
    assert q_rel.dtype == torch.int64 and q_rel.is_contiguous()
    _lib.check(_lib.lib().rg_attn_tables(L, n_rows, B, d, ld, attn_dim, ap, arr([l.rela_embed.weight for l in layers]),
                                         arr([l.Wr_attn.weight for l in layers]), arr([l.Wqr_attn.weight for l in layers]),
                                         arr([l.Wqr_attn.bias for l in layers]), _lib.ptr(q_rel), _lib.ptr(a_r), _lib.ptr(a_q),
                                         _lib.ptr(rela_p), _lib.stream_ptr()))
    return [(a_r[i], a_q[i], rela_p[i] if rela_p is not None else layers[i].rela_embed.weight) for i in range(L)]


def rank(scores, ans_ptr, ans_idx, filt_ptr, filt_idx):
    assert scores.is_cuda and scores.dtype == torch.float32 and scores.is_contiguous()
    B, n_ent = scores.shape
    out = torch.empty(ans_idx.numel(), dtype=torch.float32, device=scores.device)
    _lib.check(_lib.lib().rg_rank(_lib.ptr(scores), B, n_ent, _lib.ptr(ans_ptr), _lib.ptr(ans_idx),
                                  _lib.ptr(filt_ptr), _lib.ptr(filt_idx), _lib.ptr(out), _lib.stream_ptr()))
    return out


def topk(scores, k, q_key=None, known=None):
    assert scores.is_cuda and scores.dtype == torch.float32 and scores.is_contiguous() and scores.dim() == 2
    B, n_ent = scores.shape
    idx = torch.empty((B, k), dtype=torch.int32, device=scores.device)
    val = torch.empty((B, k), dtype=torch.float32, device=scores.device)
    if known is None or known[0].numel() == 0:
        keys = ptr = tails = q_key = None
        n_keys = 0
    else:
        keys, ptr, tails = known
        assert q_key is not None and q_key.dtype == torch.int64 and q_key.is_contiguous() and q_key.numel() == B
        assert keys.dtype == torch.int64 and ptr.dtype == torch.int64 and tails.dtype == torch.int32
        assert all(t.is_cuda and t.is_contiguous() for t in (q_key, keys, ptr, tails)) and ptr.numel() == keys.numel() + 1
        n_keys = keys.numel()
    _lib.check(_lib.lib().rg_topk(_lib.ptr(scores), B, n_ent, int(k), _lib.ptr(q_key), _lib.ptr(keys), _lib.ptr(ptr), _lib.ptr(tails),
                                  n_keys, _lib.ptr(idx), _lib.ptr(val), _lib.stream_ptr()))
    return idx, val


def _known_args(known, q_key, batch, who):
    if known is None or known[0].numel() == 0:
        return None, None, None, None, 0
    keys, ptr, idx = known
    assert q_key is not None and q_key.dtype == torch.int64 and q_key.is_contiguous() and q_key.numel() == batch, who
    assert keys.dtype == torch.int64 and ptr.dtype == torch.int64 and idx.dtype == torch.int32, who
    assert all(t.is_cuda and t.is_contiguous() for t in (q_key, keys, ptr, idx)) and ptr.numel() == keys.numel() + 1, who
    return q_key, keys, ptr, idx, keys.numel()


def segment_rank(scores, ent, seg_ptr, target, key_sp=None, known_sp=None, key_spt=None, known_spt=None):
    assert scores.is_cuda and scores.dtype == torch.float32 and scores.is_contiguous() and scores.dim() == 1
    assert ent.is_cuda and ent.dtype == torch.int32 and ent.is_contiguous() and ent.shape == scores.shape
    assert target.is_cuda and target.dtype == torch.int32 and target.is_contiguous() and target.dim() == 1
    B = target.numel()
    assert seg_ptr.is_cuda and seg_ptr.dtype in (torch.int32, torch.int64) and seg_ptr.is_contiguous() and seg_ptr.numel() == B + 1
    dev = scores.device
    rank, rank_fil, rank_fil_t = (torch.empty(B, dtype=torch.float32, device=dev) for _ in range(3))
    found = torch.empty(B, dtype=torch.int32, device=dev)
    sp, spt = _known_args(known_sp, key_sp, B, "segment_rank: (s, p) index"), _known_args(known_spt, key_spt, B, "segment_rank: (s, p, t) index")
    p = _lib.ptr
    _lib.check(_lib.lib().rg_segment_rank(p(scores), p(ent), scores.numel(), p(seg_ptr), int(seg_ptr.dtype == torch.int64), p(target), B,
                                          p(sp[0]), p(sp[1]), p(sp[2]), p(sp[3]), sp[4], p(spt[0]), p(spt[1]), p(spt[2]), p(spt[3]), spt[4],
                                          p(rank), p(rank_fil), p(rank_fil_t), p(found), _lib.stream_ptr()))
    return rank, rank_fil, rank_fil_t, found


def segment_eval(scores, ent, seg_ptr, target, n_ent, key_a=None, known_a=None, key_b=None, known_b=None):
    assert scores.is_cuda and scores.dtype == torch.float32 and scores.is_contiguous() and scores.dim() == 1
    assert ent.is_cuda and ent.dtype == torch.int32 and ent.is_contiguous() and ent.shape == scores.shape
    assert target.is_cuda and target.dtype == torch.int32 and target.is_contiguous() and target.dim() == 1
    B = target.numel()
    assert seg_ptr.is_cuda and seg_ptr.dtype in (torch.int32, torch.int64) and seg_ptr.is_contiguous() and seg_ptr.numel() == B + 1
    dev = scores.device
    logp = torch.empty(B, dtype=torch.float32, device=dev)
    counts = torch.empty((B, 6), dtype=torch.int32, device=dev)
    visited = torch.empty(B, dtype=torch.int32, device=dev)
    ka, kb = _known_args(known_a, key_a, B, "segment_eval: first index"), _known_args(known_b, key_b, B, "segment_eval: second index")
    p = _lib.ptr
    _lib.check(_lib.lib().rg_segment_eval(p(scores), p(ent), scores.numel(), p(seg_ptr), int(seg_ptr.dtype == torch.int64), p(target), B,
                                          int(n_ent), p(ka[0]), p(ka[1]), p(ka[2]), p(ka[3]), ka[4], p(kb[0]), p(kb[1]), p(kb[2]), p(kb[3]),
                                          kb[4], p(logp), p(counts), p(visited), _lib.stream_ptr()))
    return logp, counts, visited


SEGMENT_TOPK_STAGE_MAX = 24576
SEGMENT_TOPK_LIST_LDS = 256


def segment_topk(scores, ent, seg_ptr, k, q_key=None, known=None, want_prob=True):
    assert scores.is_cuda and scores.dtype == torch.float32 and scores.is_contiguous() and scores.dim() == 1
    assert ent.is_cuda and ent.dtype == torch.int32 and ent.is_contiguous() and ent.shape == scores.shape
    assert seg_ptr.is_cuda and seg_ptr.dtype in (torch.int32, torch.int64) and seg_ptr.is_contiguous() and seg_ptr.dim() == 1
    B = seg_ptr.numel() - 1
    dev = scores.device
    idx = torch.empty((B, k), dtype=torch.int32, device=dev)
    val = torch.empty((B, k), dtype=torch.float32, device=dev)
    prob = torch.empty((B, k), dtype=torch.float32, device=dev) if want_prob else None
    kn = _known_args(known, q_key, B, "segment_topk: known-object index")
    p = _lib.ptr
    _lib.check(_lib.lib().rg_segment_topk(p(scores), p(ent), scores.numel(), p(seg_ptr), int(seg_ptr.dtype == torch.int64), B, int(k),
                                          p(kn[0]), p(kn[1]), p(kn[2]), p(kn[3]), kn[4], p(idx), p(val), p(prob), _lib.stream_ptr()))
    return idx, val, prob


PATHS_MAX_K = 8
PATHS_SCRATCH_BYTES = 256 << 20


def paths_scratch_bytes(n_edges, k):
    return int(_lib.lib().rg_paths_scratch_bytes(int(n_edges), int(k)))


def paths_topk(edges, alpha, offsets, n_hops, k, scratch_bytes=PATHS_SCRATCH_BYTES, offsets_host=None):
    assert edges.is_cuda and edges.dtype == torch.int32 and edges.is_contiguous() and edges.dim() == 2 and edges.shape[1] == 5
    assert alpha.is_cuda and alpha.dtype == torch.float32 and alpha.is_contiguous() and alpha.shape == (edges.shape[0],)
    assert offsets.is_cuda and offsets.dtype == torch.int64 and offsets.is_contiguous() and offsets.dim() == 1
    B, L, dev = offsets.numel() - 1, int(n_hops), edges.device
    path_edge = torch.full((B, k, L), -1, dtype=torch.int64, device=dev)
    path_prod = torch.zeros((B, k), dtype=torch.float64, device=dev)
    path_count = torch.zeros(B, dtype=torch.int32, device=dev)
    if B == 0 or edges.shape[0] == 0:
        return path_edge, path_prod, path_count
    off = offsets.cpu().numpy() if offsets_host is None else offsets_host
    chunks, lo = [], 0
    while lo < B:
        hi = lo + 1
        while hi < B and 0 < paths_scratch_bytes(off[hi + 1] - off[lo], k) <= scratch_bytes:
            hi += 1
        chunks.append((lo, hi))
        lo = hi
    need = [paths_scratch_bytes(off[hi] - off[lo], k) for lo, hi in chunks]
    if min(need) == 0:
        raise ValueError("paths_topk: a chunk of %d edges is beyond the kernel's 2^31 edge indices"
                         % max(off[hi] - off[lo] for lo, hi in chunks))
    scratch = torch.empty(max(need), dtype=torch.uint8, device=dev)
    p = _lib.ptr
    for lo, hi in chunks:
        _lib.check(_lib.lib().rg_paths_topk(p(edges), p(alpha), p(offsets), lo, hi, L, int(k), p(scratch), p(path_edge), p(path_prod),
                                            p(path_count), _lib.stream_ptr()))
    return path_edge, path_prod, path_count


RULE_MAX_HOPS = 32
RULE_MAX_RULES = 65535
RULE_SCRATCH_BYTES = 1 << 30
RULE_EVENTS = None


def rule_ground_scratch_bytes(n_ent, n_rules, n_sources):
    return int(_lib.lib().rg_rule_ground_scratch_bytes(int(n_ent), int(n_rules), int(n_sources)))


def _int_array(x, name, who):
    a = x.detach().cpu().numpy() if torch.is_tensor(x) else np.asarray(x)
    if a.dtype not in (np.int32, np.int64):
        raise ValueError("%s: %s must be int32 or int64 (got %s)" % (who, name, a.dtype))
    return a


def check_rules(n_ent, n_rel, head, body, sources=None):
    who = "rule_ground"
    h, b = _int_array(head, "head", who), _int_array(body, "body", who)
    if h.ndim != 1 or b.ndim != 2 or b.shape[0] != h.shape[0]:
        raise ValueError("%s: head must be [R] and body [R, L] (got %s and %s)" % (who, h.shape, b.shape))
    if not 1 <= b.shape[1] <= RULE_MAX_HOPS:
        raise ValueError("%s: the body length %d is not in 1..%d" % (who, b.shape[1], RULE_MAX_HOPS))
    n_ent, n_rel = int(n_ent), int(n_rel)
    if h.size and (min(h.min(), b.min()) < 0 or max(h.max(), b.max()) > 2 * n_rel):
        raise ValueError("%s: relation id out of range 0..%d (2*n_rel; got %d..%d)"
                         % (who, 2 * n_rel, min(h.min(), b.min()), max(h.max(), b.max())))
    if sources is None:
        s = np.arange(n_ent, dtype=np.int32)
    else:
        s = _int_array(sources, "sources", who)
        if s.ndim != 1:
            raise ValueError("%s: sources must be [S] (got %s)" % (who, s.shape))
        if s.size and (s.min() < 0 or s.max() >= n_ent):
            raise ValueError("%s: source id out of range 0..%d (got %d..%d)" % (who, n_ent - 1, s.min(), s.max()))
        if np.unique(s).size != s.size:
            raise ValueError("%s: duplicate sources (%d ids, %d distinct)" % (who, s.size, np.unique(s).size))
    as32 = lambda a: np.ascontiguousarray(a, dtype=np.int32)
    return as32(h), as32(b), as32(s)


def rule_chunking(n_ent, n_rules, n_sources, scratch_bytes):
    def fits(r, s):
        return 0 < rule_ground_scratch_bytes(n_ent, r, s) <= scratch_bytes

    def largest(hi, ok):
        lo = 1
        while lo < hi:
            mid = (lo + hi + 1) // 2
            lo, hi = (mid, hi) if ok(mid) else (lo, mid - 1)
        return lo
    blocks = (n_sources + 31) // 32
    s_c = 32 * largest(blocks, lambda k: fits(1, 32 * k))
    n_r = largest(min(n_rules, RULE_MAX_RULES), lambda r: fits(r, s_c))
    if rule_ground_scratch_bytes(n_ent, n_r, s_c) == 0:
        raise ValueError("rule_ground: %d entities are beyond the bitmaps' range" % n_ent)
    return n_r, s_c


def rule_ground(graph, head, body, sources=None, scratch_bytes=RULE_SCRATCH_BYTES):
    if getattr(graph, "n_time", 0):
        raise ValueError("rule_ground: temporal graph: rules are grounded on static and inductive graphs only "
                         "(a temporal rule would have to say what it does with time)")
    if isinstance(scratch_bytes, (bool, np.bool_)) or not isinstance(scratch_bytes, (int, np.integer)) or scratch_bytes < 0:
        raise ValueError("rule_ground: scratch_bytes must be a non-negative integer (got %r)" % (scratch_bytes,))
    h, b, s = check_rules(graph.n_ent, graph.n_rel, head, body, sources)
    dev = _require_gpu(graph.device)
    R, L, S = h.shape[0], b.shape[1], s.shape[0]
    counts = torch.zeros((R, 4), dtype=torch.int64, device=dev)
    if R == 0 or S == 0:
        return counts
    n_r, s_c = rule_chunking(graph.n_ent, R, S, int(scratch_bytes))
    h_d, b_d, s_d = (torch.from_numpy(a).to(dev) for a in (h, b, s))
    p = _lib.ptr
    with torch.cuda.device(dev):
        scratch = torch.empty(rule_ground_scratch_bytes(graph.n_ent, min(n_r, R), min(s_c, S)), dtype=torch.uint8, device=dev)
        for r0 in range(0, R, n_r):
            r1 = min(r0 + n_r, R)
            for s0 in range(0, S, s_c):
                s1 = min(s0 + s_c, S)
                if RULE_EVENTS is not None:
                    ev = (torch.cuda.Event(enable_timing=True), torch.cuda.Event(enable_timing=True))
                    ev[0].record()
                _lib.check(_lib.lib().rg_rule_ground(graph.handle, p(h_d[r0:r1]), p(b_d[r0:r1]), r1 - r0, L, p(s_d[s0:s1]), s1 - s0,
                                                     p(scratch), p(counts[r0:r1]), _lib.stream_ptr()))
                if RULE_EVENTS is not None:
                    ev[1].record()
                    RULE_EVENTS.append((ev[0], ev[1], r1 - r0, s1 - s0))
    return counts
```

Before: 30.70 billion edges/s.

## Cache top-degree hub entity rows in LDS for the dense forward walk

```diff
diff --git a/include/redgnn.h b/include/redgnn.h
--- a/include/redgnn.h
+++ b/include/redgnn.h
@@ -30,6 +30,7 @@
 int rg_graph_export(const rg_graph* g, int32_t* out_ptr_host, int32_t* out_rel_tail_host,
                     int32_t* in_ptr_host, int32_t* in_head_rel_host);
 int rg_graph_export_out_by_tail(const rg_graph* g, int32_t* rel_tail_host, int32_t* pos_host, uint32_t* packed_host);
+int rg_graph_export_hubs(const rg_graph* g, int32_t* hub_ent_host, uint8_t* in_hub_host);
 int rg_graph_export_time(const rg_graph* g, int32_t* out_time_host, int32_t* in_time_host);
 
 size_t rg_frontier_workspace_bytes(int32_t n_ent, int32_t batch, int32_t n_levels);
@@ -55,6 +56,8 @@
 int rg_layer_fwd_plan(const rg_frontier* f, const rg_graph* g, int32_t level, int64_t n_old, int64_t n_new,
                       int64_t n_edges, int32_t ld);
 int rg_layer_fwd_single_source(const rg_frontier* f, const rg_graph* g, int32_t level);
+int rg_layer_fwd_hubs(const rg_graph* g);
+int rg_layer_fwd_hub_slots(const rg_graph* g, int32_t ld, int32_t ap);
 int rg_layer_fwd(const rg_frontier* f, const rg_graph* g, int32_t level, int64_t n_new,
                  const float* hidden, const float* rela, int32_t d, int32_t ld,
                  const float* a_s, const float* a_r, const float* a_q, int32_t ap,
diff --git a/red-gnn_amd/_lib.py b/red-gnn_amd/_lib.py
--- a/red-gnn_amd/_lib.py
+++ b/red-gnn_amd/_lib.py
@@ -6,10 +6,10 @@
 
 SYMBOLS = [
     "rg_last_error", "rg_version", "rg_hipgraph_fill_nodes",
-    "rg_graph_create", "rg_graph_create_device", "rg_graph_export_packs", "rg_tgraph_create", "rg_tgraph_create_excluding", "rg_graph_destroy", "rg_graph_n_fact", "rg_graph_export", "rg_graph_export_out_by_tail",
+    "rg_graph_create", "rg_graph_create_device", "rg_graph_export_packs", "rg_tgraph_create", "rg_tgraph_create_excluding", "rg_graph_destroy", "rg_graph_n_fact", "rg_graph_export", "rg_graph_export_out_by_tail", "rg_graph_export_hubs",
     "rg_frontier_workspace_bytes", "rg_frontier_create", "rg_frontier_destroy", "rg_frontier_reset",
     "rg_frontier_reset_nodes", "rg_frontier_expand", "rg_frontier_nodes", "rg_frontier_edges_scratch_bytes", "rg_frontier_edges",
-    "rg_layer_fwd_scratch_bytes", "rg_layer_fwd", "rg_layer_fwd_plan", "rg_layer_fwd_single_source", "rg_tlayer_fwd", "rg_xlayer_fwd", "rg_frontier_set_window", "rg_layer_bwd_scratch_bytes", "rg_layer_bwd", "rg_tlayer_bwd_scratch_bytes", "rg_tlayer_bwd", "rg_xlayer_bwd", "rg_dense_fwd_supported", "rg_dense_scratch_bytes", "rg_dense_fwd", "rg_dense_fwd_dev", "rg_dense_train_fwd", "rg_dense_train_fwd_as", "rg_rows_addmm", "rg_dense_train_bwd", "rg_dense_train_bwd2", "rg_split3_roundtrip", "rg_split3_product_check", "rg_gram_tn_scratch_bytes", "rg_gram_tn", "rg_rank",
+    "rg_layer_fwd_scratch_bytes", "rg_layer_fwd", "rg_layer_fwd_plan", "rg_layer_fwd_single_source", "rg_layer_fwd_hubs", "rg_layer_fwd_hub_slots", "rg_tlayer_fwd", "rg_xlayer_fwd", "rg_frontier_set_window", "rg_layer_bwd_scratch_bytes", "rg_layer_bwd", "rg_tlayer_bwd_scratch_bytes", "rg_tlayer_bwd", "rg_xlayer_bwd", "rg_dense_fwd_supported", "rg_dense_scratch_bytes", "rg_dense_fwd", "rg_dense_fwd_dev", "rg_dense_train_fwd", "rg_dense_train_fwd_as", "rg_rows_addmm", "rg_dense_train_bwd", "rg_dense_train_bwd2", "rg_split3_roundtrip", "rg_split3_product_check", "rg_gram_tn_scratch_bytes", "rg_gram_tn", "rg_rank",
     "rg_frontier_expand_async", "rg_frontier_expand_nodes_async", "rg_frontier_set_edge_hint", "rg_frontier_count_ptr", "rg_frontier_level_counts", "rg_attn_tables",
     "rg_explain_scratch_bytes", "rg_explain_seed", "rg_explain_count", "rg_explain_emit", "rg_explain_gather",
     "rg_topk",
@@ -54,6 +54,7 @@
     L.rg_graph_n_fact.restype = i64
     L.rg_graph_export.argtypes = [vp, vp, vp, vp, vp]
     L.rg_graph_export_out_by_tail.argtypes = [vp, vp, vp, vp]
+    L.rg_graph_export_hubs.argtypes = [vp, vp, vp]
     L.rg_frontier_workspace_bytes.argtypes = [i32, i32, i32]
     L.rg_frontier_workspace_bytes.restype = sz
     L.rg_frontier_create.argtypes = [i32, i32, i32, vp, sz, C.POINTER(vp)]
@@ -77,6 +78,8 @@
     L.rg_layer_fwd.argtypes = [vp, vp, i32, i64, vp, vp, i32, i32, vp, vp, vp, i32, vp, vp, i32, vp, vp, sz, i32, vp]
     L.rg_layer_fwd_plan.argtypes = [vp, vp, i32, i64, i64, i64, i32]
     L.rg_layer_fwd_single_source.argtypes = [vp, vp, i32]
+    L.rg_layer_fwd_hubs.argtypes = [vp]
+    L.rg_layer_fwd_hub_slots.argtypes = [vp, i32, i32]
     L.rg_tlayer_fwd.argtypes = [vp, vp, i32, i64, vp, vp, vp, vp, i32, i32, vp, vp, vp, i32, vp, vp, i32, vp, vp, sz, vp]
     L.rg_xlayer_fwd.argtypes = [vp, vp, i32, i64, vp, vp, vp, i32, vp, vp, vp, i32, i32, i32, vp, vp, vp, i32, vp, vp, i32, vp, vp, sz, vp]
     L.rg_frontier_set_window.argtypes = [vp, vp, vp, i32]
diff --git a/red-gnn_amd/csrc/attn.h b/red-gnn_amd/csrc/attn.h
--- a/red-gnn_amd/csrc/attn.h
+++ b/red-gnn_amd/csrc/attn.h
@@ -53,15 +53,27 @@
   __builtin_amdgcn_wave_barrier();
 }
 
-template <int G, bool WG_RELEASE>
+template <int G, bool WG_RELEASE, bool ZERO_ON_THE_SPOT = false>
 __device__ __forceinline__ int group_compact(float4* my_stage, int lane, bool valid, const float4& t) {
   const int lane_g = lane & (G - 1), gshift = lane & ~(G - 1);
   const unsigned long long gmask = G == 64 ? ~0ull : ((1ull << G) - 1ull);
   const unsigned long long m = (__ballot(valid) >> gshift) & gmask;
-  const int cnt = __popcll(m);
-  const int pos = __popcll(m & ((1ull << lane_g) - 1ull));
+  int cnt, pos;
+  if constexpr (ZERO_ON_THE_SPOT && G <= 32) {
+    cnt = __popc((uint32_t)m);
+    pos = __popc((uint32_t)m & ((1u << lane_g) - 1u));
+  } else {
+    cnt = __popcll(m);
+    pos = __popcll(m & ((1ull << lane_g) - 1ull));
+  }
   strip_fence<WG_RELEASE>();
-  if (lane_g >= cnt) my_stage[lane_g] = f4zero();
+  if constexpr (ZERO_ON_THE_SPOT) {
+    float z = 0.f;
+    asm volatile("" : "+v"(z));
+    if (lane_g >= cnt) my_stage[lane_g] = make_float4(z, z, z, z);
+  } else {
+    if (lane_g >= cnt) my_stage[lane_g] = f4zero();
+  }
   if (valid) my_stage[pos] = t;
   strip_fence<WG_RELEASE>();
   return cnt;
diff --git a/red-gnn_amd/csrc/common.h b/red-gnn_amd/csrc/common.h
--- a/red-gnn_amd/csrc/common.h
+++ b/red-gnn_amd/csrc/common.h
@@ -99,6 +99,8 @@
 };
 
 constexpr int RG_PACK = 128;
+constexpr int RG_HUB_MAX = 64;
+namespace rg { void pick_hubs(const int32_t* out_ptr, int32_t n_ent, int32_t* hub_ent); }
 struct rg_packs {
   int32_t n = 0;
   int2* ent = nullptr;
@@ -124,6 +126,8 @@
   int2* out_bt_rt = nullptr;
   uint32_t* out_bt_pk = nullptr;
   int32_t* out_bt_pos = nullptr;
+  int32_t* hub_ent = nullptr;
+  uint8_t* in_hub = nullptr;
   rg_vrows in_vr, out_vr;
   rg_packs in_pk_packs;
   int32_t* rel_ptr = nullptr;
diff --git a/red-gnn_amd/csrc/graph.hip b/red-gnn_amd/csrc/graph.hip
--- a/red-gnn_amd/csrc/graph.hip
+++ b/red-gnn_amd/csrc/graph.hip
@@ -234,6 +234,17 @@
   }
   return (int)fill.size();
 }
+
+void pick_hubs(const int32_t* out_ptr, int32_t n_ent, int32_t* hub_ent) {
+  std::vector<int32_t> order(n_ent);
+  for (int32_t e = 0; e < n_ent; ++e) order[e] = e;
+  const int32_t k = std::min<int32_t>(n_ent, RG_HUB_MAX);
+  std::partial_sort(order.begin(), order.begin() + k, order.end(), [&](int32_t a, int32_t b) {
+    const int32_t da = out_ptr[a + 1] - out_ptr[a], db = out_ptr[b + 1] - out_ptr[b];
+    return da != db ? da > db : a < b;
+  });
+  for (int32_t i = 0; i < RG_HUB_MAX; ++i) hub_ent[i] = i < k ? order[i] : -1;
+}
 }
 
 static void host_packs(const std::vector<int4>& vrows, const std::vector<uint32_t>& in_pk, HostPacks* hp, rg_packs* out) {
@@ -271,7 +282,7 @@
 extern "C" {
 
 const char* rg_last_error(void) { return rg::g_err.c_str(); }
-int rg_version(void) { return 12; }
+int rg_version(void) { return 13; }
 
 static int build_graph(int32_t n_ent, int32_t n_rel, int32_t n_rela_rows, const std::vector<int32_t>& H,
                        const std::vector<int32_t>& R, const std::vector<int32_t>& T, const std::vector<int32_t>* TIME,
@@ -343,6 +354,18 @@
       A.add(&g->out_bt_pk, out_bt_pk);
     }
   }
+  std::vector<int32_t> hub_ent;
+  std::vector<uint8_t> in_hub;
+  if (!TIME) {
+    hub_ent.resize(RG_HUB_MAX);
+    rg::pick_hubs(out_ptr.data(), n_ent, hub_ent.data());
+    std::vector<uint8_t> slot_of(n_ent, 0);
+    for (int k = 0; k < RG_HUB_MAX; ++k)
+      if (hub_ent[k] >= 0) slot_of[hub_ent[k]] = (uint8_t)(k + 1);
+    in_hub.resize(n_fact);
+    for (int64_t q = 0; q < n_fact; ++q) in_hub[q] = slot_of[in_hr[q].x];
+    A.add(&g->hub_ent, hub_ent); A.add(&g->in_hub, in_hub);
+  }
   std::vector<int32_t> rel_ptr(n_rela_rows + 1, 0), rel_tm(TIME ? n_fact : 0);
   std::vector<int2> rel_ht(n_fact);
   for (int64_t i = 0; i < n_fact; ++i) rel_ptr[R[i] + 1]++;
@@ -484,6 +507,14 @@
   return 0;
 }
 
+int rg_graph_export_hubs(const rg_graph* g, int32_t* hub_ent, uint8_t* in_hub) {
+  RG_CHECK(g != nullptr, "rg_graph_export_hubs: graph is NULL");
+  RG_CHECK(g->hub_ent && g->in_hub, "rg_graph_export_hubs: the graph has no hub slots (static graphs only)");
+  if (hub_ent) RG_HIP(hipMemcpy(hub_ent, g->hub_ent, RG_HUB_MAX * sizeof(int32_t), hipMemcpyDeviceToHost));
+  if (in_hub) RG_HIP(hipMemcpy(in_hub, g->in_hub, g->n_fact * sizeof(uint8_t), hipMemcpyDeviceToHost));
+  return 0;
+}
+
 int rg_graph_export_time(const rg_graph* g, int32_t* out_time, int32_t* in_time) {
   RG_CHECK(g != nullptr, "rg_graph_export_time: graph is NULL");
   RG_CHECK(g->n_time > 0 && g->in_time && g->out_time, "rg_graph_export_time: the graph has no timestamps (build it with rg_tgraph_create)");
diff --git a/red-gnn_amd/csrc/graph_device.hip b/red-gnn_amd/csrc/graph_device.hip
--- a/red-gnn_amd/csrc/graph_device.hip
+++ b/red-gnn_amd/csrc/graph_device.hip
@@ -141,6 +141,19 @@
 __global__ void fill_int2_kernel(int2* __restrict__ p, int64_t n, int2 v) {
   const int64_t i = (int64_t)blockIdx.x * blockDim.x + threadIdx.x;
   if (i < n) p[i] = v;
+}
+
+__global__ void in_hub_kernel(const int2* __restrict__ in_hr, const int32_t* __restrict__ hub_ent, uint8_t* __restrict__ in_hub, int64_t n) {
+  __shared__ int32_t hub[RG_HUB_MAX];
+  if (threadIdx.x < RG_HUB_MAX) hub[threadIdx.x] = hub_ent[threadIdx.x];
+  __syncthreads();
+  const int64_t q = (int64_t)blockIdx.x * blockDim.x + threadIdx.x;
+  if (q >= n) return;
+  const int32_t h = in_hr[q].x;
+  int v = 0;
+  for (int k = 0; k < RG_HUB_MAX; ++k)
+    if (hub[k] == h) v = k + 1;
+  in_hub[q] = (uint8_t)v;
 }
 
 __global__ void max_kernel(const int32_t* __restrict__ ptr, int n_rows, int32_t* __restrict__ out) {
@@ -280,7 +293,10 @@
   DEV_HIP(hipMemcpyAsync(host + 4, vout.counts, 12, hipMemcpyDeviceToHost, s));
   DEV_HIP(hipMemcpyAsync(host + 8, vrel.counts, 12, hipMemcpyDeviceToHost, s));
   DEV_HIP(hipMemcpyAsync(host + 12, flags, 16, hipMemcpyDeviceToHost, s));
+  std::vector<int32_t> out_ptr_h(n_ent + 1), hub_ent_h(RG_HUB_MAX);
+  DEV_HIP(hipMemcpyAsync(out_ptr_h.data(), out_ptr, (size_t)(n_ent + 1) * 4, hipMemcpyDeviceToHost, s));
   DEV_HIP(hipStreamSynchronize(s));
+  rg::pick_hubs(out_ptr_h.data(), n_ent, hub_ent_h.data());
   RG_CHECK(host[12] == 0, "rg_graph_create_device: triple %d out of range", host[12] - 1);
   const bool want_packs = packed && n_rela_rows < (1 << 12);
   int4* place = nullptr; int32_t* pack_nrows = nullptr; int32_t* pack_row0 = nullptr;
@@ -325,6 +341,7 @@
   add((void**)&g->in_vr.rows, vin.rows, (size_t)g->in_vr.n * 16); add((void**)&g->in_vr.split, vin.split, (size_t)g->in_vr.n_split * 16);
   add((void**)&g->out_vr.rows, vout.rows, (size_t)g->out_vr.n * 16); add((void**)&g->out_vr.split, vout.split, (size_t)g->out_vr.n_split * 16);
   add((void**)&g->rel_vr.rows, vrel.rows, (size_t)g->rel_vr.n * 16); add((void**)&g->rel_vr.split, vrel.split, (size_t)g->rel_vr.n_split * 16);
+  add((void**)&g->hub_ent, nullptr, (size_t)RG_HUB_MAX * 4); add((void**)&g->in_hub, nullptr, (size_t)n_fact);
   const size_t ent_off = total;
   if (n_packs > 0) {
     add((void**)&g->in_pk_packs.ent, nullptr, (size_t)n_packs * RG_PACK * 8);
@@ -342,6 +359,8 @@
     if (it.src && it.bytes) (void)hipMemcpyAsync(*it.field, it.src, it.bytes, hipMemcpyDeviceToDevice, s);
   }
   (void)ent_off;
+  (void)hipMemcpyAsync(g->hub_ent, hub_ent_h.data(), (size_t)RG_HUB_MAX * 4, hipMemcpyHostToDevice, s);
+  hipLaunchKernelGGL(in_hub_kernel, dim3(blocks(n_fact)), dim3(256), 0, s, g->in_hr, g->hub_ent, g->in_hub, n_fact);
   if (n_packs > 0) {
     hipLaunchKernelGGL(fill_int2_kernel, dim3(blocks((int64_t)n_packs * RG_PACK)), dim3(256), 0, s, g->in_pk_packs.ent, (int64_t)n_packs * RG_PACK,
                        make_int2(-1, 0));
diff --git a/red-gnn_amd/csrc/layer_fwd.hip b/red-gnn_amd/csrc/layer_fwd.hip
--- a/red-gnn_amd/csrc/layer_fwd.hip
+++ b/red-gnn_amd/csrc/layer_fwd.hip
@@ -24,8 +24,19 @@
   return code;
 }
 
+static bool has_hubs(const rg_graph* g) { return g->hub_ent && g->in_hub && g->n_time == 0; }
+
 static int plan_walk(const rg_frontier* f, const rg_graph* g, int32_t level, int64_t n_old, int64_t n_new, int64_t n_edges, int32_t ld) {
-  return src1_applies(f, g, level) ? 8 : plan_general(f, g, level, n_old, n_new, n_edges, ld);
+  if (src1_applies(f, g, level)) return 8;
+  const int code = plan_general(f, g, level, n_old, n_new, n_edges, ld);
+  return code == 1 && has_hubs(g) ? 9 : code;
+}
+
+extern "C" int rg_layer_fwd_hubs(const rg_graph* g) { return g && has_hubs(g) ? 1 : 0; }
+
+extern "C" int rg_layer_fwd_hub_slots(const rg_graph* g, int32_t ld, int32_t ap) {
+  if (!g || !has_hubs(g) || ld < 4 || ap < 4) return 0;
+  return rg::with_g(ld / 4, [&](auto gl) { return rgfwd::hub_slots(g->n_rela_rows, decltype(gl)::value, ap / 4); });
 }
 
 extern "C" int rg_layer_fwd_single_source(const rg_frontier* f, const rg_graph* g, int32_t level) {
@@ -45,7 +56,7 @@
   RG_CHECK(f && g && hidden && rela && a_s && a_r && a_q && w_alpha && b_alpha && agg_out, "rg_layer_fwd: NULL argument");
   RG_CHECK((((uintptr_t)hidden | (uintptr_t)rela | (uintptr_t)a_s | (uintptr_t)a_r | (uintptr_t)a_q | (uintptr_t)agg_out |
              (uintptr_t)scratch) & 15) == 0, "rg_layer_fwd: float buffers must be 16-B aligned");
-  RG_CHECK(walk >= 0 && walk <= 8, "rg_layer_fwd: walk=%d not in 0..8", walk);
+  RG_CHECK(walk >= 0 && walk <= 9, "rg_layer_fwd: walk=%d not in 0..9", walk);
   RG_CHECK(walk != 8 || src1_applies(f, g, level), "rg_layer_fwd: the single-source walk (8) needs level 1 of a frontier started by "
            "rg_frontier_reset, on a static graph (level %d, newest %d)", level, f->level);
   rgfwd::FwdArgs A;
@@ -69,6 +80,8 @@
     f->queues_clean = A.walk.queues_clean;
     return rgsrc1::launch(S, ld / 4, ap / 4, g->max_out_deg, s);
   }
+  const bool hubs = walk == 9;
+  if (hubs) walk = 1;
   if (walk >= 2 && f->n_nodes[(level - 1) % f->n_levels] < 0 && !rgwp::offsets_fit((int64_t)f->B * f->n_ent, ld))
     walk = 1;
   if (walk >= 2) {
@@ -98,5 +111,9 @@
     return rgfwd::launch_combine(A, f->B, g->in_vr, s, W.written);
   }
   const bool dense = n_new * 4 >= (int64_t)f->B * f->n_ent;
+  if (hubs && dense && has_hubs(g)) {
+    A.hub_ent = g->hub_ent; A.in_hub = g->in_hub;
+    A.n_hub = rg_layer_fwd_hub_slots(g, ld, ap);
+  }
   return rgfwd::dispatch<false>(A, ld / 4, ap / 4, f->B, g->in_vr, dense, rg::walk_kpg(g->n_fact, g->in_vr.n), s);
 }
diff --git a/red-gnn_amd/csrc/layer_fwd_kernel.h b/red-gnn_amd/csrc/layer_fwd_kernel.h
--- a/red-gnn_amd/csrc/layer_fwd_kernel.h
+++ b/red-gnn_amd/csrc/layer_fwd_kernel.h
@@ -3,6 +3,13 @@
 
 namespace rgfwd {
 namespace {
+
+typedef float lds_f4_t __attribute__((ext_vector_type(4)));
+__device__ __forceinline__ float4 lds_read_f4(const float4* p) {
+  const lds_f4_t v = *(const __attribute__((address_space(3))) lds_f4_t*)p;
+  return make_float4(v.x, v.y, v.z, v.w);
+}
+__device__ __forceinline__ int lds_read_i32(const int* p) { return *(const __attribute__((address_space(3))) int*)p; }
 
 struct FwdArgs {
   rg::WalkArgs walk;
@@ -33,12 +40,16 @@
   const int32_t* row_time;
   const int32_t* loop_time;
   int n_data;
+  const int32_t* hub_ent;
+  const uint8_t* in_hub;
+  int n_hub;
 };
 
 constexpr int FWD_BLOCK = 512;
 
-template <int G, int AP4, bool PACKED, bool DENSE, int KPG, bool RELA_LDS, bool TEMPORAL>
+template <int G, int AP4, bool PACKED, bool DENSE, int KPG, bool RELA_LDS, bool TEMPORAL, bool HUBS = false>
 __global__ __launch_bounds__(FWD_BLOCK, TEMPORAL ? 4 : (G >= 32 ? 4 : 6)) void layer_fwd_kernel(FwdArgs A) {
+  static_assert(!HUBS || (DENSE && RELA_LDS && !TEMPORAL), "the hub variant is a static dense walk with the relation rows in LDS");
   extern __shared__ float4 lds[];
   constexpr int BLOCK = FWD_BLOCK;
   float4* stage = lds;
@@ -46,6 +57,11 @@
   float4* w_l = ar_l + A.n_rela_rows * AP4;
   float4* rela_l = w_l + AP4;
   int4* recs = reinterpret_cast<int4*>(rela_l + (RELA_LDS ? A.n_rela_rows * G : 0));
+  float4* hub_h = reinterpret_cast<float4*>(recs);
+  float4* hub_as = hub_h + (HUBS ? A.n_hub * G : 0);
+  float4* hub_aq = hub_as + (HUBS ? A.n_hub * AP4 : 0);
+  int* hub_row = reinterpret_cast<int*>(hub_aq + (HUBS ? AP4 : 0));
+  int hub_b = -1;
 
   rg::stage_attention<AP4, BLOCK>(ar_l, w_l, A.a_r, A.n_rela_rows, A.w_alpha, A.attn_dim);
   if constexpr (RELA_LDS) {
@@ -66,11 +82,12 @@
   auto run_item = [&](int beg, int end, int b) -> float4 {
     const float4* aq_p = A.a_q + (int64_t)b * AP4;
     float4 aq[AP4 <= 2 ? AP4 : 1];
-    if constexpr (AP4 <= 2) {
+    if constexpr (AP4 <= 2 && !HUBS) {
 #pragma unroll
       for (int k = 0; k < AP4; ++k) aq[k] = aq_p[k];
     }
     const int2* bm_row = A.bm_old + (int64_t)b * A.W;
+    const bool cached = HUBS && b == hub_b;
     int qt = 0, wlo = 0, whi = 0;
     if constexpr (TEMPORAL) {
       qt = A.q_time[b];
@@ -86,8 +103,12 @@
         int hd;
         if constexpr (PACKED) { const uint32_t pk = A.in_pk[c]; hd = pk & 0xFFFFF; r = pk >> 20; }
         else { const int2 hr = A.in_hr[c]; hd = hr.x; r = hr.y; }
-        const int2 wp = bm_row[hd >> 5];
-        valid = rg::bm_has(wp, hd);
+        if constexpr (HUBS) {
+          if (cached) { const int hs = A.in_hub[c]; s = hs <= A.n_hub ? -hs : 0; }
+        }
+        int2 wp = make_int2(0, 0);
+        if (HUBS && s < 0) valid = lds_read_i32(hub_row - s - 1) >= 0;
+        else { wp = bm_row[hd >> 5]; valid = rg::bm_has(wp, hd); }
         if constexpr (TEMPORAL) {
           if (A.win_lo && valid) {
             const int row = A.in_time[c];
@@ -95,8 +116,28 @@
           }
         }
         if (valid) {
+          float z = b_alpha;
+          if constexpr (HUBS) {
+            float4 as[AP4];
+            const bool hub = s < 0;
+            if (hub) {
+#pragma unroll
+              for (int k = 0; k < AP4; ++k) as[k] = lds_read_f4(hub_as + (-s - 1) * AP4 + k);
+            }
+            asm volatile("" ::: "memory");
+            if (!hub) {
+              s = rg::bm_rank(wp, hd);
+#pragma unroll
+              for (int k = 0; k < AP4; ++k) as[k] = A.a_s[(int64_t)s * AP4 + k];
+            }
+#pragma unroll
+            for (int k = 0; k < AP4; ++k) {
+              float4 q;
+              if (cached) q = lds_read_f4(hub_aq + k); else q = aq_p[k];
+              rg::attn_acc_fwd(z, w_l[k], as[k], ar_l[r * AP4 + k], q);
+            }
+          } else {
           s = rg::bm_rank(wp, hd);
-          float z = b_alpha;
 #pragma clang loop unroll_count(AP4 >= 8 ? 2 : AP4)
           for (int k = 0; k < AP4; ++k) {
             const float4 as = A.a_s[(int64_t)s * AP4 + k];
@@ -105,6 +146,7 @@
             float4 q;
             if constexpr (AP4 <= 2) q = aq[k]; else q = aq_p[k];
             rg::attn_acc_fwd(z, w, as, ar, q);
+          }
           }
           alpha = rg::attn_alpha(z);
           if constexpr (TEMPORAL) {
@@ -122,16 +164,30 @@
           }
         }
       }
-      const int cnt = rg::group_compact<G, false>(my_stage, lane, valid,
+      const int cnt = rg::group_compact<G, false, HUBS>(my_stage, lane, valid,
                                                   make_float4(__int_as_float(s), __int_as_float(r), alpha, __int_as_float(trow)));
 
       for (int k = 0; k < cnt; k += 4) {
         float4 tp[4], hv[4];
 #pragma unroll
         for (int u = 0; u < 4; ++u) tp[u] = my_stage[k + u];
-#pragma unroll
-        for (int u = 0; u < 4; ++u)
-          hv[u] = A.hidden[(int64_t)__float_as_int(tp[u].x) * A.ld4 + lane_c];
+        if constexpr (HUBS) {
+#pragma unroll
+          for (int u = 0; u < 4; ++u) {
+            const int su = __float_as_int(tp[u].x);
+            if (su < 0) hv[u] = lds_read_f4(rela_l + (A.n_rela_rows - 1 - su) * G + lane_g);
+          }
+          asm volatile("" ::: "memory");
+#pragma unroll
+          for (int u = 0; u < 4; ++u) {
+            const int su = __float_as_int(tp[u].x);
+            if (su >= 0) hv[u] = A.hidden[(int64_t)su * A.ld4 + lane_c];
+          }
+        } else {
+#pragma unroll
+          for (int u = 0; u < 4; ++u)
+            hv[u] = A.hidden[(int64_t)__float_as_int(tp[u].x) * A.ld4 + lane_c];
+        }
 #pragma unroll
         for (int u = 0; u < 4; ++u) {
           const int ru = __float_as_int(tp[u].y);
@@ -157,10 +213,37 @@
     if (out >= 0) A.agg[(int64_t)out * A.ld4 + lane_g] = acc;
     else A.partial[(int64_t)(-out - 1) * A.ld4 + lane_g] = acc;
   };
+  auto refresh_hubs = [&](int b0) {
+    if constexpr (HUBS) {
+      b0 = __builtin_amdgcn_readfirstlane(b0);
+      if (b0 == hub_b) return;
+      hub_b = b0;
+      constexpr int ROW = G + AP4;
+      const int2* bm_row = A.bm_old + (int64_t)b0 * A.W;
+      int tid = threadIdx.x;
+      asm volatile("" : "+v"(tid));
+      for (int i = tid; i < A.n_hub * ROW; i += BLOCK) {
+        const int k = i / ROW, c = i - k * ROW;
+        const int e = A.hub_ent[k];
+        int s = -1;
+        if (e >= 0) {
+          const int2 wp = bm_row[e >> 5];
+          if (rg::bm_has(wp, e)) s = rg::bm_rank(wp, e);
+        }
+        if (c == 0) hub_row[k] = s;
+        if (i < AP4) hub_aq[i] = A.a_q[(int64_t)b0 * AP4 + i];
+        if (s >= 0) {
+          if (c < G) hub_h[k * G + c] = c < A.ld4 ? A.hidden[(int64_t)s * A.ld4 + c] : rg::f4zero();
+          else hub_as[k * AP4 + (c - G)] = A.a_s[(int64_t)s * AP4 + (c - G)];
+        }
+      }
+      __syncthreads();
+    }
+  };
   rg::walk_items<G, DENSE, KPG, BLOCK>(A.walk, recs, [&](const int4& R, bool live) {
     const float4 acc = run_item(R.x, R.x + rg::walk_len(R), R.z);
     if (live) store_row(rg::walk_out(R, A.walk.n_slots), acc);
-  });
+  }, refresh_hubs);
 }
 
 __global__ void combine_kernel(const int4* __restrict__ split, int n_split, int n_slots, int B, const int2* __restrict__ bm_new,
@@ -207,10 +290,10 @@
   return 0;
 }
 
-template <int G, int AP4, bool PACKED, bool DENSE, int KPG, bool RELA_LDS, bool TEMPORAL>
+template <int G, int AP4, bool PACKED, bool DENSE, int KPG, bool RELA_LDS, bool TEMPORAL, bool HUBS = false>
 int launch3(const FwdArgs& A, size_t lds, int B, const rg_vrows& vr, hipStream_t s) {
   constexpr int BLOCK = FWD_BLOCK;
-  auto kern = layer_fwd_kernel<G, AP4, PACKED, DENSE, KPG, RELA_LDS, TEMPORAL>;
+  auto kern = layer_fwd_kernel<G, AP4, PACKED, DENSE, KPG, RELA_LDS, TEMPORAL, HUBS>;
   if (lds > 64 * 1024) RG_HIP(hipFuncSetAttribute((const void*)kern, hipFuncAttributeMaxDynamicSharedMemorySize, (int)lds));
   const int per_cu = lds <= 53 * 1024 ? 3 : (lds <= 80 * 1024 ? 2 : 1);
   const int grid = rg::walk_grid(A.walk.n_items, BLOCK, G, DENSE, per_cu, KPG);
@@ -220,6 +303,15 @@
   return launch_combine(A, B, vr, s);
 }
 
+constexpr size_t FWD_LDS_3PER_CU = 53 * 1024;
+constexpr bool hubs_built(int g, int ap4) { return ap4 == 2 && g >= 8; }
+inline int hub_slots(int n_rela_rows, int g, int ap4) {
+  if (!hubs_built(g, ap4)) return 0;
+  const size_t base = (size_t)(FWD_BLOCK + n_rela_rows * ap4 + ap4 + n_rela_rows * g + ap4) * sizeof(float4);
+  if (base > FWD_LDS_3PER_CU) return 0;
+  return (int)std::min<size_t>((FWD_LDS_3PER_CU - base) / ((size_t)(g + ap4) * sizeof(float4) + sizeof(int)), RG_HUB_MAX);
+}
+
 template <int G, int AP4, bool PACKED, bool DENSE, int KPG, bool TEMPORAL>
 int launch2k(const FwdArgs& A, int B, const rg_vrows& vr, hipStream_t s) {
   size_t lds = (size_t)(FWD_BLOCK + A.n_rela_rows * AP4 + AP4) * sizeof(float4);
@@ -227,7 +319,14 @@
   const size_t rela_bytes = (size_t)A.n_rela_rows * G * sizeof(float4);
   RG_CHECK(lds <= 160 * 1024, "rg_layer_fwd: attention tables need %zu B of LDS (> 160 KiB)", lds);
   if constexpr (!TEMPORAL) {
-    if (lds + rela_bytes <= 53 * 1024) return launch3<G, AP4, PACKED, DENSE, KPG, true, false>(A, lds + rela_bytes, B, vr, s);
+    if constexpr (DENSE && hubs_built(G, AP4)) {
+      if (A.n_hub > 0) {
+        const size_t hub_bytes = rg::align_up((size_t)A.n_hub * ((G + AP4) * sizeof(float4) + sizeof(int)), 16) + AP4 * sizeof(float4);
+        RG_CHECK(lds + rela_bytes + hub_bytes <= FWD_LDS_3PER_CU, "rg_layer_fwd: %d hub slots do not fit LDS", A.n_hub);
+        return launch3<G, AP4, PACKED, true, KPG, true, false, true>(A, lds + rela_bytes + hub_bytes, B, vr, s);
+      }
+    }
+    if (lds + rela_bytes <= FWD_LDS_3PER_CU) return launch3<G, AP4, PACKED, DENSE, KPG, true, false>(A, lds + rela_bytes, B, vr, s);
   }
   return launch3<G, AP4, PACKED, DENSE, KPG, false, TEMPORAL>(A, lds, B, vr, s);
 }
@@ -269,6 +368,7 @@
   A->ld4 = ld / 4; A->attn_dim = attn_dim; A->n_rela_rows = g->n_rela_rows; A->rela_in_lds = 0;
   A->in_time = nullptr; A->q_time = nullptr; A->n_time = 0; A->time_tab = nullptr;
   A->win_lo = nullptr; A->win_hi = nullptr; A->row_time = nullptr; A->loop_time = nullptr; A->n_data = 0;
+  A->hub_ent = nullptr; A->in_hub = nullptr; A->n_hub = 0;
   return 0;
 }
 
diff --git a/red-gnn_amd/csrc/walk.h b/red-gnn_amd/csrc/walk.h
--- a/red-gnn_amd/csrc/walk.h
+++ b/red-gnn_amd/csrc/walk.h
@@ -22,8 +22,9 @@
   return sp1 == 0 ? R.w : -(R.z * n_slots + sp1 - 1) - 1;
 }
 
-template <int G, bool DENSE, int KPG, int BLOCK, bool ALWAYS = false, typename F = void>
-__device__ __forceinline__ void walk_items(const WalkArgs& A, int4* recs, F&& run_item) {
+struct WalkNoStep { __device__ __forceinline__ void operator()(int) const {} };
+template <int G, bool DENSE, int KPG, int BLOCK, bool ALWAYS = false, typename F = void, typename S = WalkNoStep>
+__device__ __forceinline__ void walk_items(const WalkArgs& A, int4* recs, F&& run_item, S&& on_step = S()) {
   constexpr int GW = 64 / G, WPB = BLOCK / 64;
   constexpr int STEP = DENSE ? WPB * GW * KPG : WPB * 64;
   const int lane = threadIdx.x & 63, wv = threadIdx.x >> 6, gi_w = lane / G;
@@ -70,6 +71,7 @@
     if (cnt_items == 0) break;
     int next_off = 0;
     if (threadIdx.x == 0) next_off = atomicAdd(&A.queues[q * RG_QSTRIDE], STEP);
+    on_step(b0);
 
     if constexpr (DENSE) {
 #pragma unroll 1
diff --git a/red-gnn_amd/engine.py b/red-gnn_amd/engine.py
--- a/red-gnn_amd/engine.py
+++ b/red-gnn_amd/engine.py
@@ -83,6 +83,12 @@
         ihr = np.empty((self.n_fact, 2), np.int32)
         _lib.check(_lib.lib().rg_graph_export(self.handle, _lib.ptr(op), _lib.ptr(ort), _lib.ptr(ip), _lib.ptr(ihr)))
         return op, ort, ip, ihr
+
+    def export_hubs(self):
+        hub_ent = np.empty(64, np.int32)
+        in_hub = np.empty(self.n_fact, np.uint8)
+        _lib.check(_lib.lib().rg_graph_export_hubs(self.handle, _lib.ptr(hub_ent), _lib.ptr(in_hub)))
+        return hub_ent, in_hub
 
     def export_out_by_tail(self):
         rt = np.empty((self.n_fact, 2), np.int32)
@@ -464,7 +470,8 @@
 def layer_fwd_walk(frontier, graph, level, n_old, n_new, n_edges, ld):
     if _lib.lib().rg_layer_fwd_single_source(frontier.handle, graph.handle, level):
         return 8
-    return layer_fwd_plan(frontier, graph, level, n_old, n_new, n_edges, ld)
+    code = layer_fwd_plan(frontier, graph, level, n_old, n_new, n_edges, ld)
+    return 9 if code == 1 and _lib.lib().rg_layer_fwd_hubs(graph.handle) else code
 
 
 def layer_fwd_scratch_bytes(frontier, graph, ld):
```

Result: slower. 26.94 billion edges/s (-12.2%).
